# HpWang-whu/RoReg

Hardware: AMD Instinct MI355X
Metric: pair-registrations/sec (higher is better)
Workload: dtype f32 (every f32 operand enters the fp16 matrix cores as hi + lo fp16 under a per-keypoint power-of-two block scale: <= 22 significant bits relative to a CONSERVATIVE per-keypoint bound -- measured on the extractor: the bound sits 2^2..2^6 above the keypoint's true coefficient maximum (config.f16x2_sc

## Files before the change

### include/roreg_hip.h

```cpp
#ifndef ROREG_HIP_H
#define ROREG_HIP_H

#include <stdint.h>
#include <stddef.h>

#ifdef __cplusplus
extern "C" {
#endif

#define ROREG_ABI_VERSION 6
int roreg_abi_version(void);
const char *roreg_last_error(void);

int roreg_set_group_tables(const int32_t *P_host, const int32_t *Nei_host, const double *R_host);

size_t roreg_group_conv_packed_size(int Cin, int Cout, int KS);
int roreg_group_conv_pack_weights(const float *W_host , int Cin, int Cout, int KS,
                                  float *wpack_host );
size_t roreg_group_conv_workspace_size(int B, int Cin, int Cout, int Lin, int Lout, int KS);
int roreg_group_conv(const float *x, const float *wpack, const float *bias,
                     const float *bn_scale, const float *bn_shift, const float *residual,
                     float *out, const int32_t *gather,
                     int B, int Cin, int Cout, int Lin, int Lout, int KS,
                     float *workspace, size_t workspace_floats, void *stream);
// ... 75 lines not shown
int roreg_des2r_irrep(const float *coef1, const int64_t *rows1, const float *coef0, const int64_t *rows0, const void *feats1,
                      const void *feats0, int feat_bf16, int M, int64_t *idx_out, void *stream);
int roreg_des2r_recheck_count(int reset, int32_t *count_out);
int roreg_feat_coefs(const void *x, int x_bf16, float *out, int B, int C, int split, void *stream);

int roreg_et_gather(const void *before0, const void *before1, const void *after0, const void *after1,
                    int feat_bf16 ,
                    const int64_t *rows0, const int64_t *rows1, const int64_t *pre_idx, int M,
                    float *x_out, void *stream);

int roreg_quat_to_trans(const float *q, const int64_t *anchor, const double *keys0, const int64_t *rows0,
                        const double *keys1, const int64_t *rows1, int M,
                        double *Trans_out, float *quat_out, void *stream);

int roreg_ransac_score(const double *k0, const double *k1, const double *w, int w_f32, int M,
                       const double *Trans, const int64_t *hyp_rows, int H, double ird,
                       double *overlap_out, int32_t *best_out, uint8_t *mask_out, void *stream);

int roreg_refine(const double *k0, const double *k1, const double *w, int w_f32, int M,
                 const double *T_in, int t_in_stride ,
                 const double *Trans, const int64_t *hyp_rows, const int32_t *best,
                 double dist, double *T_out, double *stats_out ,
                 void *stream);

typedef struct {
    const void *before0, *before1, *after0, *after1;
    const double *keys0, *keys1;
    const int64_t *matches;
    const int64_t *sel;
    int32_t n, pad_;
    int64_t off;
    const float *coef0, *coef1;
} roreg_lt_task;
int roreg_lt_prepare_batch(const roreg_lt_task *tasks_dev, int n_tasks, int max_n, int flags, int64_t *dr_out, float *x_out,
                           const float *bn_scale , const float *bn_shift, float *x_bound_out , void *stream);
int roreg_lt_finish_batch(const roreg_lt_task *tasks_dev, int n_tasks, int max_n, const float *q_all, const int64_t *dr_all,
                          double *Trans_out, void *stream);
int roreg_role_max(const void *before, const void *after, int feat_bf16, const float *bn_scale , const float *bn_shift, float *out,
                   int N, void *stream);
int roreg_row_bound_roles(const void *x_spatial, int x_bf16, float *bound_out, const float *role_scale, const float *role_shift, float *role_out, int B,
                          void *stream);
int roreg_inv_descriptor_roles(const void *eqv, int eqv_bf16, float *inv, const float *role_scale, const float *role_shift, float *role_out, int N,
                               void *stream);
int roreg_lt_prepare_rows(const roreg_lt_task *tasks_dev, const float *const *roles_dev, int n_tasks, int max_n, int flags, int64_t *dr_out,
                          uint64_t *rows_out, float *x_bound_out, void *stream);

typedef struct {
    const double *keys0, *keys1;
    const int64_t *matches;
    const double *w;
    const double *Trans;
    const int64_t *hyp_rows;
    int32_t M, H;
    int64_t koff;
} roreg_ransac_task;
size_t roreg_ransac_batch_workspace(int n_tasks, long long total_M, int max_H);
int roreg_ransac_batch(const roreg_ransac_task *tasks_dev, int n_tasks, long long total_M, int max_M, int max_H, double ird,
                       int w_f32 ,
                       int32_t *best_out, double *T1_out, double *stats1_out, double *T2_out, double *stats2_out,
                       void *workspace, size_t workspace_bytes, void *stream);

int roreg_refine_batch(const roreg_ransac_task *tasks_dev, const int32_t *sel_dev, int n_sel, long long total_M, const double *T_in,
                       double dist, int w_f32, double *T_out, double *stats_out, const void *workspace, void *stream);

int roreg_mt_shuffle_prefix(const uint32_t *seeds, int n_jobs, const int32_t *sizes, int per_job, int take, int64_t *out, int n_threads);

int roreg_mt_stream_shuffle_prefix(uint32_t *key, int32_t *pos, const int32_t *sizes, int n_lists, int take, int64_t *out);

int roreg_yohoc_draw(const uint32_t *words, long long n_words, const double *cdf, const int32_t *bin_size, int max_iter, int max_tries,
                     int32_t *bin_out, int64_t *pick_out, int32_t *n_hyp_out, long long *words_used);

typedef struct {
    const void *src;
    const int64_t *rows;
    void *dst;
    int32_t n, pad_;
} roreg_gather_task;
int roreg_gather_rows_batch(const roreg_gather_task *tasks_dev, int n_tasks, int max_n, int row_bytes, void *stream);

int roreg_gather_rows_f64(const double *src, const int64_t *rows, int M, int width, double *out, void *stream);

size_t roreg_topk_dot_workspace_size(int m, int n, int k);
int roreg_topk_dot(const float *A, int m, const float *B, int n, int k, int64_t *idx_out, float *val_out ,
                   float *ws, size_t ws_floats, const int32_t *segA, const int32_t *segB, int n_seg, int max_m, int max_n, void *stream);

int roreg_linear(const float *x, int L, int Cin, const float *W , const float *b, int Cout, float *y, void *stream);
int roreg_linear_path(int path);
int roreg_linear_cat3(const float *pos , const float *table , const int64_t *idx ,
                      const float *conf , int m, int k, const float *W , const float *b, int Cout, float *y, void *stream);
int roreg_linear_mfma(const float *x, int L, int Cin, const float *W , const float *b, int Cout, float *y, void *stream);

int roreg_instnorm_stats(const float *h, int L, int C, float eps, float *mean_rstd, double *ws, const int32_t *seg_off, int n_seg,
                         int mult, void *stream);

int roreg_mlp_tail(const float *h, int L, int Cmid, const float *mean_rstd, const float *W2 , const float *b2,
                   float *y, const int32_t *seg_off, int n_seg, int mult, void *stream);
int roreg_mlp_tail_mfma(const float *h, int L, int Cmid, const float *mean_rstd, const float *W2 , const float *b2,
                   float *y, const int32_t *seg_off, int n_seg, int mult, void *stream);

int roreg_context_colmax(const float *R, int L, const int32_t *seg_off, int n_seg, int max_len, float *ctx_out, float *ws, void *stream);

int roreg_knn_attention(const float *qp, const float *kp, const float *vp, const int64_t *idx, int k_is_table, int v_is_table,
                        int m, int k, float *x_out, void *stream);

int roreg_rm_elementwise(int op, const float *a, const float *b, const float *c, const int64_t *idx, int L, int k, int C,
                         float *out, float *ws, void *stream);

size_t roreg_sinkhorn_workspace_size(int m, int n);
int roreg_sinkhorn(const float *src_final, int m, const float *tgt_final, int n, float alpha, int iters, float *Z_out,
                   int64_t *matches0, int64_t *matches1, float *mscores0, float *mscores1, float *ws, size_t ws_floats, void *stream);

size_t roreg_sinkhorn_batch_workspace_size(int n_seg, int max_m, int max_n, long long total_m, long long total_n);
int roreg_sinkhorn_batch_consts(const int32_t *seg_src_host, const int32_t *seg_tgt_host, int n_seg, float *consts_host);
int roreg_sinkhorn_batch(const float *src_final, const float *tgt_final, const int32_t *seg_src, const int32_t *seg_tgt,
                         const int32_t *seg_src_host, const int32_t *seg_tgt_host, const float *consts, int n_seg, float alpha, int iters,
                         int64_t *matches0, int64_t *matches1, float *mscores0, float *mscores1, float *ws, size_t ws_floats,
                         void *stream);

size_t roreg_sinkhorn_batch2_workspace_size(int n_seg, int max_m, int max_n, long long total_m, long long total_n);
int roreg_sinkhorn_batch2(const float *src_final, const float *tgt_final, const int32_t *seg_src, const int32_t *seg_tgt,
                          const int32_t *seg_src_host, const int32_t *seg_tgt_host, const float *consts, int n_seg, float alpha, int iters,
                          int64_t *matches0, int64_t *matches1, float *mscores0, float *mscores1, float *ws, size_t ws_floats,
                          int recompute, void *stream);
size_t roreg_sinkhorn_batch3_workspace_size(int n_seg, int max_m, int max_n, long long total_m, long long total_n, int recompute, int want_Z);
int roreg_sinkhorn_batch3(const float *src_final, const float *tgt_final, const int32_t *seg_src, const int32_t *seg_tgt,
                          const int32_t *seg_src_host, const int32_t *seg_tgt_host, const float *consts, int n_seg, float alpha, int iters,
                          int64_t *matches0, int64_t *matches1, float *mscores0, float *mscores1, float *ws, size_t ws_floats,
                          int recompute, float *Z_out, void *stream);
int roreg_write_files(const char *const *paths, const void *const *headers, const int32_t *header_len, const void *const *data,
                      const int64_t *nbytes, int n, int n_threads);
int roreg_yohoc_draw_many(const uint32_t *seeds, int n_pairs, const int64_t *anchors, const int64_t *offsets, int max_iter, int max_tries,
                          int64_t *rows_out, int32_t *n_hyp_out, double *giveup_out, int n_threads);
size_t roreg_mlp_head_workspace(int L, int n_seg, int C1);
int roreg_mlp_head(const float *x, const float *pos, const float *table, const int64_t *idx, const float *conf, int m, int k, int L, int Cin,
                   const float *W1, const float *b1, int C1, const float *Wr, const float *br, float *h, float *y, const int32_t *seg_off,
                   int n_seg, int mult, float eps, float *mean_rstd, double *ws, void *stream);
int roreg_sinkhorn_early_exit(int on);
int roreg_sinkhorn_iteration_stats(long long *iterations, long long *pairs, int reset, void *stream);

int roreg_set_fourier_tables(const float *F_host);
size_t roreg_irrep_gemm_tiles(int O, int B, int32_t *tiles_host);
size_t roreg_irrep_gemm_tiles_m(int O, int B, int tile_m , int32_t *tiles_host);
int roreg_irrep_gemm(const float *const *X, float *const *Out, const float *const *Add, const float *const *Wpack, int C, int O, int B,
                     const int32_t *tiles_dev, int n_tiles, void *stream);
int roreg_irrep_gemm_split(const float *const *X, float *const *Out, const float *const *Add, const void *const *Wsplit, int C, int O, int B,
                           const int32_t *tiles_dev, int n_tiles, void *stream);
int roreg_irrep_gemm_f16x2(const float *const *X, float *const *Out, const float *const *Add, const void *const *Wsplit2,
                           const float *x_bound_dev, int w_exp, const float *next_u_dev, const float *next_v_dev, float *out_bound_dev,
                           int C, int O, int B, const int32_t *tiles_dev, int n_tiles,
                           int tile_m ,
                           int x_planes , void *stream);
int roreg_gemm_persistent(int on);
int roreg_gemm_thin(int on);
int roreg_row_bound(const void *x_spatial, int x_bf16 , const float *bn_scale, const float *bn_shift,
                    float *bound_out, int B, int C, void *stream);
int roreg_ft_nonlin(const float *Xin , const float *x_spatial, const float *bias,
                    const float *bias2, const float *bn_scale, const float *bn_shift, const float *resid_spatial,
                    float *Xout , float *out_spatial ,
                    const int32_t *g_map ,
                    int Lout , int Lvalid,
                    int B, int C, int split ,
                    const float *out_bound ,
                    float *out_rowmax ,
                    int spatial_bf16 ,
                    int out_planes ,
                    void *stream);
int roreg_ft_nonlin_packed(const float *Xin, const float *bias, const float *bn_scale, const float *bn_shift, uint32_t *out_words,
                           const int32_t *g_map, int Lout, int Lvalid, int B, int C, const float *out_bound, float *raw_col, int raw_g,
                           void *stream);
int roreg_ft_nonlin_gathered(const uint64_t *rows , const int64_t *dr , int feat_bf16, const float *bn_scale ,
                             const float *bn_shift, float *Xout, int B, const float *out_bound , int out_planes, void *stream);

typedef struct roreg_icp_grid_desc {
    double origin[3];
    double edge;
    int32_t dims[3];
    int32_t n;
    int64_t cells;
    int64_t reserved;
} roreg_icp_grid_desc;
size_t roreg_icp_grid_size(const double *lo_host, const double *hi_host, int n, double max_dist, roreg_icp_grid_desc *desc_host,
                           size_t *workspace_bytes);
int roreg_icp_grid_build(const float *points, const roreg_icp_grid_desc *desc_host, void *grid, void *workspace, size_t workspace_bytes,
                         void *stream);
typedef struct roreg_icp_task {
    const void *tgt_grid;
    const void *src_grid;
    const double *T0;
    int32_t n_src;
    int32_t slot0;
} roreg_icp_task;
size_t roreg_icp_batch_workspace(int n_tasks, long long total_slots);
int roreg_icp_batch(const roreg_icp_task *tasks, int n_tasks, const int32_t *work, int n_work, long long total_slots, double max_dist,
                    int max_iter, double tol_deg, double tol_t, double *T_out, int32_t *iters_out, int32_t *inliers_out, double *rmse_out,
                    int32_t *status_out, int32_t *assign_out, double *stats_out, void *workspace, size_t workspace_bytes, void *stream);

int roreg_icp_normals(const void *grid, double radius, int min_neighbors, double *out, void *stream);
typedef struct roreg_icp_plane_task {
    const void *tgt_grid;
    const void *src_grid;
    const double *tgt_normals;
    const double *T0;
    int32_t n_src;
    int32_t slot0;
} roreg_icp_plane_task;
size_t roreg_icp_plane_batch_workspace(int n_tasks, long long total_slots);
int roreg_icp_plane_batch(const roreg_icp_plane_task *tasks, int n_tasks, const int32_t *work, int n_work, long long total_slots, double max_dist,
                          int max_iter, double tol_deg, double tol_t, double *T_out, int32_t *iters_out, int32_t *inliers_out, double *rmse_out,
                          int32_t *status_out, int32_t *assign_out, double *stats_out, void *workspace, size_t workspace_bytes, void *stream);

typedef struct roreg_icp_gicp_task {
    const void *tgt_grid;
    const void *src_grid;
    const double *tgt_normals;
    const double *src_normals;
    const double *T0;
    double epsilon;
    int32_t n_src;
    int32_t slot0;
} roreg_icp_gicp_task;
size_t roreg_icp_gicp_batch_workspace(int n_tasks, long long total_slots);
int roreg_icp_gicp_batch(const roreg_icp_gicp_task *tasks, int n_tasks, const int32_t *work, int n_work, long long total_slots, double max_dist,
                         int max_iter, double tol_deg, double tol_t, double *T_out, int32_t *iters_out, int32_t *inliers_out, double *rmse_out,
                         int32_t *status_out, int32_t *assign_out, double *stats_out, void *workspace, size_t workspace_bytes, void *stream);

size_t roreg_icp_eval_workspace(int n_pairs, long long total_slots);
int roreg_icp_eval_batch(const roreg_icp_task *tasks, int n_pairs, const int32_t *work, int n_work, long long total_slots, double max_dist,
                         double *stats_out, double *info_out, int32_t *status_out, int32_t *assign_out, void *workspace, size_t workspace_bytes,
                         void *stream);

size_t roreg_voxel_workspace(int n);
int roreg_voxel_downsample(const float *points, int n, double voxel, int32_t *inverse, int32_t *first, int32_t *counts, int32_t *coords,
                           double *centroid, int32_t *info, void *workspace, size_t workspace_bytes, void *stream);

typedef struct roreg_pg_graph {
    int32_t node0, n_nodes, edge0, n_edges, act0, n_act, anchor, reserved0;
    int64_t h0;
    double tau, lambda0, tol_t, tol_rot, tol_cost, reserved1;
} roreg_pg_graph;
size_t roreg_pg_workspace(const roreg_pg_graph *graphs_host, int n_graphs);
int roreg_pg_optimize_batch(const roreg_pg_graph *graphs_host, const roreg_pg_graph *graphs, int n_graphs, const int32_t *edge_i,
                            const int32_t *edge_j, const int32_t *edge_graph, const double *transforms, const double *infos, const int32_t *var,
                            const int32_t *inc_ptr, const int32_t *inc_edge, const int32_t *act_graph, const int32_t *act_node,
                            const int32_t *walk, int has_init, int max_iter, double *poses, double *cost_out, int32_t *iters_out,
                            int32_t *status_out, double *weights_out, double *chi2_out, double *history_out, double *lin_out, double *H_out,
                            double *gd_out, void *workspace, size_t workspace_bytes, void *stream);

size_t roreg_sparse_map_workspace(int n);
int roreg_sparse_stride_map(const int32_t *coords, int n, int ts, const int32_t *cuts, int n_items, int32_t *coarse, int32_t *parent,
                            int32_t *coarse_cuts, int32_t *info, void *workspace, size_t workspace_bytes, void *stream);
int roreg_sparse_kernel_map(const int32_t *coords_in, int n_in, const int32_t *coords_out, int n_out, int k, int step, int32_t *map,
                            int32_t *info, void *workspace, size_t workspace_bytes, void *stream);
int roreg_sparse_conv(const float *x, int ldx, int Cin, int n_in, const int32_t *map, int n_out, int K, const float *W, int Cout,
                      const float *scale, const float *shift, const float *residual, int ldr, int relu, float *out, int ldo, void *stream);
int roreg_sparse_l2norm(const float *x, int n, int C, float *out, void *stream);

int roreg_profile_enable(int on);
int roreg_profile_read(int slot, double *total_ms, int *launches);

#ifdef __cplusplus
}
#endif
#endif
```

### roreg_amd/_abi.py

```python
import ctypes
from ctypes import c_int, c_void_p, c_size_t, c_double, c_float, c_char_p

import numpy as np

ABI_VERSION = 6

_P = c_void_p
PROTOTYPES = {
    'roreg_abi_version': (c_int, []),
    'roreg_last_error': (c_char_p, []),
    'roreg_set_group_tables': (c_int, [_P, _P, _P]),
    'roreg_group_conv_packed_size': (c_size_t, [c_int, c_int, c_int]),
    'roreg_group_conv_pack_weights': (c_int, [_P, c_int, c_int, c_int, _P]),
    'roreg_group_conv_workspace_size': (c_size_t, [c_int, c_int, c_int, c_int, c_int, c_int]),
    'roreg_group_conv': (c_int, [_P, _P, _P, _P, _P, _P, _P, _P, c_int, c_int, c_int, c_int, c_int, c_int, _P, c_size_t, _P]),
    'roreg_group_conv_split': (c_int, [_P, _P, _P, _P, _P, _P, _P, _P, c_int, c_int, c_int, c_int, c_int, c_int, c_int, _P]),
    'roreg_group_conv_f16x2': (c_int, [_P, _P, c_int, _P, _P, _P, c_float, c_float, _P, _P, _P, _P, _P, c_int, c_int, c_int, c_int, c_int, c_int, c_int, _P]),
    'roreg_group_conv_f16x2_packed': (c_int, [_P, _P, c_int, _P, _P, _P, _P, _P, _P, c_int, c_int, c_int, c_int, c_int, c_int, c_int, _P]),
    'roreg_dense_f16x2': (c_int, [_P, _P, c_int, _P, _P, _P, c_float, c_float, _P, _P, c_int, _P, _P, c_int, c_int, c_int, _P]),
    'roreg_dense_split': (c_int, [_P, _P, _P, _P, _P, _P, c_int, _P, c_int, c_int, c_int, _P]),
    'roreg_gf_finalize': (c_int, [_P, _P, c_int, _P, c_int, _P]),
    'roreg_det_score': (c_int, [_P, _P, c_int, _P]),
    'roreg_inv_descriptor': (c_int, [_P, c_int, _P, c_int, _P]),
    'roreg_nn_search': (c_int, [_P, _P, c_int, _P, _P, c_int, c_int, _P, _P, _P, _P]),
    'roreg_nn_search_ex': (c_int, [_P, _P, c_int, _P, _P, c_int, c_int, c_int, _P, _P, _P, _P]),
    'roreg_pdist': (c_int, [_P, c_int, _P, c_int, c_int, c_int, _P, _P]),
    'roreg_knn_search_workspace': (c_size_t, [c_int, c_int]),
    'roreg_knn_search': (c_int, [_P, c_int, _P, c_int, c_int, c_int, _P, _P, c_size_t, _P]),
    'roreg_knn_search_ex': (c_int, [_P, c_int, _P, c_int, c_int, c_int, c_int, _P, _P, _P, c_size_t, _P]),
    'roreg_knn_search_seg_workspace': (c_size_t, [ctypes.c_longlong, c_int, c_int, c_int]),
    'roreg_knn_search_seg': (c_int, [_P, _P, _P, _P, c_int, ctypes.c_longlong, c_int, c_int, c_int, c_int, _P, _P, c_size_t, _P]),
    'roreg_mutual_matches': (c_int, [_P, _P, c_int, c_int, _P, _P, _P, _P, _P]),
    'roreg_mutual_match_batch_workspace': (c_size_t, [c_int, c_int]),
    'roreg_mutual_match_batch': (c_int, [_P, c_int, c_int, _P, _P, _P, c_size_t, _P]),
    'roreg_des2r': (c_int, [_P, _P, _P, _P, c_int, _P, _P, _P]),
    'roreg_set_des2r_tables': (c_int, [c_int, _P, _P, _P, _P]),
    'roreg_group_corr_irrep': (c_int, [_P, _P, _P, _P, c_int, c_int, _P, _P]),
    'roreg_group_corr_mfma': (c_int, [_P, _P, _P, _P, c_int, c_int, _P, _P]),
    'roreg_des2r_irrep': (c_int, [_P, _P, _P, _P, _P, _P, c_int, c_int, _P, _P]),
    'roreg_des2r_recheck_count': (c_int, [c_int, _P]),
    'roreg_feat_coefs': (c_int, [_P, c_int, _P, c_int, c_int, c_int, _P]),
    'roreg_et_gather': (c_int, [_P, _P, _P, _P, c_int, _P, _P, _P, c_int, _P, _P]),
    'roreg_quat_to_trans': (c_int, [_P, _P, _P, _P, _P, _P, c_int, _P, _P, _P]),
    'roreg_ransac_score': (c_int, [_P, _P, _P, c_int, c_int, _P, _P, c_int, c_double, _P, _P, _P, _P]),
    'roreg_refine': (c_int, [_P, _P, _P, c_int, c_int, _P, c_int, _P, _P, _P, c_double, _P, _P, _P]),
    'roreg_lt_prepare_batch': (c_int, [_P, c_int, c_int, c_int, _P, _P, _P, _P, _P, _P]),
    'roreg_lt_finish_batch': (c_int, [_P, c_int, c_int, _P, _P, _P, _P]),
    'roreg_role_max': (c_int, [_P, _P, c_int, _P, _P, _P, c_int, _P]),
    'roreg_row_bound_roles': (c_int, [_P, c_int, _P, _P, _P, _P, c_int, _P]),
    'roreg_inv_descriptor_roles': (c_int, [_P, c_int, _P, _P, _P, _P, c_int, _P]),
    'roreg_lt_prepare_rows': (c_int, [_P, _P, c_int, c_int, c_int, _P, _P, _P, _P]),
    'roreg_ransac_batch_workspace': (c_size_t, [c_int, ctypes.c_longlong, c_int]),
    'roreg_ransac_batch': (c_int, [_P, c_int, ctypes.c_longlong, c_int, c_int, c_double, c_int, _P, _P, _P, _P, _P, _P, c_size_t, _P]),
    'roreg_refine_batch': (c_int, [_P, _P, c_int, ctypes.c_longlong, _P, ctypes.c_double, c_int, _P, _P, _P, _P]),
    'roreg_yohoc_draw': (c_int, [_P, ctypes.c_longlong, _P, _P, c_int, c_int, _P, _P, _P, _P]),
    'roreg_gather_rows_batch': (c_int, [_P, c_int, c_int, c_int, _P]),
    'roreg_gather_rows_f64': (c_int, [_P, _P, c_int, c_int, _P, _P]),
    'roreg_group_corr': (c_int, [_P, _P, _P, _P, c_int, c_int, _P, _P, _P]),
    'roreg_topk_dot_workspace_size': (c_size_t, [c_int, c_int, c_int]),
    'roreg_topk_dot': (c_int, [_P, c_int, _P, c_int, c_int, _P, _P, _P, c_size_t, _P, _P, c_int, c_int, c_int, _P]),
    'roreg_context_colmax': (c_int, [_P, c_int, _P, c_int, c_int, _P, _P, _P]),
    'roreg_sinkhorn_batch_workspace_size': (c_size_t, [c_int, c_int, c_int, ctypes.c_longlong, ctypes.c_longlong]),
    'roreg_sinkhorn_batch_consts': (c_int, [_P, _P, c_int, _P]),
    'roreg_sinkhorn_batch': (c_int, [_P, _P, _P, _P, _P, _P, _P, c_int, c_float, c_int, _P, _P, _P, _P, _P, c_size_t, _P]),
    'roreg_sinkhorn_batch2_workspace_size': (c_size_t, [c_int, c_int, c_int, ctypes.c_longlong, ctypes.c_longlong]),
    'roreg_sinkhorn_batch2': (c_int, [_P, _P, _P, _P, _P, _P, _P, c_int, c_float, c_int, _P, _P, _P, _P, _P, c_size_t, c_int, _P]),
    'roreg_sinkhorn_batch3_workspace_size': (c_size_t, [c_int, c_int, c_int, ctypes.c_longlong, ctypes.c_longlong, c_int, c_int]),
    'roreg_sinkhorn_batch3': (c_int, [_P, _P, _P, _P, _P, _P, _P, c_int, c_float, c_int, _P, _P, _P, _P, _P, c_size_t, c_int, _P, _P]),
    'roreg_write_files': (c_int, [_P, _P, _P, _P, _P, c_int, c_int]),
    'roreg_yohoc_draw_many': (c_int, [_P, c_int, _P, _P, c_int, c_int, _P, _P, _P, c_int]),
    'roreg_mlp_head_workspace': (c_size_t, [c_int, c_int, c_int]),
    'roreg_mlp_head': (c_int, [_P, _P, _P, _P, _P, c_int, c_int, c_int, c_int, _P, _P, c_int, _P, _P, _P, _P, _P, c_int, c_int, c_float, _P, _P, _P]),
    'roreg_sinkhorn_early_exit': (c_int, [c_int]),
    'roreg_sinkhorn_iteration_stats': (c_int, [_P, _P, c_int, _P]),
    'roreg_linear': (c_int, [_P, c_int, c_int, _P, _P, c_int, _P, _P]),
    'roreg_linear_mfma': (c_int, [_P, c_int, c_int, _P, _P, c_int, _P, _P]),
    'roreg_linear_path': (c_int, [c_int]),
    'roreg_linear_cat3': (c_int, [_P, _P, _P, _P, c_int, c_int, _P, _P, c_int, _P, _P]),
    'roreg_gemm_persistent': (c_int, [c_int]),
    'roreg_gemm_thin': (c_int, [c_int]),
    'roreg_instnorm_stats': (c_int, [_P, c_int, c_int, c_float, _P, _P, _P, c_int, c_int, _P]),
    'roreg_mlp_tail': (c_int, [_P, c_int, c_int, _P, _P, _P, _P, _P, c_int, c_int, _P]),
    'roreg_mlp_tail_mfma': (c_int, [_P, c_int, c_int, _P, _P, _P, _P, _P, c_int, c_int, _P]),
    'roreg_knn_attention': (c_int, [_P, _P, _P, _P, c_int, c_int, c_int, c_int, _P, _P]),
    'roreg_rm_elementwise': (c_int, [c_int, _P, _P, _P, _P, c_int, c_int, c_int, _P, _P, _P]),
    'roreg_sinkhorn_workspace_size': (c_size_t, [c_int, c_int]),
    'roreg_sinkhorn': (c_int, [_P, c_int, _P, c_int, c_float, c_int, _P, _P, _P, _P, _P, _P, c_size_t, _P]),
    'roreg_icp_grid_size': (c_size_t, [_P, _P, c_int, c_double, _P, _P]),
    'roreg_icp_grid_build': (c_int, [_P, _P, _P, _P, c_size_t, _P]),
    'roreg_icp_batch_workspace': (c_size_t, [c_int, ctypes.c_longlong]),
    'roreg_icp_batch': (c_int, [_P, c_int, _P, c_int, ctypes.c_longlong, c_double, c_int, c_double, c_double, _P, _P, _P, _P, _P, _P, _P, _P, c_size_t, _P]),
    'roreg_icp_normals': (c_int, [_P, c_double, c_int, _P, _P]),
    'roreg_icp_plane_batch_workspace': (c_size_t, [c_int, ctypes.c_longlong]),
    'roreg_icp_plane_batch': (c_int, [_P, c_int, _P, c_int, ctypes.c_longlong, c_double, c_int, c_double, c_double, _P, _P, _P, _P, _P, _P, _P, _P, c_size_t, _P]),
    'roreg_icp_gicp_batch_workspace': (c_size_t, [c_int, ctypes.c_longlong]),
    'roreg_icp_gicp_batch': (c_int, [_P, c_int, _P, c_int, ctypes.c_longlong, c_double, c_int, c_double, c_double, _P, _P, _P, _P, _P, _P, _P, _P, c_size_t, _P]),
    'roreg_icp_eval_workspace': (c_size_t, [c_int, ctypes.c_longlong]),
    'roreg_icp_eval_batch': (c_int, [_P, c_int, _P, c_int, ctypes.c_longlong, c_double, _P, _P, _P, _P, _P, c_size_t, _P]),
    'roreg_voxel_workspace': (c_size_t, [c_int]),
    'roreg_voxel_downsample': (c_int, [_P, c_int, c_double, _P, _P, _P, _P, _P, _P, _P, c_size_t, _P]),
    'roreg_pg_workspace': (c_size_t, [_P, c_int]),
    'roreg_pg_optimize_batch': (c_int, [_P, _P, c_int, _P, _P, _P, _P, _P, _P, _P, _P, _P, _P, _P, c_int, c_int, _P, _P, _P, _P, _P, _P, _P, _P, _P, _P, _P, c_size_t, _P]),
    'roreg_sparse_map_workspace': (c_size_t, [c_int]),
    'roreg_sparse_stride_map': (c_int, [_P, c_int, c_int, _P, c_int, _P, _P, _P, _P, _P, c_size_t, _P]),
    'roreg_sparse_kernel_map': (c_int, [_P, c_int, _P, c_int, c_int, c_int, _P, _P, _P, c_size_t, _P]),
    'roreg_sparse_conv': (c_int, [_P, c_int, c_int, c_int, _P, c_int, c_int, _P, c_int, _P, _P, _P, c_int, c_int, _P, c_int, _P]),
    'roreg_sparse_l2norm': (c_int, [_P, c_int, c_int, _P, _P]),
    'roreg_profile_enable': (c_int, [c_int]),
    'roreg_profile_read': (c_int, [c_int, _P, _P]),
    'roreg_set_fourier_tables': (c_int, [_P]),
    'roreg_mt_shuffle_prefix': (c_int, [_P, c_int, _P, c_int, c_int, _P, c_int]),
    'roreg_mt_stream_shuffle_prefix': (c_int, [_P, _P, _P, c_int, c_int, _P]),
    'roreg_irrep_gemm_tiles': (c_size_t, [c_int, c_int, _P]),
    'roreg_irrep_gemm_tiles_m': (c_size_t, [c_int, c_int, c_int, _P]),
    'roreg_irrep_gemm': (c_int, [_P, _P, _P, _P, c_int, c_int, c_int, _P, c_int, _P]),
    'roreg_irrep_gemm_split': (c_int, [_P, _P, _P, _P, c_int, c_int, c_int, _P, c_int, _P]),
    'roreg_irrep_gemm_f16x2': (c_int, [_P, _P, _P, _P, _P, c_int, _P, _P, _P, c_int, c_int, c_int, _P, c_int, c_int, c_int, _P]),
    'roreg_row_bound': (c_int, [_P, c_int, _P, _P, _P, c_int, c_int, _P]),
    'roreg_ft_nonlin': (c_int, [_P, _P, _P, _P, _P, _P, _P, _P, _P, _P, c_int, c_int, c_int, c_int, c_int, _P, _P, c_int, c_int, _P]),
    'roreg_ft_nonlin_packed': (c_int, [_P, _P, _P, _P, _P, _P, c_int, c_int, c_int, c_int, _P, _P, c_int, _P]),
    'roreg_ft_nonlin_gathered': (c_int, [_P, _P, c_int, _P, _P, _P, c_int, _P, c_int, _P]),
}


_RANSAC_TASK = np.dtype([('keys0', np.uint64), ('keys1', np.uint64), ('matches', np.uint64), ('w', np.uint64), ('Trans', np.uint64),
                         ('hyp_rows', np.uint64), ('M', np.int32), ('H', np.int32), ('koff', np.int64)])

_MATCH_TASK = np.dtype([('desc0', np.uint64), ('desc1', np.uint64), ('rows0', np.uint64), ('rows1', np.uint64), ('m0', np.int32), ('m1', np.int32)])

_GATHER_TASK = np.dtype([('src', np.uint64), ('rows', np.uint64), ('dst', np.uint64), ('n', np.int32), ('pad', np.int32)])

_LT_TASK = np.dtype([('before0', np.uint64), ('before1', np.uint64), ('after0', np.uint64), ('after1', np.uint64), ('keys0', np.uint64),
                     ('keys1', np.uint64), ('matches', np.uint64), ('sel', np.uint64), ('n', np.int32), ('pad', np.int32), ('off', np.int64),
                     ('coef0', np.uint64), ('coef1', np.uint64)])

_ICP_GRID_DESC = np.dtype([('origin', np.float64, 3), ('edge', np.float64), ('dims', np.int32, 3), ('n', np.int32), ('cells', np.int64),
                           ('reserved', np.int64)])

_ICP_TASK = np.dtype([('tgt_grid', np.uint64), ('src_grid', np.uint64), ('T0', np.uint64), ('n_src', np.int32), ('slot0', np.int32)])

_ICP_PLANE_TASK = np.dtype([('tgt_grid', np.uint64), ('src_grid', np.uint64), ('tgt_normals', np.uint64), ('T0', np.uint64), ('n_src', np.int32),
                            ('slot0', np.int32)])

_ICP_GICP_TASK = np.dtype([('tgt_grid', np.uint64), ('src_grid', np.uint64), ('tgt_normals', np.uint64), ('src_normals', np.uint64), ('T0', np.uint64),
                           ('epsilon', np.float64), ('n_src', np.int32), ('slot0', np.int32)])

_PG_GRAPH = np.dtype([('node0', np.int32), ('n_nodes', np.int32), ('edge0', np.int32), ('n_edges', np.int32), ('act0', np.int32), ('n_act', np.int32),
                      ('anchor', np.int32), ('reserved0', np.int32), ('h0', np.int64), ('tau', np.float64), ('lambda0', np.float64),
                      ('tol_t', np.float64), ('tol_rot', np.float64), ('tol_cost', np.float64), ('reserved1', np.float64)])
```

### roreg_amd/_hip_fourier.py

```python
import os
from ctypes import c_void_p

import numpy as np
import torch

from . import hip as _core
from .hip import HipError, _check, _feat, _ptr, _stream, lib

__all__ = ['DenseSplitLayer', 'IRREP_DIMS', 'IRREP_OFFSETS', '_bf16_split3', '_keypoint_of_columns', '_ptr_array', '_res_ptr', '_tile_cache', 'bf16_split3_frags', 'bf16_split3_pack', 'bound_exp', 'coef_pitch', 'coef_size', 'coef_views', 'dense_split', 'ensure_fourier', 'f16_scale_exp', 'f16_split2_frags', 'f16_split2_pack', 'frag_pack', 'ft_nonlin', 'ft_nonlin_gathered', 'ft_nonlin_packed', 'gemm_persistent', 'gemm_thin', 'group_conv_split_pack', 'irrep_gemm', 'next_bound', 'next_bound_spatial', 'pack_coefs_f16x2', 'row_bound', 'unpack_coefs_f16x2', 'words_to_planes']


_fourier_ready = False
IRREP_DIMS = (1, 3, 3, 4, 5)
IRREP_OFFSETS = (0, 1, 10, 19, 35, 60)


def ensure_fourier():
    global _fourier_ready
    if not _fourier_ready:
        from .fourier import group_fourier
        F = np.ascontiguousarray(group_fourier().F, np.float32)
        _check(lib().roreg_set_fourier_tables(F.ctypes.data), 'roreg_set_fourier_tables')
        _fourier_ready = True


def _ptr_array(views):
    arr = (c_void_p * 5)(*[c_void_p(v.data_ptr()) for v in views])
    return arr


def coef_pitch(B):
    return (int(B) + 31) // 32 * 32


def coef_size(C, B):
    return 60 * C * coef_pitch(B)


def coef_views(buf, C, B):
    Bp = coef_pitch(B)
    return [buf[IRREP_OFFSETS[r] * C * Bp:IRREP_OFFSETS[r + 1] * C * Bp].view(IRREP_DIMS[r] * C, IRREP_DIMS[r] * Bp) for r in range(5)]


_tile_cache = {}


def _x_planes_kernel(x_planes):
    if not x_planes:
        return 0
    if x_planes is not True and x_planes in (1, 2):
        return int(x_planes)
    return 2 if _core.MFMA16 else 1


def irrep_gemm(X_buf, Wpacks, C, O, B, split=None, add=None, f16x2=None, x_bound=None, next_bound=None, x_planes=False):
    Bp = coef_pitch(B)
    if X_buf.numel() != 60 * C * Bp or (add is not None and add.numel() != 60 * O * Bp):
        raise HipError(f'irrep_gemm: coefficient buffers must hold 60*C*{Bp} floats (B={B} padded to the 32-keypoint pitch)')
    out = torch.empty(60 * O * Bp, dtype=torch.float32, device=X_buf.device)
    tile_m = 256 if (f16x2 is not None and O % 256 == 0 and not os.environ.get('ROREG_TILE_M128')) else 128
    key = (O, Bp, tile_m)
    t = _tile_cache.get(key)
    if t is None:
        n = lib().roreg_irrep_gemm_tiles_m(O, Bp, tile_m, None)
        host = np.empty((n, 3), np.int32)
        lib().roreg_irrep_gemm_tiles_m(O, Bp, tile_m, host.ctypes.data)
        t = torch.from_numpy(host).cuda()
        _tile_cache[key] = t
    xv = coef_views(X_buf, C, B); ov = coef_views(out, O, B)
    av = _ptr_array(coef_views(add, O, B)) if add is not None else None
    if _core.PROFILE is not None:
        e0 = torch.cuda.Event(enable_timing=True); e1 = torch.cuda.Event(enable_timing=True); e0.record()
    bound_out = None
    if f16x2 is not None:
        wl, w_exp = f16x2
        if x_bound is None or x_bound.numel() != Bp:
            raise HipError(f'irrep_gemm: the fp16 x 2 GEMM needs x_bound with one value per (padded) keypoint ({Bp})')
        nu = nv = None
        if next_bound is not None:
            nu, nv = next_bound
            if nu.numel() != O or nv.numel() != O:
                raise HipError('irrep_gemm: next_bound must hold one (u, v) per output channel')
            bound_out = torch.zeros(Bp, dtype=torch.float32, device=X_buf.device)
        _check(lib().roreg_irrep_gemm_f16x2(_ptr_array(xv), _ptr_array(ov), av, _ptr_array(wl), _ptr(x_bound, torch.float32), int(w_exp),
                                            _ptr(nu, torch.float32), _ptr(nv, torch.float32), _ptr(bound_out), C, O, Bp,
                                            _ptr(t, torch.int32), int(t.shape[0]), tile_m, _x_planes_kernel(x_planes), _stream()), 'roreg_irrep_gemm_f16x2')
    elif split is not None:
        _check(lib().roreg_irrep_gemm_split(_ptr_array(xv), _ptr_array(ov), av, _ptr_array(split), C, O, Bp, _ptr(t, torch.int32), int(t.shape[0]),
                                            _stream()), 'roreg_irrep_gemm_split')
    else:
        _check(lib().roreg_irrep_gemm(_ptr_array(xv), _ptr_array(ov), av, _ptr_array(Wpacks), C, O, Bp, _ptr(t, torch.int32), int(t.shape[0]), _stream()),
               'roreg_irrep_gemm')
    if _core.PROFILE is not None:
        e1.record(); _core.PROFILE.append((('irrep_gemm_f16x2' if f16x2 is not None else 'irrep_gemm_split' if split is not None else 'irrep_gemm', Bp, C, O), e0, e1))
    return (out, bound_out) if next_bound is not None else out


class _GemmSwitch:

    def __init__(self, entry, coerce, doc, on=None):
        self.entry, self.coerce, self.__doc__, self.on = entry, coerce, doc, on

    def __call__(self, on=True):
        return _GemmSwitch(self.entry, self.coerce, self.__doc__, self.coerce(on))

    def __enter__(self):
        self.prev = getattr(lib(), self.entry)(self.on)

    def __exit__(self, *exc):
        getattr(lib(), self.entry)(self.prev)
        return False


gemm_persistent = _GemmSwitch('roreg_gemm_persistent', int,
                              """`with hip.gemm_persistent(True | False):` -- how the 16x16x32 LDS-DMA GEMM is launched inside the block (roreg_gemm_persistent): persistent
    workgroups that claim tiles, or one workgroup per tile.  Same bits either way -- tests and A/B measurements.""")
gemm_thin = _GemmSwitch('roreg_gemm_thin', lambda on: int(bool(on)),
                        """`with hip.gemm_thin(True | False):` -- whether the thin layers (C == 32 or O == 32, fp16 x 2, word layout, no residual) run on their own
    kernels inside the block (roreg_gemm_thin; the default) or on the generic one.  Same bits either way -- tests and A/B measurements.""")


def row_bound(x, bn=None, roles=None):
    B, C = int(x.shape[0]), int(x.shape[1])
    out = torch.empty(coef_pitch(B), dtype=torch.float32, device=x.device)
    scale, shift = bn if bn is not None else (None, None)
    xp, bf = _feat(x)
    if roles is not None:
        if bn is not None or C != 32:
            raise HipError('row_bound: roles go with the 32-channel input features and no BatchNorm')
        r_scale, r_shift, role = _core._role_args(roles, B)
        _check(lib().roreg_row_bound_roles(xp, bf, _ptr(out), _ptr(r_scale), _ptr(r_shift), _ptr(role), B, _stream()), 'roreg_row_bound_roles')
        return out
    _check(lib().roreg_row_bound(xp, bf, _ptr(scale), _ptr(shift), _ptr(out), B, C, _stream()), 'roreg_row_bound')
    return out


def _keypoint_of_columns(d, Bp):
    n = torch.arange(d * Bp, device='cuda')
    return ((n // 32) // d) * 32 + (n % 32)


def bound_exp(bound):
    _, ex = torch.frexp(bound.float())
    e = torch.where((bound > 0) & torch.isfinite(bound), 14 - ex, torch.zeros_like(ex))
    return e.clamp(-100, 100)


def pack_coefs_f16x2(X_buf, C, B, bound=None):
    Bp = coef_pitch(B)
    views = coef_views(X_buf, C, B)
    if bound is None:
        bound = torch.zeros(Bp, dtype=torch.float32, device=X_buf.device)
        for r, v in enumerate(views):
            kp = _keypoint_of_columns(IRREP_DIMS[r], Bp)
            bound.scatter_reduce_(0, kp, v.abs().amax(0), 'amax')
    e = bound_exp(bound)
    out = torch.empty_like(X_buf)
    for r, (v, o) in enumerate(zip(views, coef_views(out, C, B))):
        kp = _keypoint_of_columns(IRREP_DIMS[r], Bp)
        y = torch.ldexp(v, e[kp][None, :])
        hi = y.half()
        lo = (y - hi.float()).half()
        w = (hi.view(torch.int16).to(torch.int32) & 0xffff) | (lo.view(torch.int16).to(torch.int32) << 16)
        o.copy_(w.view(torch.float32))
    return out, bound


def words_to_planes(X_words, C, B):
    w = X_words.contiguous().view(torch.int32).view(-1, 2, 16)
    hi = (w & 0xffff).to(torch.int16).transpose(1, 2); lo = (w >> 16).to(torch.int16).transpose(1, 2)
    return torch.cat([hi.reshape(-1, 32), lo.reshape(-1, 32)], 1).contiguous().view(torch.float32).view(-1)


def unpack_coefs_f16x2(X_words, bound, C, B):
    Bp = coef_pitch(B)
    e = bound_exp(bound)
    out = torch.empty_like(X_words)
    for r, (v, o) in enumerate(zip(coef_views(X_words, C, B), coef_views(out, C, B))):
        kp = _keypoint_of_columns(IRREP_DIMS[r], Bp)
        w = v.view(torch.int32)
        hi = (w & 0xffff).to(torch.int16).view(torch.float16).float()
        lo = (w >> 16).to(torch.int16).view(torch.float16).float()
        o.copy_(torch.ldexp(hi + lo, -e[kp][None, :]))
    return out


def next_bound_spatial(bn, bias):
    scale, shift = bn
    sc = scale.detach().double().abs().cpu(); sh = shift.detach().double().abs().cpu()
    b = bias.detach().double().cpu()
    k = 1.0 + 2.0 ** -9
    u = (np.sqrt(60.0) * k) * sc
    v = k * (sc * b.abs() + sh) + 1e-30
    return u.float().cuda().contiguous(), v.float().cuda().contiguous()


def ft_nonlin_packed(B, C, coef_in, bias, bn, out_bound, g_map=None, Lout=60, Lvalid=60, raw_g=None):
    ensure_fourier()
    dev = coef_in.device
    if coef_in.numel() != coef_size(C, B) or out_bound.numel() != coef_pitch(B):
        raise HipError('ft_nonlin_packed: coef_in / out_bound sizes')
    words = torch.empty((B, C, Lout if g_map is not None else 60), dtype=torch.int32, device=dev)
    raw = torch.empty((B, C), dtype=torch.float32, device=dev) if raw_g is not None else None
    scale, shift = bn if bn is not None else (None, None)
    _check(lib().roreg_ft_nonlin_packed(_ptr(coef_in, torch.float32), _ptr(bias), _ptr(scale), _ptr(shift), _ptr(words), _ptr(g_map, torch.int32),
                                        int(Lout), int(Lvalid), B, C, _ptr(out_bound, torch.float32), _ptr(raw), int(raw_g or 0), _stream()),
           'roreg_ft_nonlin_packed')
    return words, raw


def next_bound(bn, bias, bias2=None):
    scale, shift = bn
    sc = scale.detach().double().abs().cpu(); sh = shift.detach().double().abs().cpu()
    b = bias.detach().double().cpu() + (bias2.detach().double().cpu() if bias2 is not None else 0.0)
    k = 1.0 + 2.0 ** -9
    u = (60.0 * k) * sc
    v = (np.sqrt(60.0) * k) * (sc * b.abs() + sh) + 1e-30
    return u.float().cuda().contiguous(), v.float().cuda().contiguous()


def ft_nonlin(B, C, coef_in=None, x_spatial=None, bias=None, bias2=None, bn=None, resid_spatial=None, spatial_out=False,
              g_map=None, Lout=60, Lvalid=60, split=False, out_bound=None, want_rowmax=False, planes=False):
    ensure_fourier()
    dev = (coef_in if coef_in is not None else x_spatial).device
    if spatial_out:
        out = torch.empty((B, C, Lout if g_map is not None else 60), dtype=torch.float32, device=dev); xout = None; osp = _ptr(out)
    else:
        out = torch.empty(coef_size(C, B), dtype=torch.float32, device=dev); xout = _ptr(out); osp = None
    scale, shift = bn if bn is not None else (None, None)
    if want_rowmax and not spatial_out:
        raise HipError('ft_nonlin: want_rowmax goes with spatial_out')
    amax = torch.zeros(B, dtype=torch.float32, device=dev) if want_rowmax else None
    if coef_in is not None and coef_in.numel() != coef_size(C, B):
        raise HipError(f'ft_nonlin: coef_in must hold 60*C*{coef_pitch(B)} floats')
    if out_bound is not None and out_bound.numel() != coef_pitch(B):
        raise HipError(f'ft_nonlin: out_bound must hold one value per (padded) keypoint ({coef_pitch(B)})')
    xs, bf_x = _feat(x_spatial); rs, bf_r = _feat(resid_spatial)
    if x_spatial is not None and resid_spatial is not None and bf_x != bf_r:
        raise HipError('ft_nonlin: x_spatial and resid_spatial must share one dtype')
    _check(lib().roreg_ft_nonlin(_ptr(coef_in, torch.float32), xs, _ptr(bias),
                                 _ptr(bias2), _ptr(scale), _ptr(shift), rs, xout, osp,
                                 _ptr(g_map, torch.int32), int(Lout), int(Lvalid), B, C, 2 if split == 'f16x2' else (1 if split else 0),
                                 _ptr(out_bound, torch.float32), _ptr(amax), bf_x or bf_r, 1 if planes else 0, _stream()), 'roreg_ft_nonlin')
    return (out, amax) if want_rowmax else out


def ft_nonlin_gathered(g, bn=None, planes=False):
    ensure_fourier()
    _core.ensure_tables()
    B = g.shape[0]
    out = torch.empty(coef_size(128, B), dtype=torch.float32, device=g.rows.device)
    scale, shift = bn if bn is not None else (None, None)
    if g.bound.numel() != coef_pitch(B) or g.dr.numel() != B:
        raise HipError('ft_nonlin_gathered: rows / dr / bound sizes')
    _check(lib().roreg_ft_nonlin_gathered(_ptr(g.rows, torch.int64), _ptr(g.dr, torch.int64), 1 if g.bf16 else 0, _ptr(scale), _ptr(shift), _ptr(out), B,
                                          _ptr(g.bound, torch.float32), 1 if planes else 0, _stream()), 'roreg_ft_nonlin_gathered')
    return out


def _bf16_split3(x):
    out = []
    rem = np.ascontiguousarray(x, np.float32)
    for _ in range(3):
        u = rem.view(np.uint32)
        r = ((u >> 16) & 1) + 0x7fff
        hi = ((u + r) >> 16).astype(np.uint16)
        out.append(hi)
        rem = rem - (hi.astype(np.uint32) << 16).view(np.float32)
    return out


def f16_scale_exp(absmax):
    return 14 - int(np.frexp(float(absmax))[1]) if absmax > 0 else 0
# ... 82 lines not shown
```

### roreg_amd/csrc/fourier.hip

```cpp
#include "common.h"
#include "primitives.h"
#include <algorithm>
#include <atomic>
#include <cmath>
#include <cstdlib>
#include <type_traits>
#include <utility>
#include <vector>

namespace {

constexpr int NIRR = 5;

struct GemmDescs {
    const float *X[NIRR];
    float *Out[NIRR];
    const float *Add[NIRR];
    const float4 *W[NIRR];
    int K[NIRR], M[NIRR], Mpad[NIRR], N[NIRR];
};

__device__ __forceinline__ void lds_dma16(const void *src, void *dst) {
    __builtin_amdgcn_global_load_lds((const __attribute__((address_space(1))) void *)src, (__attribute__((address_space(3))) void *)dst, 16, 0, 0);
}

template <int CT>
__global__ __launch_bounds__(256, 2) void irrep_gemm_kernel(GemmDescs p, const int *__restrict__ tiles) {
    extern __shared__ __attribute__((aligned(16))) char smem[];
    float *xs = reinterpret_cast<float *>(smem);
    constexpr int NCOL = 256, OT = 128, NQ = CT / 8;
    const int tid = threadIdx.x, lane = tid & 63, w = tid >> 6;
    const int j = lane & 31, h = lane >> 5;
    const int irr = tiles[blockIdx.x * 3], mt = tiles[blockIdx.x * 3 + 1], nt = tiles[blockIdx.x * 3 + 2];
    if (irr < 0) return;
    const float *__restrict__ X = p.X[irr];
    const float4 *__restrict__ W = p.W[irr];
    const int K = p.K[irr], M = p.M[irr], Mpad = p.Mpad[irr], N = p.N[irr];
    const int wo = w & 1, wb = w >> 1;
    const int m_wave = mt * OT + wo * 64;
    const int n0 = nt * NCOL;
    const int ncol_wave = wb * 128;

    f32x16 acc[2][4];
#pragma unroll
    for (int a = 0; a < 2; ++a)
#pragma unroll
        for (int t = 0; t < 4; ++t)
#pragma unroll
            for (int r = 0; r < 16; ++r) acc[a][t][r] = 0.f;

    int ncol = n0 + lane * 4;
    if (ncol > N - 4) ncol = N - 4;
    const float *xrow = X + ncol;
    auto issue_tile = [&](int k0, int buf) {
#pragma unroll
        for (int i = 0; i < CT / 4; ++i) {
            const int c = w * (CT / 4) + i;
            lds_dma16(xrow + (size_t)(k0 + c) * N, xs + (buf * CT + c) * NCOL);
        }
    };
    float4 a_cur[NQ][2], a_nxt[NQ][2];
    auto load_a = [&](int k0, float4 (&a)[NQ][2]) {
        const float4 *wk = W + ((size_t)(k0 / 8) * Mpad + m_wave + j) * 2 + h;
#pragma unroll
        for (int q = 0; q < NQ; ++q)
#pragma unroll
            for (int ot = 0; ot < 2; ++ot) a[q][ot] = wk[((size_t)q * Mpad + ot * 32) * 2];
    };

    issue_tile(0, 0);
    load_a(0, a_cur);
    asm volatile("s_waitcnt vmcnt(0)" ::: "memory");
    __syncthreads();
    int buf = 0;
    for (int k0 = 0; k0 < K; k0 += CT) {
        const bool more = k0 + CT < K;
        if (more) {
            issue_tile(k0 + CT, buf ^ 1);
            load_a(k0 + CT, a_nxt);
        }
        const float *xt = xs + buf * (CT * NCOL) + ncol_wave + j;
#pragma unroll
        for (int q = 0; q < NQ; ++q) {
#pragma unroll
            for (int r = 0; r < 4; ++r) {
                float bv[4];
#pragma unroll
                for (int t = 0; t < 4; ++t) bv[t] = xt[(q * 8 + r * 2 + h) * NCOL + t * 32];
#pragma unroll
                for (int ot = 0; ot < 2; ++ot) {
                    const float av = r == 0 ? a_cur[q][ot].x : r == 1 ? a_cur[q][ot].y : r == 2 ? a_cur[q][ot].z : a_cur[q][ot].w;
#pragma unroll
                    for (int t = 0; t < 4; ++t) acc[ot][t] = __builtin_amdgcn_mfma_f32_32x32x2f32(av, bv[t], acc[ot][t], 0, 0, 0);
                }
            }
        }
        if (more) {
            asm volatile("s_waitcnt vmcnt(0)" ::: "memory");
#pragma unroll
            for (int q = 0; q < NQ; ++q) { a_cur[q][0] = a_nxt[q][0]; a_cur[q][1] = a_nxt[q][1]; }
        }
        __syncthreads();
        buf ^= 1;
    }
    float *__restrict__ Out = p.Out[irr];
    const float *__restrict__ Add = p.Add[irr];
#pragma unroll
    for (int ot = 0; ot < 2; ++ot)
#pragma unroll
        for (int t = 0; t < 4; ++t) {
            const int n = n0 + ncol_wave + t * 32 + j;
            if (n >= N) continue;
#pragma unroll
            for (int r = 0; r < 16; ++r) {
                const int m = cd_row32(r, h, m_wave + ot * 32);
                if (m < M) {
                    float o = acc[ot][t][r];
                    if (Add) o += Add[(size_t)m * N + n];
                    Out[(size_t)m * N + n] = o;
                }
            }
        }
}

typedef unsigned u32x4 __attribute__((ext_vector_type(4)));

struct GemmSplitDescs {
    const float *X[NIRR];
    float *Out[NIRR];
    const float *Add[NIRR];
    const float *xbound;
    int w_exp;
    const float *nb_u, *nb_v;
    float *out_bound;
    int O;
    const void *W[NIRR];
    int K[NIRR], M[NIRR], Mpad[NIRR], N[NIRR];
};

__constant__ int kIrrDim[NIRR] = {1, 3, 3, 4, 5};
__device__ __forceinline__ int column_keypoint(int n, int d) { return ((n >> 5) / d) * 32 + (n & 31); }

enum : int { COLS_BLOCKED = 0, COLS_INTERLEAVED = 1, COLS_PAIRED = 2 };
template <int MODE>
__device__ __forceinline__ int wave_col(int t, int j) { return MODE == COLS_INTERLEAVED ? 4 * j + t : MODE == COLS_PAIRED ? t * 32 + (j >> 1) + 16 * (j & 1) : t * 32 + j; }
template <int MODE>
__device__ __forceinline__ int col_slot(int n ) {
    static_assert(MODE != COLS_PAIRED, "the LDS-DMA kernel does not stage through fragment slots");
    if constexpr (MODE == COLS_BLOCKED) return n ^ ((n >> 3) & 1);
    const int t = n & 3, q = (n & 127) >> 2;
    return (n & ~127) | (t * 32 + ((q + 4 * t) & 31));
}

template <int NT, int NCOL>
__device__ __forceinline__ void bound_stage_merge(const GemmSplitDescs &p, const unsigned *cm, int n0, int N, int dirr) {
    const int tid = threadIdx.x;
    __syncthreads();
    for (int i = tid; i < NCOL; i += NT) {
        const int n = n0 + i;
        if (n < N) atomicMax(reinterpret_cast<unsigned *>(p.out_bound) + column_keypoint(n, dirr), cm[i]);
    }
}

template <int NP, int WO, int COLS = COLS_INTERLEAVED>
__device__ __forceinline__ void gemm_split_epilogue(const GemmSplitDescs &p, int irr, int mt, int n0, int wo, int ncol_wave, f32x16 (&acc)[2][4],
                                                    char *smem) {
    constexpr int NCOL = 256, OT = WO * 64, NT = WO * 128;
    const int tid = threadIdx.x, lane = tid & 63;
    const int j = lane & 31, h = lane >> 5;
    const unsigned jc = (unsigned)wave_col<COLS == COLS_PAIRED ? COLS_PAIRED : COLS_BLOCKED>(0, j);
    const int M = p.M[irr], N = p.N[irr];
    const int dirr = kIrrDim[irr];
    float *__restrict__ Out = p.Out[irr];
    const float *__restrict__ Add = p.Add[irr];
    float oscale[4] = {1.f, 1.f, 1.f, 1.f};
    float bmax[4] = {0.f, 0.f, 0.f, 0.f};
    const bool want_bound = NP == 2 && p.out_bound != nullptr;
    float *su = reinterpret_cast<float *>(smem), *sv = su + OT;
    unsigned *cm = reinterpret_cast<unsigned *>(sv + OT);
    if constexpr (NP == 2) {
#pragma unroll
        for (int t = 0; t < 4; ++t) {
            const int n = n0 + ncol_wave + wave_col<COLS>(t, j);
            if (n < N) oscale[t] = ldexpf(1.f, -(bound_exp(p.xbound[column_keypoint(n, dirr)]) + p.w_exp));
        }
        if (want_bound) {
            for (int i = tid; i < OT; i += NT) {
                const int m = mt * OT + i;
                su[i] = m < M ? p.nb_u[m % p.O] : 0.f; sv[i] = m < M ? p.nb_v[m % p.O] : 0.f;
            }
            for (int i = tid; i < NCOL; i += NT) cm[i] = 0u;
            __syncthreads();
        }
    }
    const bool interior = (mt + 1) * OT <= M && n0 + NCOL <= N;
    if (interior) {
        const size_t base = (size_t)(mt * OT + wo * 64) * N + n0 + ncol_wave;
        float *__restrict__ ob = Out + base;
        const float *__restrict__ ab = Add ? Add + base : nullptr;
        const unsigned un = (unsigned)N;
        auto body = [&](auto has_add, auto has_bound) {
#pragma unroll
            for (int ot = 0; ot < 2; ++ot)
#pragma unroll
                for (int rq = 0; rq < 4; ++rq) {
                    float res[4][4];
                    if constexpr (decltype(has_add)::value) {
#pragma unroll
                        for (int rr = 0; rr < 4; ++rr) {
                            const unsigned roff = (unsigned)(ot * 32 + rr + 8 * rq + 4 * h) * un;
                            if constexpr (COLS == COLS_INTERLEAVED) {
                                const float4 q = *reinterpret_cast<const float4 *>(ab + roff + 4u * (unsigned)j);
                                res[rr][0] = q.x; res[rr][1] = q.y; res[rr][2] = q.z; res[rr][3] = q.w;
                            } else {
#pragma unroll
                                for (int t = 0; t < 4; ++t) res[rr][t] = ab[roff + jc + t * 32];
                            }
                        }
                    }
#pragma unroll
                    for (int rr = 0; rr < 4; ++rr) {
                        const int r = rq * 4 + rr;
                        const int rl = ot * 32 + rr + 8 * rq + 4 * h;
                        float ur = 0.f, vr = 0.f;
                        if constexpr (decltype(has_bound)::value) { ur = su[wo * 64 + rl]; vr = sv[wo * 64 + rl]; }
                        float o4[4];
#pragma unroll
                        for (int t = 0; t < 4; ++t) {
                            float o = acc[ot][t][r];
                            if constexpr (NP == 2) o *= oscale[t];
                            if constexpr (decltype(has_add)::value) o += res[rr][t];
                            o4[t] = o;
                            if constexpr (decltype(has_bound)::value) bmax[t] = fmaxf(bmax[t], fmaf(ur, fabsf(o), vr));
                        }
                        if constexpr (COLS == COLS_INTERLEAVED) {
                            *reinterpret_cast<float4 *>(ob + (unsigned)rl * un + 4u * (unsigned)j) = make_float4(o4[0], o4[1], o4[2], o4[3]);
                        } else {
#pragma unroll
                            for (int t = 0; t < 4; ++t) ob[(unsigned)rl * un + jc + t * 32] = o4[t];
                        }
                    }
                }
        };
        if (Add) { if (want_bound) body(std::true_type{}, std::true_type{}); else body(std::true_type{}, std::false_type{}); }
        else     { if (want_bound) body(std::false_type{}, std::true_type{}); else body(std::false_type{}, std::false_type{}); }
    } else {
#pragma unroll
        for (int ot = 0; ot < 2; ++ot)
#pragma unroll
            for (int r = 0; r < 16; ++r) {
                const int row = cd_row32(r, h, wo * 64 + ot * 32);
                const int m = mt * OT + row;
                if (m >= M) continue;
                float ur = 0.f, vr = 0.f;
                if constexpr (NP == 2) { if (want_bound) { ur = su[row]; vr = sv[row]; } }
#pragma unroll
                for (int t = 0; t < 4; ++t) {
                    const int n = n0 + ncol_wave + wave_col<COLS>(t, j);
                    if (n >= N) continue;
                    float o = acc[ot][t][r];
                    if constexpr (NP == 2) o *= oscale[t];
                    if (Add) o += Add[(size_t)m * N + n];
                    Out[(size_t)m * N + n] = o;
                    if constexpr (NP == 2) { if (want_bound) bmax[t] = fmaxf(bmax[t], fmaf(ur, fabsf(o), vr)); }
                }
            }
    }
    if constexpr (NP == 2) {
        if (want_bound) {
#pragma unroll
            for (int t = 0; t < 4; ++t) {
                const float bm = fmaxf(bmax[t], __shfl_xor(bmax[t], 32));
                if (h == 0) atomicMax(cm + ncol_wave + wave_col<COLS>(t, j), __float_as_uint(bm));
            }
            bound_stage_merge<NT, NCOL>(p, cm, n0, N, dirr);
        }
    }
}

#define ROREG_WAIT_X(cnt, xr) asm volatile("s_waitcnt vmcnt(" #cnt ")" : "+v"(xr[0]), "+v"(xr[1]), "+v"(xr[2]), "+v"(xr[3]), "+v"(xr[4]), "+v"(xr[5]), "+v"(xr[6]), "+v"(xr[7]) :: "memory")
template <int CT, int NP, int WO, int BIG, int PIPE = 0>
__global__ __launch_bounds__(WO * 128, 2) void irrep_gemm_split_kernel(GemmSplitDescs p, const int *__restrict__ tiles) {
    using frag = typename std::conditional<NP == 3, bf16x8, f16x8>::type;
    extern __shared__ __attribute__((aligned(16))) char smem[];
    constexpr int NCOL = 256, OT = WO * 64, NT = WO * 128, CPT = 512 / NT;
// ... 235 lines not shown
        H[i] = __builtin_amdgcn_perm(v[2 * i + 1], v[2 * i], 0x05040100u);
        L[i] = __builtin_amdgcn_perm(v[2 * i + 1], v[2 * i], 0x07060302u);
    }
    hi = __builtin_bit_cast(f16x8, H); lo = __builtin_bit_cast(f16x8, L);
}

template <int D>
__device__ __forceinline__ void thin_k_body(const GemmSplitDescs &p, int irr, int nt, f16x8 *as, float *uv ) {
    constexpr int NS = 2 * D;
    constexpr int NI = 2 * NS;
    constexpr int NDMA = (NI + 7) / 8;
    constexpr int SLOT = NI * 64;
    const int tid = threadIdx.x, lane = tid & 63, w = tid >> 6, j = lane & 31, h = lane >> 5;
    const int N = p.N[irr], Mpad = p.Mpad[irr], O = p.O;
    const int nblk = D * O / 32;
    const f16x8 *__restrict__ W = reinterpret_cast<const f16x8 *>(p.W[irr]);
    const size_t split_stride = (size_t)NS * 2 * Mpad;
    const int n = nt * 256 + w * 32 + j;
    const bool live = n < N;
    const int nl = live ? n : N - 32 + j;

    const f16x8 *wsrc[NDMA];
    int wdst[NDMA];
#pragma unroll
    for (int q = 0; q < NDMA; ++q) {
        const int i = (w + 8 * q) % NI, sp = i / NS, ks = i % NS;
        wsrc[q] = W + sp * split_stride + (size_t)(ks * 2 + h) * Mpad + j;
        wdst[q] = i * 64;
    }
    auto dma = [&](int blk, int slot) {
#pragma unroll
        for (int q = 0; q < NDMA; ++q)
            lds_dma16(wsrc[q] + blk * 32, as + slot * SLOT + wdst[q]);
        __builtin_amdgcn_sched_barrier(0);
        asm volatile("" ::: "memory");
    };
    dma(0, 0);

    f16x8 bh[NS], bl[NS];
    {
        const unsigned *xq = reinterpret_cast<const unsigned *>(p.X[irr]) + nl + (size_t)(8 * h) * N;
#pragma unroll
        for (int s = 0; s < NS; ++s) {
            unsigned v[8];
#pragma unroll
            for (int e = 0; e < 8; ++e) v[e] = __builtin_nontemporal_load(xq + (size_t)(16 * s + e) * N);
            words_to_frags(v, bh[s], bl[s]);
        }
    }
    if (!live) {
        for (int blk = 0; blk < nblk; ++blk) {
            asm volatile("s_waitcnt vmcnt(0) lgkmcnt(0)\n\ts_barrier" ::: "memory");
            dma(blk + 1 < nblk ? blk + 1 : nblk - 1, (blk + 1) & 1);
        }
        asm volatile("s_waitcnt vmcnt(0)" ::: "memory");
        return;
    }
    const float oscale = ldexpf(1.f, -(bound_exp(p.xbound[column_keypoint(n, D)]) + p.w_exp));
    float bmax = 0.f;
    float *__restrict__ Out = p.Out[irr];
    const unsigned ocol = (unsigned)(4 * h) * (unsigned)N + (unsigned)n;
    const unsigned uvbase = (unsigned)(uintptr_t)uv + 16 * h;

    auto store_quad = [&](int pb, const f32x16 &c, int rq, const f32x4 &u, const f32x4 &v, auto bound_c) {
        float *ob = Out + (size_t)(pb * 32 + 8 * rq) * N;
        #pragma unroll
        for (int rr = 0; rr < 4; ++rr) {
            const float o = c[rq * 4 + rr] * oscale;
            __builtin_nontemporal_store(o, ob + (size_t)rr * N + ocol);
            if constexpr (decltype(bound_c)::value) bmax = fmaxf(bmax, fmaf(u[rr], fabsf(o), v[rr]));
        }
    };
    auto read_uv = [&](int pb, int rq, f32x4 &u, f32x4 &v) {
        const unsigned a = uvbase + (unsigned)(((pb * 32) % O + 8 * rq) * 4);
        asm volatile("ds_read_b128 %0, %1" : "=v"(u) : "v"(a));
        asm volatile("ds_read_b128 %0, %1" : "=v"(v) : "v"(a + 4 * 512));
    };
    auto block = [&](int blk, f32x16 &cur, const f32x16 &prev, auto drain_c, auto w16_c, auto bound_c) {
        constexpr bool DRAIN = decltype(drain_c)::value, BOUND = decltype(bound_c)::value;
        if constexpr (decltype(w16_c)::value) asm volatile("s_waitcnt vmcnt(16)\n\ts_barrier" ::: "memory");
        else asm volatile("s_waitcnt vmcnt(0) lgkmcnt(0)\n\ts_barrier" ::: "memory");
        dma(blk + 1 < nblk ? blk + 1 : nblk - 1, (blk + 1) & 1);
        const unsigned abase = (unsigned)(uintptr_t)(as + (blk & 1) * SLOT) + lane * 16;
        f16x8 a[2][2];
        a[0][0] = lds_frag_read(abase, 0); a[0][1] = lds_frag_read(abase, NS * 1024);
#pragma unroll
        for (int r = 0; r < 16; ++r) cur[r] = 0.f;
#pragma unroll
        for (int s = 0; s < NS; ++s) {
            f32x4 u[4], v[4];
#pragma unroll
            for (int rq = 0; rq < 4; ++rq)
                if (DRAIN && BOUND && rq * NS / 4 == s) read_uv(blk - 1, rq, u[rq], v[rq]);
            ROREG_WAIT_LDS2(a[s & 1][0], a[s & 1][1]);
#pragma unroll
            for (int rq = 0; rq < 4; ++rq)
                if (DRAIN && BOUND && rq * NS / 4 == s) ROREG_WAIT_LDS2(u[rq], v[rq]);
            if (s + 1 < NS) { a[(s + 1) & 1][0] = lds_frag_read(abase, (s + 1) * 1024); a[(s + 1) & 1][1] = lds_frag_read(abase, (NS + s + 1) * 1024); }
            cur = __builtin_amdgcn_mfma_f32_32x32x16_f16(a[s & 1][1], bh[s], cur, 0, 0, 0);
            cur = __builtin_amdgcn_mfma_f32_32x32x16_f16(a[s & 1][0], bl[s], cur, 0, 0, 0);
            cur = __builtin_amdgcn_mfma_f32_32x32x16_f16(a[s & 1][0], bh[s], cur, 0, 0, 0);
#pragma unroll
            for (int rq = 0; rq < 4; ++rq)
                if (DRAIN && rq * NS / 4 == s) store_quad(blk - 1, prev, rq, u[rq], v[rq], bound_c);
        }
    };
    auto run = [&](auto bound_c) {
        using T = std::true_type; using F = std::false_type;
        f32x16 c0, c1;
#pragma unroll
        for (int r = 0; r < 16; ++r) { c0[r] = 0.f; c1[r] = 0.f; }
        block(0, c0, c1, F{}, F{}, bound_c);
        if (nblk > 1) block(1, c1, c0, T{}, F{}, bound_c);
        for (int blk = 2; blk < nblk; blk += 2) {
            block(blk, c0, c1, T{}, T{}, bound_c);
            if (blk + 1 < nblk) block(blk + 1, c1, c0, T{}, T{}, bound_c);
        }
        const f32x16 &last = (nblk & 1) ? c0 : c1;
        f32x4 u[4], v[4];
        if constexpr (decltype(bound_c)::value) {
#pragma unroll
            for (int rq = 0; rq < 4; ++rq) read_uv(nblk - 1, rq, u[rq], v[rq]);
#pragma unroll
            for (int rq = 0; rq < 4; ++rq) ROREG_WAIT_LDS2(u[rq], v[rq]);
        }
#pragma unroll
        for (int rq = 0; rq < 4; ++rq) store_quad(nblk - 1, last, rq, u[rq], v[rq], bound_c);
    };
    if (p.out_bound != nullptr) {
        run(std::true_type{});
        const float bm = fmaxf(bmax, __shfl_xor(bmax, 32));
        if (h == 0) atomicMax(reinterpret_cast<unsigned *>(p.out_bound) + column_keypoint(n, D), __float_as_uint(bm));
    } else {
        run(std::false_type{});
    }
    asm volatile("s_waitcnt vmcnt(0)" ::: "memory");
}

__global__ __launch_bounds__(512) void irrep_gemm_thin_k_kernel(GemmSplitDescs p) {
    __shared__ __attribute__((aligned(16))) f16x8 as[2 * 20 * 64];
    __shared__ __attribute__((aligned(16))) float uv[2 * 512];
    if (p.out_bound != nullptr)
        for (int i = threadIdx.x; i < p.O; i += 512) { uv[i] = p.nb_u[i]; uv[512 + i] = p.nb_v[i]; }
    int irr, nt;
    thin_wg_irrep<false>(p, irr, nt);
    switch (irr) {
        case 0: thin_k_body<1>(p, irr, nt, as, uv); break;
        case 1: case 2: thin_k_body<3>(p, irr, nt, as, uv); break;
        case 3: thin_k_body<4>(p, irr, nt, as, uv); break;
        default: thin_k_body<5>(p, irr, nt, as, uv); break;
    }
}

template <int D, int CB>
__device__ __forceinline__ void thin_m_body(const GemmSplitDescs &p, int irr, int nt, f16x8 *as) {
    constexpr int NI = 2 * D;
    constexpr int NDMA = (NI + 3) / 4;
    constexpr int SLOT = NI * 64;
    const int tid = threadIdx.x, lane = tid & 63, w = tid >> 6, j = lane & 31, h = lane >> 5;
    const int N = p.N[irr], Mpad = p.Mpad[irr], K = p.K[irr];
    const int nsteps = K / 16;
    const f16x8 *__restrict__ W = reinterpret_cast<const f16x8 *>(p.W[irr]);
    const size_t split_stride = (size_t)nsteps * 2 * Mpad;
    const int n = nt * (128 * CB) + w * (32 * CB) + CB * j;
    const bool live = n < N;
    const int nl = live ? n : N - CB;

    const f16x8 *wsrc[NDMA];
    int wdst[NDMA];
#pragma unroll
    for (int q = 0; q < NDMA; ++q) {
        const int i = (w + 4 * q) % NI, sp = i / D, rb = i % D;
        wsrc[q] = W + sp * split_stride + (size_t)h * Mpad + rb * 32 + j;
        wdst[q] = i * 64;
    }
    auto dma = [&](int s, int slot) {
        const size_t off = (size_t)(s < nsteps ? s : nsteps - 1) * 2 * Mpad;
#pragma unroll
        for (int q = 0; q < NDMA; ++q)
            lds_dma16(wsrc[q] + off, as + slot * SLOT + wdst[q]);
        __builtin_amdgcn_sched_barrier(0);
    };
    const unsigned *xp = reinterpret_cast<const unsigned *>(p.X[irr]);
    const unsigned xoff = ((unsigned)(8 * h) * (unsigned)N + (unsigned)nl) * 4u;
    typedef typename std::conditional<CB == 1, unsigned, unsigned long long>::type xword;
    auto load_x = [&](int s, xword (&x)[8]) {
        const unsigned *q = xp + (size_t)(s < nsteps ? s : nsteps - 1) * 16 * N;
#pragma unroll
        for (int e = 0; e < 8; ++e) {
            if constexpr (CB == 1) asm volatile("global_load_dword %0, %1, %2" : "=v"(x[e]) : "v"(xoff), "s"(q + (size_t)e * N) : "memory");
            else asm volatile("global_load_dwordx2 %0, %1, %2" : "=v"(x[e]) : "v"(xoff), "s"(q + (size_t)e * N) : "memory");
        }
        __builtin_amdgcn_sched_barrier(0);
    };

    f32x16 acc[D][CB];
#pragma unroll
    for (int rb = 0; rb < D; ++rb)
#pragma unroll
        for (int cb = 0; cb < CB; ++cb)
#pragma unroll
            for (int r = 0; r < 16; ++r) acc[rb][cb][r] = 0.f;

    auto step = [&](int s, int slot, xword (&x)[8]) {
        if constexpr (NDMA == 1) ROREG_WAIT_X(9, x); else if constexpr (NDMA == 2) ROREG_WAIT_X(10, x); else ROREG_WAIT_X(11, x);
        asm volatile("s_barrier" ::: "memory");
        f16x8 bh[CB], bl[CB];
#pragma unroll
        for (int cb = 0; cb < CB; ++cb) {
            unsigned v[8];
#pragma unroll
            for (int e = 0; e < 8; ++e) v[e] = (unsigned)(x[e] >> (CB == 1 ? 0 : 32 * cb));
            words_to_frags(v, bh[cb], bl[cb]);
        }
        __builtin_amdgcn_sched_barrier(0);
        const int fill = slot >= 1 ? slot - 1 : 2;
        dma(s + 2, fill);
        load_x(s + 2, x);
        const unsigned abase = (unsigned)(uintptr_t)(as + slot * SLOT) + lane * 16;
        f16x8 a[2][2];
        a[0][0] = lds_frag_read(abase, 0); a[0][1] = lds_frag_read(abase, D * 1024);
#pragma unroll
        for (int rb = 0; rb < D; ++rb) {
            ROREG_WAIT_LDS2(a[rb & 1][0], a[rb & 1][1]);
            if (rb + 1 < D) { a[(rb + 1) & 1][0] = lds_frag_read(abase, (rb + 1) * 1024); a[(rb + 1) & 1][1] = lds_frag_read(abase, (D + rb + 1) * 1024); }
#pragma unroll
            for (int cb = 0; cb < CB; ++cb) {
                const f16x8 b[2] = {bh[cb], bl[cb]};
                acc[rb][cb] = split_mma<2>(a[rb & 1], b, acc[rb][cb]);
            }
        }
    };
    xword xa[8], xb[8];
    dma(0, 0); load_x(0, xa);
    dma(1, 1); load_x(1, xb);
    int slot = 0;
    for (int s = 0; s < nsteps; s += 2) {
        step(s, slot, xa);
        slot = slot == 2 ? 0 : slot + 1;
        step(s + 1, slot, xb);
        slot = slot == 2 ? 0 : slot + 1;
    }
    ROREG_WAIT_X(0, xa);
    ROREG_WAIT_X(0, xb);

    if (!live) return;
    float oscale[CB];
#pragma unroll
    for (int cb = 0; cb < CB; ++cb) oscale[cb] = ldexpf(1.f, -(bound_exp(p.xbound[column_keypoint(n + cb, D)]) + p.w_exp));
    const bool want_bound = p.out_bound != nullptr;
    float ur[16], vr[16], bmax[CB];
#pragma unroll
    for (int cb = 0; cb < CB; ++cb) bmax[cb] = 0.f;
    if (want_bound) {
#pragma unroll
        for (int r = 0; r < 16; ++r) { const int o = cd_row32(r, h); ur[r] = p.nb_u[o]; vr[r] = p.nb_v[o]; }
    }
    float *__restrict__ ob = p.Out[irr] + n + (size_t)(4 * h) * N;
#pragma unroll
    for (int rb = 0; rb < D; ++rb)
#pragma unroll
        for (int r = 0; r < 16; ++r) {
            float o[CB];
#pragma unroll
            for (int cb = 0; cb < CB; ++cb) {
                o[cb] = acc[rb][cb][r] * oscale[cb];
                if (want_bound) bmax[cb] = fmaxf(bmax[cb], fmaf(ur[r], fabsf(o[cb]), vr[r]));
            }
            float *dst = ob + (size_t)cd_row32(r, 0, rb * 32) * N;
            if constexpr (CB == 1) *dst = o[0]; else *reinterpret_cast<float2 *>(dst) = make_float2(o[0], o[CB - 1]);
        }
    if (want_bound) {
#pragma unroll
        for (int cb = 0; cb < CB; ++cb) {
            const float bm = fmaxf(bmax[cb], __shfl_xor(bmax[cb], 32));
            if (h == 0) atomicMax(reinterpret_cast<unsigned *>(p.out_bound) + column_keypoint(n + cb, D), __float_as_uint(bm));
        }
    }
}

__global__ __launch_bounds__(256, 2) void irrep_gemm_thin_m_kernel(GemmSplitDescs p) {
    __shared__ __attribute__((aligned(16))) f16x8 as[3 * 10 * 64];
    int irr, nt;
    thin_wg_irrep<true>(p, irr, nt);
    switch (irr) {
        case 0: thin_m_body<1, 2>(p, irr, nt, as); break;
        case 1: case 2: thin_m_body<3, 2>(p, irr, nt, as); break;
        case 3: thin_m_body<4, 1>(p, irr, nt, as); break;
        default: thin_m_body<5, 1>(p, irr, nt, as); break;
    }
}
#undef ROREG_WAIT_LDS2
#undef ROREG_WAIT_X


template <int XIMG, int QUAD, int OFF>
__device__ __forceinline__ void xdma_read_b(unsigned a, f16x8 (&b)[2]) {
    unsigned long long u[4];
    asm volatile("ds_read_b64_tr_b16 %0, %1 offset:%2" : "=v"(u[0]) : "v"(a), "n"(OFF));
    asm volatile("ds_read_b64_tr_b16 %0, %1 offset:%2" : "=v"(u[1]) : "v"(a), "n"(OFF + QUAD));
    asm volatile("ds_read_b64_tr_b16 %0, %1 offset:%2" : "=v"(u[2]) : "v"(a), "n"(XIMG + OFF));
    asm volatile("ds_read_b64_tr_b16 %0, %1 offset:%2" : "=v"(u[3]) : "v"(a), "n"(XIMG + OFF + QUAD));
    struct Pair { unsigned long long lo, hi; };
    b[0] = __builtin_bit_cast(f16x8, Pair{u[0], u[1]});
    b[1] = __builtin_bit_cast(f16x8, Pair{u[2], u[3]});
}

template <int BIG>
__global__ __launch_bounds__(512, 2) void irrep_gemm_xdma_kernel(GemmSplitDescs p, const int *__restrict__ tiles) {
    using frag = f16x8;
    extern __shared__ __attribute__((aligned(16))) char smem[];
    constexpr int NCOL = 256, OT = 256;
    constexpr int XIMG = 16 * NCOL * 2, XSTAGE = 2 * XIMG;
    constexpr int ABUF = 2 * 2 * OT;
    char *xs = smem;
    frag *as = reinterpret_cast<frag *>(smem + 3 * XSTAGE);
    const int tid = threadIdx.x, lane = tid & 63, w = tid >> 6;
    const int j = lane & 31, h = lane >> 5;
    const int irr = tiles[blockIdx.x * 3], mt = tiles[blockIdx.x * 3 + 1], nt = tiles[blockIdx.x * 3 + 2];
    if (irr < 0) return;
    const frag *__restrict__ W = reinterpret_cast<const frag *>(p.W[irr]);
    const int K = p.K[irr], Mpad = p.Mpad[irr], N = p.N[irr];
    const size_t split_stride = (size_t)(K / 16) * 2 * Mpad;
    const int wo = w % 4, wb = w / 4;
    const int n0 = nt * NCOL;
    const int ncol_wave = wb * 128;
    const int nsteps = K / 16;

    f32x16 acc[2][4];
#pragma unroll
    for (int a = 0; a < 2; ++a)
#pragma unroll
        for (int t = 0; t < 4; ++t)
#pragma unroll
            for (int r = 0; r < 16; ++r) acc[a][t][r] = 0.f;

    const int x_plane = w >> 2;
    const char *xsrc[2];
    int xdst[2];
#pragma unroll
    for (int i2 = 0; i2 < 2; ++i2) {
        const int mm = (2 * w + i2) & 7;
        const int pi = mm * 64 + lane;
        const int beta = pi >> 3, r = (pi & 7) >> 1, half = pi & 1;
        const int k = 4 * (beta >> 4) + r;
        int col = n0 + 16 * (beta & 15) + 8 * half;
        if (col > N - 8) col = N - 8;
        xsrc[i2] = reinterpret_cast<const char *>(p.X[irr]) + (size_t)k * N * 4 + (col >> 5) * 128 + x_plane * 64 + (col & 31) * 2;
        xdst[i2] = x_plane * XIMG + mm * 1024;
    }
    const size_t xstep = (size_t)16 * N * 4;
    auto dma_x = [&](int i2, int kstep, int stage) {
        const char *q = xsrc[i2] + (size_t)(kstep < nsteps ? kstep : nsteps - 1) * xstep;
        lds_dma16(q, xs + stage * XSTAGE + xdst[i2]);
    };
    const frag *wsrc = W + (size_t)(tid / OT) * Mpad + mt * OT + (tid % OT);
    auto dma_w = [&](int sp, int kstep, int buf) {
        const frag *q = wsrc + (size_t)(kstep < nsteps ? kstep : nsteps - 1) * 2 * Mpad;
        lds_dma16(q + sp * split_stride, as + buf * ABUF + sp * (2 * OT) + w * 64);
    };
    const int aslot = h * OT + wo * 64 + j;
    const unsigned xlane = (unsigned)(uintptr_t)xs + (unsigned)((2 * h * 16 + wb * 8 + ((lane >> 4) & 1)) * 128 + (lane & 15) * 8);
    frag aA[2][2], aB[2][2], b[4][2];
    auto read_a = [&](int buf, frag (&a)[2][2]) {
        const frag *at = as + buf * ABUF + aslot;
#pragma unroll
        for (int ot = 0; ot < 2; ++ot)
#pragma unroll
            for (int sp = 0; sp < 2; ++sp) a[ot][sp] = at[sp * (2 * OT) + ot * 32];
    };
    auto read_b = [&](unsigned stage_off, auto tc) { xdma_read_b<XIMG, 2048, decltype(tc)::value * 256>(xlane + stage_off, b[decltype(tc)::value]); };
#define ROREG_WAIT_FRAGS(waits)                                                                                                          \
    asm volatile(waits : "+v"(b[0][0]), "+v"(b[0][1]), "+v"(b[1][0]), "+v"(b[1][1]), "+v"(b[2][0]), "+v"(b[2][1]), "+v"(b[3][0]), "+v"(b[3][1]) \
                 :: "memory")
    auto step = [&](int ks, int wbuf, unsigned xs_next , int xs_fill ,
                    const frag (&a)[2][2], frag (&an)[2][2]) {
        const frag *aq = as + (wbuf ^ 1) * ABUF + aslot;
        auto mm = [&](int t, int i) {
            const f16x8 bb = b[t][i == 1 ? 1 : 0];
            const int ai = i == 0 ? 1 : 0;
            acc[0][t] = __builtin_amdgcn_mfma_f32_32x32x16_f16(a[0][ai], bb, acc[0][t], 0, 0, 0);
            acc[1][t] = __builtin_amdgcn_mfma_f32_32x32x16_f16(a[1][ai], bb, acc[1][t], 0, 0, 0);
            __builtin_amdgcn_sched_barrier(0);
        };
        auto rb = [&](auto tc) { read_b(xs_next, tc); __builtin_amdgcn_sched_barrier(0); };
        auto ra = [&](int ot) { an[ot][0] = aq[ot * 32]; an[ot][1] = aq[2 * OT + ot * 32]; __builtin_amdgcn_sched_barrier(0); };
        using std::integral_constant;
        __builtin_amdgcn_sched_barrier(0);
        mm(0, 0); dma_w(0, ks + 2, wbuf); __builtin_amdgcn_sched_barrier(0);
        mm(0, 1); dma_w(1, ks + 2, wbuf); __builtin_amdgcn_sched_barrier(0);
        mm(0, 2); rb(integral_constant<int, 0>{});
        mm(1, 0); ra(0); mm(1, 1); ra(1); mm(1, 2); rb(integral_constant<int, 1>{});
        mm(2, 0); dma_x(0, ks + 3, xs_fill); __builtin_amdgcn_sched_barrier(0);
        mm(2, 1); dma_x(1, ks + 3, xs_fill); __builtin_amdgcn_sched_barrier(0);
        mm(2, 2); rb(integral_constant<int, 2>{});
        mm(3, 0); mm(3, 1); mm(3, 2); rb(integral_constant<int, 3>{});
        ROREG_WAIT_FRAGS("s_waitcnt vmcnt(2) lgkmcnt(0)\n\ts_barrier");
    };
    dma_x(0, 0, 0); dma_x(1, 0, 0); dma_x(0, 1, 1); dma_x(1, 1, 1); dma_x(0, 2, 2); dma_x(1, 2, 2);
    dma_w(0, 0, 0); dma_w(1, 0, 0); dma_w(0, 1, 1); dma_w(1, 1, 1);
    asm volatile("s_waitcnt vmcnt(0)\n\ts_barrier" ::: "memory");
    read_a(0, aA);
    read_b(0u, std::integral_constant<int, 0>{}); read_b(0u, std::integral_constant<int, 1>{});
    read_b(0u, std::integral_constant<int, 2>{}); read_b(0u, std::integral_constant<int, 3>{});
    ROREG_WAIT_FRAGS("s_waitcnt lgkmcnt(0)\n\ts_barrier");
    int cur = 0;
    for (int ks = 0; ks < nsteps; ks += 2) {
        const int n1 = cur == 2 ? 0 : cur + 1, n2 = n1 == 2 ? 0 : n1 + 1;
        step(ks, 0, (unsigned)(n1 * XSTAGE), cur, aA, aB);
        step(ks + 1, 1, (unsigned)(n2 * XSTAGE), n1, aB, aA);
        cur = n2;
    }
    asm volatile("s_waitcnt vmcnt(0)\n\ts_barrier" ::: "memory");
#undef ROREG_WAIT_FRAGS
    gemm_split_epilogue<2, 4, COLS_PAIRED>(p, irr, mt, n0, wo, ncol_wave, acc, smem);
}

template <int N, class F> __device__ __forceinline__ void static_for(F &&f);

typedef float f32x4_t __attribute__((ext_vector_type(4)));
struct Epi16Pre {
    float osc[4];
    float u, v;
};
__device__ __forceinline__ Epi16Pre gemm_split_epilogue16_request(const GemmSplitDescs &p, int irr, int mt, int n0, int wb) {
    constexpr int OT = 256;
    const int tid = threadIdx.x, rl = tid & 31;
    const int N = p.N[irr], M = p.M[irr], dirr = kIrrDim[irr];
    const int ncol = n0 + wb * 128 + 4 * rl;
    Epi16Pre e;
    const f32x4_t xb = ncol < N ? *reinterpret_cast<const f32x4_t *>(p.xbound + column_keypoint(ncol, dirr)) : f32x4_t{0.f, 0.f, 0.f, 0.f};
#pragma unroll
    for (int i = 0; i < 4; ++i) e.osc[i] = xb[i];
    e.u = 0.f; e.v = 0.f;
    if (p.out_bound != nullptr && tid < OT) {
        const int m = mt * OT + tid;
        if (m < M) { e.u = p.nb_u[m % p.O]; e.v = p.nb_v[m % p.O]; }
    }
    return e;
}
__device__ __forceinline__ void gemm_split_epilogue16_scales(const GemmSplitDescs &p, Epi16Pre &e, bool col_ok) {
#pragma unroll
// ... 899 lines not shown
                    }
#pragma unroll
                    for (int q = 0; q < 8; ++q)
                        if (lane < p.Lout) ob[(size_t)(g8 * 8 + q) * ostep] = lane < p.Lvalid ? tv[q] : 0.f;
                }
            } else {
                for (int bl = 0; bl < 32 && b0 + bl < B; ++bl)
                    if (lane < p.Lout) {
                        float tv = tb[bl * 65 + lane];
                        if (rs_late && lane < ROREG_G) tv += ld_sp(p.r_spatial, ((size_t)(b0 + bl) * C + c) * ROREG_G + lane);
                        p.out_spatial[((size_t)(b0 + bl) * C + c) * p.Lout + lane] = lane < p.Lvalid ? tv : 0.f;
                    }
            }
            asm volatile("s_waitcnt lgkmcnt(0)" ::: "memory");
            if (p.out_rowmax) {
                wmax = fmaxf(wmax, __shfl_xor(wmax, 32));
                atomicMax(reinterpret_cast<unsigned *>(p.out_rowmax) + bb, __float_as_uint(valid ? wmax : 0.f));
            }
        }
        if (!OUT_SPATIAL) {
            f32x16 o[2];
#pragma unroll
            for (int t = 0; t < 2; ++t)
#pragma unroll
                for (int r = 0; r < 16; ++r) o[t][r] = 0.f;
            if constexpr (SPLIT == 3) {
#pragma unroll
                for (int st = 0; st < 4; ++st) {
                    float x8[8];
#pragma unroll
                    for (int e = 0; e < 8; ++e) x8[e] = v[st >> 1][8 * (st & 1) + e];
                    bf16x8 b[3];
                    split3(x8, b[0], b[1], b[2]);
                    o[0] = table_mma(sA2s + ((st * 2 + 0) * 3) * 64 + lane, b, o[0]);
                    o[1] = table_mma(sA2s + ((st * 2 + 1) * 3) * 64 + lane, b, o[1]);
                }
            } else if constexpr (SPLIT == 2) {
                float mx = 0.f;
#pragma unroll
                for (int t = 0; t < 2; ++t)
#pragma unroll
                    for (int r = 0; r < 16; ++r) mx = fmaxf(mx, fabsf(v[t][r]));
                float xsc, osc;
                column_scale(mx, xsc, osc);
#pragma unroll
                for (int st = 0; st < 4; ++st) {
                    float x8[8];
#pragma unroll
                    for (int e = 0; e < 8; ++e) x8[e] = v[st >> 1][8 * (st & 1) + e];
                    f16x8 bh, bl;
                    split2(x8, xsc, bh, bl);
                    const f16x8 b[2] = {bh, bl};
                    o[0] = table_mma(sA2h + ((st * 2 + 0) * 2) * 64 + lane, b, o[0]);
                    o[1] = table_mma(sA2h + ((st * 2 + 1) * 2) * 64 + lane, b, o[1]);
                }
                if constexpr (PACK_OUT) {
                    const float psc = osc * ldexpf(1.f, bound_exp(cv[NCV]));
#pragma unroll
                    for (int t = 0; t < 2; ++t)
#pragma unroll
                        for (int r = 0; r < 16; ++r) {
                            const float x = o[t][r] * psc;
                            const _Float16 h1 = (_Float16)x;
                            const _Float16 l1 = (_Float16)(x - (float)h1);
                            o[t][r] = __uint_as_float((unsigned)__builtin_bit_cast(unsigned short, h1) | ((unsigned)__builtin_bit_cast(unsigned short, l1) << 16));
                        }
                } else {
#pragma unroll
                    for (int t = 0; t < 2; ++t)
#pragma unroll
                        for (int r = 0; r < 16; ++r) o[t][r] *= osc;
                }
            } else {
#pragma unroll
                for (int t = 0; t < 2; ++t)
#pragma unroll
                    for (int r = 0; r < 16; ++r) {
                        const int s = t * 16 + r;
                        o[0] = __builtin_amdgcn_mfma_f32_32x32x2f32(sA2[(s * 2 + 0) * 64 + lane], v[t][r], o[0], 0, 0, 0);
                        o[1] = __builtin_amdgcn_mfma_f32_32x32x2f32(sA2[(s * 2 + 1) * 64 + lane], v[t][r], o[1], 0, 0, 0);
                    }
            }
            if constexpr (OUT_ROWS) {
#pragma unroll
                for (int t = 0; t < 2; ++t)
#pragma unroll
                    for (int r = 0; r < 16; ++r) {
                        const int qq = h ? kPS.qb[t * 16 + r] : kPS.qa[t * 16 + r];
                        if (qq < ROREG_G) tb[jn * 65 + qq] = o[t][r];
                    }
                asm volatile("s_waitcnt lgkmcnt(0)" ::: "memory");
                const int b0 = tbi * 32;
                if (b0 + 32 <= B) {
                    float *ob = p.out_spatial + ((size_t)b0 * C + c) * ROREG_G + lane;
                    const size_t ostep = (size_t)C * ROREG_G;
#pragma unroll
                    for (int g8 = 0; g8 < 4; ++g8) {
                        float tv[8];
#pragma unroll
                        for (int q = 0; q < 8; ++q) tv[q] = tb[(g8 * 8 + q) * 65 + lane];
#pragma unroll
                        for (int q = 0; q < 8; ++q)
                            if (lane < ROREG_G) ob[(size_t)(g8 * 8 + q) * ostep] = tv[q];
                    }
                } else {
                    for (int bl = 0; bl < 32 && b0 + bl < B; ++bl)
                        if (lane < ROREG_G) p.out_spatial[((size_t)(b0 + bl) * C + c) * ROREG_G + lane] = tb[bl * 65 + lane];
                }
                asm volatile("s_waitcnt lgkmcnt(0)" ::: "memory");
            } else if (PACK_OUT && p.out_planes) {
                const int tb = tbi;
                const unsigned sel = (jn & 16) ? 0x07060302u : 0x05040100u;
                static_for<32>([&](auto ic) {
                    constexpr int S = decltype(ic)::value, t = S / 16, r = S % 16;
                    const unsigned own = __float_as_uint(o[t][r]);
                    const auto pr = __builtin_amdgcn_permlane16_swap(own, own, false, false);
                    const unsigned word = __builtin_amdgcn_perm(pr[1], pr[0], sel);
                    unsigned *dst = reinterpret_cast<unsigned *>(const_cast<char *>(slot_ptr(ic, p.Xout, c, tb)));
                    if (kPS.kind[S] != 2 || h == 0) __builtin_nontemporal_store(word, dst);
                });
            } else {
                const int tb = tbi;
                static_for<32>([&](auto ic) {
                    constexpr int S = decltype(ic)::value, t = S / 16, r = S % 16;
                    float *dst = reinterpret_cast<float *>(const_cast<char *>(slot_ptr(ic, p.Xout, c, tb)));
                    if (kPS.kind[S] != 2 || h == 0) __builtin_nontemporal_store(o[t][r], dst);
                });
            }
        }
    };
    if (wave_global < n_tiles) {
        const int last = wave_global + ((n_tiles - 1 - wave_global) / n_waves) * n_waves;
        float cb[NCV + 1];
        GDesc da{0u, 0u, 0}, db{0u, 0u, 0};
        if constexpr (GATHER) {
            da = load_desc(wave_global);
            db = load_desc(min(wave_global + n_waves, last));
            load_rows_gathered(wave_global, da, cn);
        } else {
            load_coefs(wave_global, cn);
        }
        __builtin_amdgcn_s_waitcnt(0x0F70);
        for (int tile = wave_global; tile <= last; tile += 2 * n_waves) {
            const int t1 = min(tile + n_waves, last), t2 = min(tile + 2 * n_waves, last), t3 = min(tile + 3 * n_waves, last);
            process(tile, t1, cn, cb, t2, db, da);
            process(t1, t2, cb, cn, t3, da, db);
        }
    }
}

#undef OFF_OF
#undef OFF_Q

float *g_A1 = nullptr, *g_A2 = nullptr;
uint16_t *g_A1s = nullptr, *g_A2s = nullptr, *g_A1h = nullptr, *g_A2h = nullptr;
int g_f_exp = 0;

}

extern "C" int roreg_set_fourier_tables(const float *F_host ) {
    ROREG_REQUIRE(F_host, "roreg_set_fourier_tables: null table");
    static float A1[30 * 2 * 64], A2[32 * 2 * 64];
    for (int s = 0; s < 30; ++s)
        for (int tile = 0; tile < 2; ++tile)
            for (int lane = 0; lane < 64; ++lane) {
                const int qq = 2 * s + (lane >> 5), g = tile * 32 + (lane & 31);
                A1[(s * 2 + tile) * 64 + lane] = g < 60 ? F_host[qq * 60 + g] : 0.f;
            }
    for (int t = 0; t < 2; ++t)
        for (int r = 0; r < 16; ++r)
            for (int tile = 0; tile < 2; ++tile)
                for (int lane = 0; lane < 64; ++lane) {
                    const int qq = slot_out_q(tile * 32 + (lane & 31)), g = cd_row32(r, lane >> 5, t * 32);
                    A2[((t * 16 + r) * 2 + tile) * 64 + lane] = (qq < 60 && g < 60) ? F_host[qq * 60 + g] : 0.f;
                }
    if (!g_A1) {
        if (hipMalloc(&g_A1, sizeof(A1)) != hipSuccess || hipMalloc(&g_A2, sizeof(A2)) != hipSuccess) {
            roreg::set_error("roreg_set_fourier_tables: hipMalloc failed");
            return 1;
        }
    }
    if (hipMemcpy(g_A1, A1, sizeof(A1), hipMemcpyHostToDevice) != hipSuccess || hipMemcpy(g_A2, A2, sizeof(A2), hipMemcpyHostToDevice) != hipSuccess) {
        roreg::set_error("roreg_set_fourier_tables: hipMemcpy failed");
        return 1;
    }
    static uint16_t A1s[4 * 2 * 3 * 64 * 8], A2s[4 * 2 * 3 * 64 * 8];
    auto split3_host = [](float x, uint16_t out[3]) {
        float rem = x;
        for (int sp = 0; sp < 3; ++sp) {
            uint32_t u; memcpy(&u, &rem, 4);
            const uint32_t r = ((u >> 16) & 1u) + 0x7fffu;
            const uint16_t hi = (uint16_t)((u + r) >> 16);
            out[sp] = hi;
            const uint32_t back = (uint32_t)hi << 16;
            float v; memcpy(&v, &back, 4);
            rem = rem - v;
        }
    };
    for (int st = 0; st < 4; ++st)
        for (int tile = 0; tile < 2; ++tile)
            for (int lane = 0; lane < 64; ++lane)
                for (int e = 0; e < 8; ++e) {
                    const int j = lane & 31, h = lane >> 5;
                    const int q1 = 16 * st + 8 * h + e, g1 = tile * 32 + j;
                    const float f1 = (q1 < 60 && g1 < 60) ? F_host[q1 * 60 + g1] : 0.f;
                    const int r = 8 * (st & 1) + e, q2 = slot_out_q(tile * 32 + j), g2 = cd_row32(r, h, 32 * (st >> 1));
                    const float f2 = (q2 < 60 && g2 < 60) ? F_host[q2 * 60 + g2] : 0.f;
                    uint16_t p1[3], p2[3];
                    split3_host(f1, p1); split3_host(f2, p2);
                    for (int sp = 0; sp < 3; ++sp) {
                        const size_t at = ((((size_t)st * 2 + tile) * 3 + sp) * 64 + lane) * 8 + e;
                        A1s[at] = p1[sp]; A2s[at] = p2[sp];
                    }
                }
    if (!g_A1s) {
        if (hipMalloc(&g_A1s, sizeof(A1s)) != hipSuccess || hipMalloc(&g_A2s, sizeof(A2s)) != hipSuccess) {
            roreg::set_error("roreg_set_fourier_tables: hipMalloc failed");
            return 1;
        }
    }
    if (hipMemcpy(g_A1s, A1s, sizeof(A1s), hipMemcpyHostToDevice) != hipSuccess || hipMemcpy(g_A2s, A2s, sizeof(A2s), hipMemcpyHostToDevice) != hipSuccess) {
        roreg::set_error("roreg_set_fourier_tables: hipMemcpy failed");
        return 1;
    }
    static uint16_t A1h[4 * 2 * 2 * 64 * 8], A2h[4 * 2 * 2 * 64 * 8];
    float fmx = 0.f;
    for (int i = 0; i < 3600; ++i) fmx = std::max(fmx, std::fabs(F_host[i]));
    int fex = 0;
    (void)std::frexp(fmx, &fex);
    g_f_exp = fmx > 0.f ? 14 - fex : 0;
    auto f2h = [](float x) -> uint16_t {
        _Float16 hv = (_Float16)x;
        uint16_t b; memcpy(&b, &hv, 2);
        return b;
    };
    auto h2f = [](uint16_t b) -> float { _Float16 hv; memcpy(&hv, &b, 2); return (float)hv; };
    for (int st = 0; st < 4; ++st)
        for (int tile = 0; tile < 2; ++tile)
            for (int lane = 0; lane < 64; ++lane)
                for (int e = 0; e < 8; ++e) {
                    const int j = lane & 31, h = lane >> 5;
                    const int q1 = 16 * st + 8 * h + e, g1 = tile * 32 + j;
                    const float f1 = (q1 < 60 && g1 < 60) ? std::ldexp(F_host[q1 * 60 + g1], g_f_exp) : 0.f;
                    const int r = 8 * (st & 1) + e, q2 = slot_out_q(tile * 32 + j), g2 = cd_row32(r, h, 32 * (st >> 1));
                    const float f2 = (q2 < 60 && g2 < 60) ? std::ldexp(F_host[q2 * 60 + g2], g_f_exp) : 0.f;
                    const uint16_t h1 = f2h(f1), h2 = f2h(f2);
                    const size_t hi_at = ((((size_t)st * 2 + tile) * 2 + 0) * 64 + lane) * 8 + e, lo_at = hi_at + 64 * 8;
                    A1h[hi_at] = h1; A1h[lo_at] = f2h(f1 - h2f(h1));
                    A2h[hi_at] = h2; A2h[lo_at] = f2h(f2 - h2f(h2));
                }
    if (!g_A1h) {
        if (hipMalloc(&g_A1h, sizeof(A1h)) != hipSuccess || hipMalloc(&g_A2h, sizeof(A2h)) != hipSuccess) {
            roreg::set_error("roreg_set_fourier_tables: hipMalloc failed");
            return 1;
        }
    }
    if (hipMemcpy(g_A1h, A1h, sizeof(A1h), hipMemcpyHostToDevice) != hipSuccess || hipMemcpy(g_A2h, A2h, sizeof(A2h), hipMemcpyHostToDevice) != hipSuccess) {
        roreg::set_error("roreg_set_fourier_tables: hipMemcpy failed");
        return 1;
    }
    return 0;
}

extern "C" size_t roreg_irrep_gemm_tiles_m(int O, int B, int tile_m, int32_t *tiles_host);
extern "C" size_t roreg_irrep_gemm_tiles(int O, int B, int32_t *tiles_host ) { return roreg_irrep_gemm_tiles_m(O, B, 128, tiles_host); }

extern "C" size_t roreg_irrep_gemm_tiles_m(int O, int B, int tile_m , int32_t *tiles_host) {
    static const int dims[5] = {1, 3, 3, 4, 5};
    struct Block { int r, mg, ng, cost; };
    std::vector<Block> blocks;
    for (int r = 4; r >= 0; --r) {
        const int d = dims[r];
        const int mts = round_up(d * O, tile_m) / tile_m, nts = (d * B + 255) / 256;
        for (int ng = 0; ng * 8 < nts; ++ng)
            for (int mg = 0; mg * 8 < mts; ++mg) {
                const int a = std::min(8, mts - mg * 8), b = std::min(8, nts - ng * 8);
                blocks.push_back({r, mg, ng, a * b * d});
            }
    }
    std::stable_sort(blocks.begin(), blocks.end(), [](const Block &x, const Block &y) { return x.cost > y.cost; });
    std::vector<std::vector<int>> stream(8);
    long long load[8] = {0, 0, 0, 0, 0, 0, 0, 0};
    for (const Block &bk : blocks) {
        int k = 0;
        for (int q = 1; q < 8; ++q)
            if (load[q] < load[k]) k = q;
        load[k] += bk.cost;
        const int d = dims[bk.r];
        const int mts = round_up(d * O, tile_m) / tile_m, nts = (d * B + 255) / 256;
        for (int nt = bk.ng * 8; nt < std::min(nts, bk.ng * 8 + 8); ++nt)
            for (int mt = bk.mg * 8; mt < std::min(mts, bk.mg * 8 + 8); ++mt) {
                stream[k].push_back(bk.r); stream[k].push_back(mt); stream[k].push_back(nt);
            }
    }
    size_t longest = 0;
    for (int k = 0; k < 8; ++k) longest = std::max(longest, stream[k].size() / 3);
    const size_t n = longest * 8;
    if (tiles_host)
        for (size_t i = 0; i < longest; ++i)
            for (int k = 0; k < 8; ++k) {
                int32_t *t = tiles_host + (i * 8 + k) * 3;
                if (i * 3 < stream[k].size()) { t[0] = stream[k][i * 3]; t[1] = stream[k][i * 3 + 1]; t[2] = stream[k][i * 3 + 2]; }
                else { t[0] = -1; t[1] = 0; t[2] = 0; }
            }
    return n;
}

extern "C" int roreg_irrep_gemm(const float *const *X, float *const *Out, const float *const *Add, const float *const *Wpack, int C, int O, int B,
                                const int32_t *tiles_dev, int n_tiles, void *stream) {
    ROREG_REQUIRE(X && Out && Wpack && tiles_dev && C > 0 && O > 0 && B > 0 && n_tiles > 0, "roreg_irrep_gemm: bad arguments");
    ROREG_REQUIRE(C % 32 == 0, "roreg_irrep_gemm: C must be a multiple of 32 (got %d)", C);
    ROREG_REQUIRE(B % 4 == 0, "roreg_irrep_gemm: B must be a multiple of 4 (got %d); pad the keypoint batch", B);
    static const int dims[5] = {1, 3, 3, 4, 5};
    GemmDescs p;
    for (int r = 0; r < 5; ++r) {
        p.X[r] = X[r]; p.Out[r] = Out[r]; p.Add[r] = Add ? Add[r] : nullptr; p.W[r] = reinterpret_cast<const float4 *>(Wpack[r]);
        p.K[r] = dims[r] * C; p.M[r] = dims[r] * O; p.Mpad[r] = round_up(dims[r] * O, 128); p.N[r] = dims[r] * B;
    }
    constexpr int CT = 32;
    const size_t lds = 2 * CT * 256 * sizeof(float);
    return roreg::launch_lds("roreg_irrep_gemm", irrep_gemm_kernel<CT>, dim3(n_tiles), dim3(256), lds, roreg::as_stream(stream), p, tiles_dev);
}

struct GemmSwitch {
    const char *env;
    int dflt, hi;
    std::atomic<int> v{-1};
    int get() {
        int x = v.load(std::memory_order_relaxed);
        if (x < 0) {
            const char *e = getenv(env);
            x = e && e[0] >= '0' && e[0] <= '0' + hi ? e[0] - '0' : dflt;
            v.store(x, std::memory_order_relaxed);
        }
        return x;
    }
    int set(int on) {
        const int prev = get();
        if (on >= 0 && on <= hi) v.store(on, std::memory_order_relaxed);
        return prev;
    }
};
static GemmSwitch g_gemm_persist{"ROREG_GEMM_PERSIST", 0, 2};
static GemmSwitch g_gemm_thin{"ROREG_GEMM_THIN", 1, 1};
extern "C" int roreg_gemm_persistent(int on) { return g_gemm_persist.set(on); }
extern "C" int roreg_gemm_thin(int on) { return g_gemm_thin.set(on); }
static int gemm_cu_count() {
    static const int n = [] {
        int dev = 0, cus = 0;
        if (hipGetDevice(&dev) != hipSuccess || hipDeviceGetAttribute(&cus, hipDeviceAttributeMultiprocessorCount, dev) != hipSuccess || cus <= 0) cus = 256;
        return cus;
    }();
    return n;
}
template <int NP, int WO>
static int launch_gemm_split(const char *what, const float *const *X, float *const *Out, const float *const *Add, const void *const *Wsplit,
                             const float *xbound, int w_exp, const float *nb_u, const float *nb_v, float *out_bound, int C, int O, int B,
                             const int32_t *tiles_dev, int n_tiles, void *stream, int x_planes = 0) {
    static const int dims[5] = {1, 3, 3, 4, 5};
    GemmSplitDescs p;
    for (int r = 0; r < 5; ++r) {
        p.X[r] = X[r]; p.Out[r] = Out[r]; p.Add[r] = Add ? Add[r] : nullptr; p.W[r] = Wsplit[r];
        p.K[r] = dims[r] * C; p.M[r] = dims[r] * O; p.Mpad[r] = round_up(dims[r] * O, 128); p.N[r] = dims[r] * B;
        if (WO == 4 && p.Mpad[r] % 256 != 0) { roreg::set_error("%s: tile_m = 256 needs O %% 256 == 0 (got %d)", what, O); return 2; }
    }
    p.xbound = xbound; p.w_exp = w_exp; p.nb_u = nb_u; p.nb_v = nb_v; p.out_bound = out_bound; p.O = O;
    if constexpr (NP == 2) {
        if (!x_planes && !Add && (O == 32 || (C == 32 && O % 32 == 0 && O <= 512)) && g_gemm_thin.get()) {
            int wgs = 0;
            for (int r = 0; r < 5; ++r) { const int tc = C == 32 ? thin_tile_cols<false>(r) : thin_tile_cols<true>(r); wgs += (p.N[r] + tc - 1) / tc; }
            if (C == 32) hipLaunchKernelGGL(irrep_gemm_thin_k_kernel, dim3(wgs), dim3(512), 0, roreg::as_stream(stream), p);
            else hipLaunchKernelGGL(irrep_gemm_thin_m_kernel, dim3(wgs), dim3(256), 0, roreg::as_stream(stream), p);
            hipError_t e2 = hipGetLastError();
            if (e2 != hipSuccess) { roreg::set_error("%s: launch failed: %s", what, hipGetErrorString(e2)); return 1; }
            return 0;
        }
    }
    auto launch = [&](auto kern, int wgs, int threads, size_t lds, auto... more) {
        return roreg::launch_lds(what, kern, dim3(wgs), dim3(threads), lds, roreg::as_stream(stream), p, tiles_dev, more...);
    };
    constexpr int CT = 32;
    const bool big = (long long)C * O == 256ll * 512;
    if (x_planes) {
        if constexpr (NP == 2 && WO == 4) {
            if (x_planes != 2) return launch(big ? irrep_gemm_xdma_kernel<1> : irrep_gemm_xdma_kernel<0>, n_tiles, 512, 3 * (2 * 16 * 256 * 2) + 2 * (2 * 2 * 256) * 16);
            const size_t lds16 = (size_t)(6 + 4) * 16384;
            const int form = g_gemm_persist.get();
            if (form == 2)
                return launch(big ? irrep_gemm_xdma16h_kernel<1> : irrep_gemm_xdma16h_kernel<0>, 2 * n_tiles, 256, (size_t)6 * 8192 + 2 * 16384);
            if (form == 1) {
                static const int ra = [] { const char *v = getenv("ROREG_GEMM_PERSIST_RA"); return v ? atoi(v) : 2; }();
                auto kp = ra == 0 ? (big ? irrep_gemm_xdma16p_kernel<1, 0> : irrep_gemm_xdma16p_kernel<0, 0>)
                        : ra == 4 ? (big ? irrep_gemm_xdma16p_kernel<1, 4> : irrep_gemm_xdma16p_kernel<0, 4>)
                                  : (big ? irrep_gemm_xdma16p_kernel<1, 2> : irrep_gemm_xdma16p_kernel<0, 2>);
                const int wgs = std::min(n_tiles, std::max(8, gemm_cu_count() / 8 * 8));
                return launch(kp, wgs, 512, lds16, n_tiles / 8);
            }
            return launch(big ? irrep_gemm_xdma16_kernel<1> : irrep_gemm_xdma16_kernel<0>, n_tiles, 512, lds16);
        } else {
            roreg::set_error("%s: the half-block layout needs the fp16 x 2 kernel with tile_m = 256", what);
            return 2;
        }
    }
    static const int pipe = [] { const char *e = getenv("ROREG_GEMM_PIPE"); return e ? atoi(e) : 1; }();
    auto kern = big ? irrep_gemm_split_kernel<CT, NP, WO, 1> : irrep_gemm_split_kernel<CT, NP, WO, 0>;
    if constexpr (NP == 2) { if (pipe == 1) kern = big ? irrep_gemm_split_kernel<CT, NP, WO, 1, 1> : irrep_gemm_split_kernel<CT, NP, WO, 0, 1>; }
    return launch(kern, n_tiles, WO * 128, 2 * (NP * 2 * 256 + NP * (WO * 64) * 2) * 16);
}

extern "C" int roreg_irrep_gemm_split(const float *const *X, float *const *Out, const float *const *Add, const void *const *Wsplit, int C, int O, int B,
                                      const int32_t *tiles_dev, int n_tiles, void *stream) {
    ROREG_REQUIRE(X && Out && Wsplit && tiles_dev && C > 0 && O > 0 && B > 0 && n_tiles > 0, "roreg_irrep_gemm_split: bad arguments");
    ROREG_REQUIRE(C % 32 == 0 && B % 4 == 0, "roreg_irrep_gemm_split: C %% 32 and B %% 4 must be 0 (got %d, %d)", C, B);
    return launch_gemm_split<3, 2>("roreg_irrep_gemm_split", X, Out, Add, Wsplit, nullptr, 0, nullptr, nullptr, nullptr, C, O, B, tiles_dev, n_tiles, stream);
}

extern "C" int roreg_irrep_gemm_f16x2(const float *const *X, float *const *Out, const float *const *Add, const void *const *Wsplit2,
                                      const float *x_bound_dev, int w_exp, const float *next_u_dev, const float *next_v_dev, float *out_bound_dev,
                                      int C, int O, int B, const int32_t *tiles_dev, int n_tiles, int tile_m, int x_planes, void *stream) {
    ROREG_REQUIRE(X && Out && Wsplit2 && tiles_dev && C > 0 && O > 0 && B > 0 && n_tiles > 0, "roreg_irrep_gemm_f16x2: bad arguments");
    ROREG_REQUIRE(!x_planes || tile_m == 256, "roreg_irrep_gemm_f16x2: x_planes needs tile_m = 256");
    ROREG_REQUIRE(C % 32 == 0 && B % 32 == 0, "roreg_irrep_gemm_f16x2: C %% 32 and B %% 32 must be 0 (got %d, %d)", C, B);
    ROREG_REQUIRE(x_bound_dev, "roreg_irrep_gemm_f16x2: x_bound_dev (the per-keypoint bound the activations were split under) is required");
    ROREG_REQUIRE(!out_bound_dev || (next_u_dev && next_v_dev), "roreg_irrep_gemm_f16x2: out_bound_dev needs next_u_dev / next_v_dev");
    ROREG_REQUIRE(tile_m == 128 || tile_m == 256, "roreg_irrep_gemm_f16x2: tile_m must be 128 or 256 (the value the tile list was built with)");
    if (tile_m == 256)
        return launch_gemm_split<2, 4>("roreg_irrep_gemm_f16x2", X, Out, Add, Wsplit2, x_bound_dev, w_exp, next_u_dev, next_v_dev, out_bound_dev, C, O, B,
                                       tiles_dev, n_tiles, stream, x_planes);
    return launch_gemm_split<2, 2>("roreg_irrep_gemm_f16x2", X, Out, Add, Wsplit2, x_bound_dev, w_exp, next_u_dev, next_v_dev, out_bound_dev, C, O, B,
                                   tiles_dev, n_tiles, stream);
}

__global__ __launch_bounds__(256) void row_bound_kernel(const float *__restrict__ x, int x_bf16, const float *__restrict__ bn_scale,
                                                        const float *__restrict__ bn_shift, float *__restrict__ bound, int B, int Bp, int C) {
    const int b = blockIdx.x * 4 + (threadIdx.x >> 6), lane = threadIdx.x & 63;
    if (b >= Bp) return;
    float mx = 0.f;
    if (b < B) {
        const size_t row = (size_t)b * C * ROREG_G;
        for (int i = lane; i < C * ROREG_G; i += 64) {
            float v = x_bf16 ? __uint_as_float((unsigned)reinterpret_cast<const unsigned short *>(x)[row + i] << 16) : x[row + i];
            if (bn_scale) { const int c = i / ROREG_G; v = fmaxf(fmaf(v, bn_scale[c], bn_shift[c]), 0.f); }
            mx = fmaxf(mx, fabsf(v));
        }
#pragma unroll
        for (int o = 32; o > 0; o >>= 1) mx = fmaxf(mx, __shfl_xor(mx, o));
    }
    if (lane == 0) bound[b] = mx * 7.7536f;
}

__global__ __launch_bounds__(256) void row_bound_roles_kernel(const float *__restrict__ x, int x_bf16, float *__restrict__ bound, int B, int Bp,
                                                              const float *__restrict__ role_scale, const float *__restrict__ role_shift,
                                                              float *__restrict__ role_out) {
    const int b = blockIdx.x * 4 + (threadIdx.x >> 6), lane = threadIdx.x & 63;
    if (b >= Bp) return;
    float mx = 0.f, m1 = 0.f, m0 = 0.f;
    if (b < B) {
        const size_t row = (size_t)b * ROREG_F * ROREG_G;
        for (int i = lane; i < ROREG_F * ROREG_G; i += 64) {
            const float v = x_bf16 ? __uint_as_float((unsigned)reinterpret_cast<const unsigned short *>(x)[row + i] << 16) : x[row + i];
            const int c = i / ROREG_G;
            mx = fmaxf(mx, fabsf(v));
            m1 = fmaxf(m1, fmaxf(fmaf(v, role_scale[c], role_shift[c]), 0.f));
            m0 = fmaxf(m0, fmaxf(fmaf(v, role_scale[ROREG_F + c], role_shift[ROREG_F + c]), 0.f));
        }
#pragma unroll
        for (int o = 32; o > 0; o >>= 1) { mx = fmaxf(mx, __shfl_xor(mx, o)); m1 = fmaxf(m1, __shfl_xor(m1, o)); m0 = fmaxf(m0, __shfl_xor(m0, o)); }
        if (lane == 0) { role_out[(size_t)b * 4] = m1; role_out[(size_t)b * 4 + 1] = m0; }
    }
    if (lane == 0) bound[b] = mx * 7.7536f;
}

extern "C" int roreg_row_bound_roles(const void *x_spatial, int x_bf16, float *bound_out, const float *role_scale, const float *role_shift, float *role_out,
                                     int B, void *stream) {
    ROREG_REQUIRE(x_spatial && bound_out && role_scale && role_shift && role_out && B > 0, "roreg_row_bound_roles: bad arguments");
    const int Bp = (B + 31) / 32 * 32;
    hipLaunchKernelGGL(row_bound_roles_kernel, dim3((Bp + 3) / 4), dim3(256), 0, roreg::as_stream(stream), reinterpret_cast<const float *>(x_spatial), x_bf16, bound_out,
                       B, Bp, role_scale, role_shift, role_out);
    ROREG_CHECK_LAUNCH("roreg_row_bound_roles");
    return 0;
}

extern "C" int roreg_row_bound(const void *x_spatial, int x_bf16, const float *bn_scale, const float *bn_shift, float *bound_out, int B, int C,
                               void *stream) {
    ROREG_REQUIRE(x_spatial && bound_out && B > 0 && C > 0, "roreg_row_bound: bad arguments");
    ROREG_REQUIRE((bn_scale == nullptr) == (bn_shift == nullptr), "roreg_row_bound: bn_scale and bn_shift go together");
    const int Bp = (B + 31) / 32 * 32;
    hipLaunchKernelGGL(row_bound_kernel, dim3((Bp + 3) / 4), dim3(256), 0, roreg::as_stream(stream), reinterpret_cast<const float *>(x_spatial), x_bf16, bn_scale, bn_shift,
                       bound_out, B, Bp, C);
    ROREG_CHECK_LAUNCH("roreg_row_bound");
    return 0;
}

template <void (*KERN)(NonlinParams)>
static void launch_ft(const NonlinParams &p, long long n_tiles, hipStream_t s) {
    static const int resident = [] {
        int per_cu = 0, dev = 0, cus = 256;
        if (hipOccupancyMaxActiveBlocksPerMultiprocessor(&per_cu, KERN, 256, 0) != hipSuccess || per_cu < 1) per_cu = 2;
        if (hipGetDevice(&dev) == hipSuccess) (void)hipDeviceGetAttribute(&cus, hipDeviceAttributeMultiprocessorCount, dev);
        return per_cu * cus;
    }();
    static const int rounds = [] { const char *e = getenv("ROREG_FT_ROUNDS"); const int r = e ? atoi(e) : 0; return r > 0 ? r : 4; }();
    const long long want = (n_tiles + 3) / 4, cap = (long long)resident * rounds;
    hipLaunchKernelGGL(KERN, dim3((unsigned)(want > cap ? cap : want)), dim3(256), 0, s, p);
}

extern "C" int roreg_ft_nonlin(const float *Xin, const float *x_spatial, const float *bias, const float *bias2,
                               const float *bn_scale, const float *bn_shift, const float *resid_spatial, float *Xout, float *out_spatial,
                               const int32_t *g_map, int Lout, int Lvalid, int B, int C, int split, const float *out_bound, float *out_rowmax,
                               int spatial_bf16, int out_planes, void *stream) {
    ROREG_REQUIRE(g_A1 && g_A2, "roreg_ft_nonlin: roreg_set_fourier_tables has not been called");
    ROREG_REQUIRE((Xin != nullptr) != (x_spatial != nullptr), "roreg_ft_nonlin: exactly one of Xin / x_spatial");
    ROREG_REQUIRE((Xout != nullptr) != (out_spatial != nullptr), "roreg_ft_nonlin: exactly one of Xout / out_spatial");
    ROREG_REQUIRE((bn_scale == nullptr) == (bn_shift == nullptr) && B > 0 && C > 0 && C <= 512, "roreg_ft_nonlin: bad arguments (C <= 512)");
    ROREG_REQUIRE((long long)60 * C * B < (1ll << 40), "roreg_ft_nonlin: tensor too large");
    ROREG_REQUIRE(!g_map || (Lout >= Lvalid && Lvalid > 0 && Lout <= 64), "roreg_ft_nonlin: bad Lout/Lvalid");
    NonlinParams p;
    memset(&p, 0, sizeof(p));
    p.Xin = Xin; p.Xout = Xout;
    p.x_spatial = x_spatial; p.r_spatial = resid_spatial; p.out_spatial = out_spatial;
    p.g_map = g_map; p.Lout = g_map ? Lout : ROREG_G; p.Lvalid = g_map ? Lvalid : ROREG_G;
    p.bias = bias; p.bias2 = bias2; p.bn_scale = bn_scale; p.bn_shift = bn_shift; p.A1 = g_A1; p.A2 = g_A2;
    p.A1s = reinterpret_cast<const bf16x8 *>(g_A1s); p.A2s = reinterpret_cast<const bf16x8 *>(g_A2s); p.out_bound = out_bound; p.out_rowmax = out_rowmax; p.x_bf16 = spatial_bf16;
    p.A1h = reinterpret_cast<const f16x8 *>(g_A1h); p.A2h = reinterpret_cast<const f16x8 *>(g_A2h); p.f_exp = g_f_exp;
    p.B = B; p.Bp = (B + 31) / 32 * 32; p.C = C; p.tiles_per_c = (B + 31) / 32;
    p.out_planes = out_planes;
    ROREG_REQUIRE((unsigned long long)C * p.Bp * 20ull < (1ull << 32), "roreg_ft_nonlin: C * round_up(B, 32) must stay below 2^32 / 20 (32-bit lane offsets)");
    ROREG_REQUIRE(!out_planes || (split == 2 && Xout), "roreg_ft_nonlin: out_planes is a layout of the fp16 x 2 coefficient output");
    const long long n_tiles = (long long)C * p.tiles_per_c;
    hipStream_t s = roreg::as_stream(stream);
    roreg::ProfScope prof(roreg::PROF_FT_NONLIN, s);
    const bool in_sp = x_spatial != nullptr, out_sp = out_spatial != nullptr;
    if (in_sp && out_sp) { roreg::set_error("roreg_ft_nonlin: spatial -> spatial is not a transform"); return 2; }
    ROREG_REQUIRE(split != 2 || out_sp || out_bound, "roreg_ft_nonlin: split = 2 writes the coefficients as fp16 hi/lo pairs and needs out_bound");
    ROREG_REQUIRE(!spatial_bf16 || in_sp || resid_spatial, "roreg_ft_nonlin: spatial_bf16 refers to x_spatial / resid_spatial");
    ROREG_REQUIRE(!out_rowmax || out_sp, "roreg_ft_nonlin: out_rowmax goes with a group-domain output");
    ROREG_REQUIRE(split >= 0 && split <= 2, "roreg_ft_nonlin: split must be 0 (f32 MFMA), 1 (bf16 x 3) or 2 (fp16 x 2)");
    if (split == 2) {
        if (in_sp) launch_ft<ft_nonlin_kernel<true, false, 2, 4, 1>>(p, n_tiles, s);
        else if (!out_sp) launch_ft<ft_nonlin_kernel<false, false, 2, 4, 1>>(p, n_tiles, s);
        else launch_ft<ft_nonlin_kernel<false, true, 2, 4, 1>>(p, n_tiles, s);
    } else if (split == 1) {
        if (in_sp) launch_ft<ft_nonlin_kernel<true, false, 3, 4, 1>>(p, n_tiles, s);
        else if (!out_sp) launch_ft<ft_nonlin_kernel<false, false, 3, 4, 1>>(p, n_tiles, s);
        else launch_ft<ft_nonlin_kernel<false, true, 3, 4, 1>>(p, n_tiles, s);
    } else {
        if (in_sp) launch_ft<ft_nonlin_kernel<true, false, 0, 4, 1>>(p, n_tiles, s);
        else if (!out_sp) launch_ft<ft_nonlin_kernel<false, false, 0, 4, 1>>(p, n_tiles, s);
        else launch_ft<ft_nonlin_kernel<false, true, 0, 4, 1>>(p, n_tiles, s);
    }
    ROREG_CHECK_LAUNCH("roreg_ft_nonlin");
    return 0;
}

extern "C" int roreg_ft_nonlin_packed(const float *Xin, const float *bias, const float *bn_scale, const float *bn_shift, uint32_t *out_words,
                                      const int32_t *g_map, int Lout, int Lvalid, int B, int C, const float *out_bound, float *raw_col, int raw_g,
                                      void *stream) {
    ROREG_REQUIRE(g_A1 && g_A2, "roreg_ft_nonlin_packed: roreg_set_fourier_tables has not been called");
    ROREG_REQUIRE(Xin && out_words && out_bound && B > 0 && C > 0 && C <= 512 && (bn_scale == nullptr) == (bn_shift == nullptr), "roreg_ft_nonlin_packed: bad arguments");
    ROREG_REQUIRE(!g_map || (Lout >= Lvalid && Lvalid > 0 && Lout <= 64), "roreg_ft_nonlin_packed: bad Lout/Lvalid");
    ROREG_REQUIRE(!raw_col || (raw_g >= 0 && raw_g < ROREG_G), "roreg_ft_nonlin_packed: raw_g out of range");
    NonlinParams p;
    memset(&p, 0, sizeof(p));
    p.Xin = Xin; p.out_spatial = reinterpret_cast<float *>(out_words);
    p.g_map = g_map; p.Lout = g_map ? Lout : ROREG_G; p.Lvalid = g_map ? Lvalid : ROREG_G;
    p.bias = bias; p.bn_scale = bn_scale; p.bn_shift = bn_shift; p.A1 = g_A1; p.A2 = g_A2;
    p.A1s = reinterpret_cast<const bf16x8 *>(g_A1s); p.A2s = reinterpret_cast<const bf16x8 *>(g_A2s);
    p.A1h = reinterpret_cast<const f16x8 *>(g_A1h); p.A2h = reinterpret_cast<const f16x8 *>(g_A2h); p.f_exp = g_f_exp;
    p.out_bound = out_bound; p.sp_pack = 1; p.raw_col = raw_col; p.raw_g = raw_g;
    p.B = B; p.Bp = (B + 31) / 32 * 32; p.C = C; p.tiles_per_c = (B + 31) / 32;
    ROREG_REQUIRE((unsigned long long)C * p.Bp * 20ull < (1ull << 32), "roreg_ft_nonlin_packed: C * round_up(B, 32) must stay below 2^32 / 20 (32-bit lane offsets)");
    hipStream_t s = roreg::as_stream(stream);
    roreg::ProfScope prof(roreg::PROF_FT_NONLIN, s);
    launch_ft<ft_nonlin_kernel<false, true, 2, 4, 1>>(p, (long long)C * p.tiles_per_c, s);
    ROREG_CHECK_LAUNCH("roreg_ft_nonlin_packed");
    return 0;
}

extern "C" int roreg_ft_nonlin_gathered(const uint64_t *rows, const int64_t *dr, int feat_bf16, const float *bn_scale, const float *bn_shift, float *Xout,
                                        int B, const float *out_bound, int out_planes, void *stream) {
    ROREG_REQUIRE(g_A1 && g_A2, "roreg_ft_nonlin_gathered: roreg_set_fourier_tables has not been called");
    ROREG_REQUIRE(roreg::group_tables().ready, "roreg_ft_nonlin_gathered: group tables not set");
    ROREG_REQUIRE(rows && dr && Xout && out_bound && B > 0 && (bn_scale == nullptr) == (bn_shift == nullptr), "roreg_ft_nonlin_gathered: bad arguments");
    constexpr int C = 4 * ROREG_F;
    ROREG_REQUIRE((long long)60 * C * B < (1ll << 40), "roreg_ft_nonlin_gathered: tensor too large");
    NonlinParams p;
    memset(&p, 0, sizeof(p));
    p.Xout = Xout; p.Lout = ROREG_G; p.Lvalid = ROREG_G;
    p.bn_scale = bn_scale; p.bn_shift = bn_shift; p.A1 = g_A1; p.A2 = g_A2;
    p.A1s = reinterpret_cast<const bf16x8 *>(g_A1s); p.A2s = reinterpret_cast<const bf16x8 *>(g_A2s);
    p.A1h = reinterpret_cast<const f16x8 *>(g_A1h); p.A2h = reinterpret_cast<const f16x8 *>(g_A2h); p.f_exp = g_f_exp;
    p.out_bound = out_bound; p.x_bf16 = feat_bf16; p.out_planes = out_planes;
    p.g_rows = reinterpret_cast<const roreg::LtRow *>(rows); p.g_dr = dr; p.g_P8 = roreg::group_tables().P8;
    p.B = B; p.Bp = (B + 31) / 32 * 32; p.C = C; p.tiles_per_c = (B + 31) / 32;
    ROREG_REQUIRE((unsigned long long)C * p.Bp * 20ull < (1ull << 32), "roreg_ft_nonlin_gathered: 128 * round_up(B, 32) must stay below 2^32 / 20 (32-bit lane offsets)");
    hipStream_t s = roreg::as_stream(stream);
    roreg::ProfScope prof(roreg::PROF_FT_NONLIN, s);
    launch_ft<ft_nonlin_kernel<true, false, 2, 4, 1, false, true>>(p, (long long)C * p.tiles_per_c, s);
    ROREG_CHECK_LAUNCH("roreg_ft_nonlin_gathered");
    return 0;
}

extern "C" int roreg_feat_coefs(const void *x, int x_bf16, float *out, int B, int C, int split, void *stream) {
    if (B == 0) return 0;
    ROREG_REQUIRE(g_A1 && g_A2, "roreg_feat_coefs: roreg_set_fourier_tables has not been called");
    ROREG_REQUIRE(x && out && B > 0 && C > 0 && C <= 512 && split >= 0 && split <= 2, "roreg_feat_coefs: bad arguments");
    NonlinParams p;
    memset(&p, 0, sizeof(p));
    p.x_spatial = reinterpret_cast<const float *>(x); p.x_bf16 = x_bf16; p.out_spatial = out;
    p.Lout = ROREG_G; p.Lvalid = ROREG_G; p.A1 = g_A1; p.A2 = g_A2;
    p.A1s = reinterpret_cast<const bf16x8 *>(g_A1s); p.A2s = reinterpret_cast<const bf16x8 *>(g_A2s);
    p.A1h = reinterpret_cast<const f16x8 *>(g_A1h); p.A2h = reinterpret_cast<const f16x8 *>(g_A2h); p.f_exp = g_f_exp;
    p.B = B; p.Bp = (B + 31) / 32 * 32; p.C = C; p.tiles_per_c = (B + 31) / 32;
    const long long n_tiles = (long long)C * p.tiles_per_c;
    hipStream_t s = roreg::as_stream(stream);
    if (split == 2) launch_ft<ft_nonlin_kernel<true, false, 2, 4, 1, true>>(p, n_tiles, s);
    else if (split == 1) launch_ft<ft_nonlin_kernel<true, false, 3, 4, 1, true>>(p, n_tiles, s);
    else launch_ft<ft_nonlin_kernel<true, false, 0, 4, 1, true>>(p, n_tiles, s);
    ROREG_CHECK_LAUNCH("roreg_feat_coefs");
    return 0;
}
```

### roreg_amd/csrc/pointwise.hip

```cpp
#include "common.h"

#pragma clang fp contract(off)

namespace {

__device__ __forceinline__ float np_pairwise_sum(const float *a, int n) {
    float r[8];
#pragma unroll
    for (int j = 0; j < 8; ++j) r[j] = a[j];
    int i = 8;
    for (; i < n - (n % 8); i += 8) {
#pragma unroll
        for (int j = 0; j < 8; ++j) r[j] = __fadd_rn(r[j], a[i + j]);
    }
    float res = __fadd_rn(__fadd_rn(__fadd_rn(r[0], r[1]), __fadd_rn(r[2], r[3])),
                          __fadd_rn(__fadd_rn(r[4], r[5]), __fadd_rn(r[6], r[7])));
    for (; i < n; ++i) res = __fadd_rn(res, a[i]);
    return res;
}

__device__ __forceinline__ float clamp_min_norm(float n) { return n < 1e-4f ? 1e-4f : n; }

template <typename OT>
__global__ __launch_bounds__(256) void gf_finalize_kernel(const float *__restrict__ raw, void *__restrict__ eqv_v,
                                                          float *__restrict__ inv, int B) {
    const int lane = threadIdx.x & 63, w = threadIdx.x >> 6;
    const int b = blockIdx.x * 4 + w;
    if (b >= B) return;
    const float *src = raw + (size_t)b * (ROREG_F * ROREG_G);
    OT *dst = reinterpret_cast<OT *>(eqv_v) + (size_t)b * (ROREG_F * ROREG_G);
    const bool act = lane < ROREG_G;
    float v[ROREG_F];
    float n2 = 0.f;
#pragma unroll
    for (int f = 0; f < ROREG_F; ++f) {
        v[f] = act ? src[f * ROREG_G + lane] : 0.f;
        n2 += v[f] * v[f];
    }
    const float nrm = clamp_min_norm(sqrtf(n2));
    if (act) {
#pragma unroll
        for (int f = 0; f < ROREG_F; ++f) dst[f * ROREG_G + lane] = (OT)(v[f] / nrm);
    }
    if (inv) {
        float mine = 0.f, m2 = 0.f;
#pragma unroll
        for (int f = 0; f < ROREG_F; ++f) {
            float s = v[f];
#pragma unroll
            for (int o = 32; o > 0; o >>= 1) s += __shfl_xor(s, o);
            s *= (1.0f / ROREG_G);
            m2 += s * s;
            if (lane == f) mine = s;
        }
        const float mn = clamp_min_norm(sqrtf(m2));
        if (lane < ROREG_F) inv[(size_t)b * ROREG_F + lane] = mine / mn;
    }
}

template <typename FT, bool ROLES = false>
__global__ __launch_bounds__(256) void inv_descriptor_kernel(const void *__restrict__ eqv_v, float *__restrict__ inv, int N,
                                                             const float *__restrict__ role_scale = nullptr, const float *__restrict__ role_shift = nullptr,
                                                             float *__restrict__ role_out = nullptr) {
    __shared__ float tile[4][ROREG_F * ROREG_G + 32];
    const int lane = threadIdx.x & 63, w = threadIdx.x >> 6;
    const int n = blockIdx.x * 4 + w;
    const bool live = n < N;
    if (live) {
        const FT *src = reinterpret_cast<const FT *>(eqv_v) + (size_t)n * (ROREG_F * ROREG_G);
        if constexpr (ROLES) {
            float m1 = 0.f, m0 = 0.f, v[ROREG_F];
#pragma unroll
            for (int c = 0; c < ROREG_F; ++c) v[c] = lane < ROREG_G ? (float)src[c * ROREG_G + lane] : 0.f;
#pragma unroll
            for (int c = 0; c < ROREG_F; ++c) {
                if (lane < ROREG_G) {
                    tile[w][c * ROREG_G + lane] = v[c];
                    m1 = fmaxf(m1, fmaxf(fmaf(v[c], role_scale[c], role_shift[c]), 0.f));
                    m0 = fmaxf(m0, fmaxf(fmaf(v[c], role_scale[ROREG_F + c], role_shift[ROREG_F + c]), 0.f));
                }
            }
#pragma unroll
            for (int o = 32; o > 0; o >>= 1) { m1 = fmaxf(m1, __shfl_xor(m1, o)); m0 = fmaxf(m0, __shfl_xor(m0, o)); }
            if (lane == 0) { role_out[(size_t)n * 4 + 2] = m1; role_out[(size_t)n * 4 + 3] = m0; }
        } else
        for (int i = lane; i < ROREG_F * ROREG_G; i += 64) tile[w][i] = (float)src[i];
    }
    __syncthreads();
    if (!live) return;
    float m = 0.f;
    if (lane < ROREG_F) {
        float row[ROREG_G];
#pragma unroll
        for (int g = 0; g < ROREG_G; ++g) row[g] = tile[w][lane * ROREG_G + g];
        m = (float)((double)np_pairwise_sum(row, ROREG_G) / 60.0);
    }
    float sq[ROREG_F];
#pragma unroll
    for (int f = 0; f < ROREG_F; ++f) {
        const float mf = __shfl(m, f);
        sq[f] = __fmul_rn(mf, mf);
    }
    const float nrm = __fadd_rn(sqrtf(np_pairwise_sum(sq, ROREG_F)), 1e-5f);
    if (lane < ROREG_F) inv[(size_t)n * ROREG_F + lane] = __fdiv_rn(m, nrm);
}

__global__ __launch_bounds__(256) void det_score_kernel(const float *__restrict__ enc, const uint8_t *__restrict__ P8,
                                                        float *__restrict__ scores, int B) {
    __shared__ float fn[4][16 * ROREG_G];
    __shared__ uint8_t Pl[ROREG_G * ROREG_G];
    for (int i = threadIdx.x; i < ROREG_G * ROREG_G; i += 256) Pl[i] = P8[i];
    __syncthreads();
    const int lane = threadIdx.x & 63, w = threadIdx.x >> 6;
    const int b = blockIdx.x * 4 + w;
    const bool live = b < B;
    const float *src = enc + (size_t)(live ? b : 0) * (16 * ROREG_G);
    const bool act = lane < ROREG_G;
    float v[16];
    float n2 = 0.f;
#pragma unroll
    for (int f = 0; f < 16; ++f) {
        v[f] = act ? src[f * ROREG_G + lane] : 0.f;
        n2 += v[f] * v[f];
    }
    const float rn = sqrtf(n2);
    if (act) {
#pragma unroll
        for (int f = 0; f < 16; ++f) fn[w][f * ROREG_G + lane] = v[f] / rn;
    }
    __syncthreads();
    if (!live) return;
    float c = 0.f;
    if (act) {
        float s[16];
#pragma unroll
        for (int f = 0; f < 16; ++f) s[f] = 0.f;
        for (int g = 0; g < ROREG_G; ++g) {
            const int pg = Pl[lane * ROREG_G + g];
#pragma unroll
            for (int f = 0; f < 16; ++f) s[f] += fn[w][f * ROREG_G + pg] * fn[w][f * ROREG_G + g];
        }
#pragma unroll
        for (int f = 0; f < 16; ++f) c += s[f];
    }
    float sum = act ? c : 0.f;
#pragma unroll
    for (int o = 32; o > 0; o >>= 1) sum += __shfl_xor(sum, o);
    const float mean = sum * (1.0f / ROREG_G);
    float d = act ? (c - mean) : 0.f;
    float ss = d * d;
#pragma unroll
    for (int o = 32; o > 0; o >>= 1) ss += __shfl_xor(ss, o);
    if (lane == 0) scores[b] = sqrtf(ss / (ROREG_G - 1));
}

template <typename FT>
__device__ __forceinline__ void et_gather_body(const void *__restrict__ before0_v, const void *__restrict__ before1_v,
                                               const void *__restrict__ after0_v, const void *__restrict__ after1_v, size_t r0, size_t r1,
                                               int a, const int32_t *__restrict__ P, float *__restrict__ dst,
                                               const float *__restrict__ bn_scale = nullptr, const float *__restrict__ bn_shift = nullptr,
                                               float *__restrict__ bound_row = nullptr) {
    __shared__ int perm[ROREG_G];
    __shared__ float red[4];
    if (threadIdx.x < ROREG_G) perm[threadIdx.x] = P[a * ROREG_G + threadIdx.x];
    __syncthreads();
    const FT *s_b1 = reinterpret_cast<const FT *>(before1_v) + r1 * (ROREG_F * ROREG_G), *s_b0 = reinterpret_cast<const FT *>(before0_v) + r0 * (ROREG_F * ROREG_G);
    const FT *s_a1 = reinterpret_cast<const FT *>(after1_v) + r1 * (ROREG_F * ROREG_G), *s_a0 = reinterpret_cast<const FT *>(after0_v) + r0 * (ROREG_F * ROREG_G);
    float mx = 0.f;
    for (int i = threadIdx.x; i < ROREG_F * ROREG_G; i += 256) {
        const int c = i / ROREG_G, g = i - c * ROREG_G;
        const int pg = c * ROREG_G + perm[g];
        const float v0 = (float)s_b1[pg], v1 = (float)s_b0[i], v2 = (float)s_a1[pg], v3 = (float)s_a0[i];
        __builtin_nontemporal_store(v0, dst + i);
        __builtin_nontemporal_store(v1, dst + ROREG_F * ROREG_G + i);
// ... 332 lines not shown
```

### roreg_amd/csrc/primitives.h

```cpp
#pragma once
#include <hip/hip_runtime.h>

typedef float f32x16 __attribute__((ext_vector_type(16)));
typedef __bf16 bf16x8 __attribute__((ext_vector_type(8)));
typedef _Float16 f16x8 __attribute__((ext_vector_type(8)));

template <class T>
constexpr T round_up(T x, int a) { return (x + a - 1) / a * a; }

__device__ __forceinline__ int bound_exp(float mx) {
    int e = 0;
    if (mx > 0.f && mx < __builtin_inff()) { int ex; (void)frexpf(mx, &ex); e = 14 - ex; }
    return e > 100 ? 100 : (e < -100 ? -100 : e);
}

__device__ __forceinline__ void split3(const float (&v)[8], bf16x8 &b1, bf16x8 &b2, bf16x8 &b3) {
#pragma unroll
    for (int e = 0; e < 8; ++e) {
        const __bf16 h1 = (__bf16)v[e];
        const float r1 = v[e] - (float)h1;
        const __bf16 h2 = (__bf16)r1;
        const float r2 = r1 - (float)h2;
        b1[e] = h1; b2[e] = h2; b3[e] = (__bf16)r2;
    }
}

__device__ __forceinline__ void split2(const float (&v)[8], float scale, f16x8 &hi, f16x8 &lo) {
#pragma unroll
    for (int e = 0; e < 8; ++e) {
        const float x = v[e] * scale;
        const _Float16 h1 = (_Float16)x;
        hi[e] = h1; lo[e] = (_Float16)(x - (float)h1);
    }
}

__device__ __forceinline__ f32x16 mfma_32x32x16(const bf16x8 &a, const bf16x8 &b, f32x16 c) { return __builtin_amdgcn_mfma_f32_32x32x16_bf16(a, b, c, 0, 0, 0); }
__device__ __forceinline__ f32x16 mfma_32x32x16(const f16x8 &a, const f16x8 &b, f32x16 c) { return __builtin_amdgcn_mfma_f32_32x32x16_f16(a, b, c, 0, 0, 0); }
template <int NP, class F>
__device__ __forceinline__ f32x16 split_mma(const F (&a)[NP], const F (&b)[NP], f32x16 c) {
    static_assert(NP == 2 || NP == 3, "fp16 x 2 or bf16 x 3");
    if constexpr (NP == 3) {
        c = mfma_32x32x16(a[2], b[0], c);
        c = mfma_32x32x16(a[1], b[1], c);
        c = mfma_32x32x16(a[0], b[2], c);
    }
    c = mfma_32x32x16(a[1], b[0], c);
    c = mfma_32x32x16(a[0], b[1], c);
    c = mfma_32x32x16(a[0], b[0], c);
    return c;
}
template <int NP, class F>
__device__ __forceinline__ void split_mma_pair(const F (&a)[2][NP], const F (&b)[NP], f32x16 &c0, f32x16 &c1) {
    static_assert(NP == 2 || NP == 3, "fp16 x 2 or bf16 x 3");
    f32x16 x = c0, y = c1;
    const F b1 = b[0], b2 = b[1];
    if constexpr (NP == 3) {
        const F b3 = b[2];
        x = mfma_32x32x16(a[0][2], b1, x); y = mfma_32x32x16(a[1][2], b1, y);
        x = mfma_32x32x16(a[0][1], b2, x); y = mfma_32x32x16(a[1][1], b2, y);
        x = mfma_32x32x16(a[0][0], b3, x); y = mfma_32x32x16(a[1][0], b3, y);
    }
    x = mfma_32x32x16(a[0][1], b1, x); y = mfma_32x32x16(a[1][1], b1, y);
    x = mfma_32x32x16(a[0][0], b2, x); y = mfma_32x32x16(a[1][0], b2, y);
    x = mfma_32x32x16(a[0][0], b1, x); y = mfma_32x32x16(a[1][0], b1, y);
    c0 = x; c1 = y;
}

__host__ __device__ constexpr int cd_row32(int r, int h, int first = 0) { return first + (r & 3) + 8 * (r >> 2) + 4 * h; }

__device__ __forceinline__ double wave_sum(double v) {
#pragma unroll
    for (int o = 32; o > 0; o >>= 1) v += __shfl_xor(v, o);
    return v;
}

__device__ __forceinline__ int seg_of(const int *__restrict__ off, int n_seg, int r) {
    int lo = 0, hi = n_seg - 1;
    while (lo < hi) {
        const int mid = (lo + hi + 1) >> 1;
        if (off[mid] <= r) lo = mid; else hi = mid - 1;
    }
    return lo;
}

template <int CTRL, int ROW_MASK>
__device__ __forceinline__ float dpp_mov(float x) {
    return __builtin_bit_cast(float, __builtin_amdgcn_update_dpp(__builtin_bit_cast(int, x), __builtin_bit_cast(int, x), CTRL, ROW_MASK, 0xf, false));
}
```

### roreg_amd/engine.py

```python
from dataclasses import dataclass, field

import os
import time

import numpy as np
import torch

from . import hip


@dataclass
class CloudState:
    before: torch.Tensor
    eqv: torch.Tensor = None
    eqv_ft: torch.Tensor = None
    inv: torch.Tensor = None
    role: torch.Tensor = None
    role_bn: object = None
    keys: torch.Tensor = None
    det: np.ndarray = None
    keys_host: np.ndarray = None
    nms: dict = field(default_factory=dict)
    points: torch.Tensor = None
    points_box: np.ndarray = None
# ... 113 lines not shown
                if done is not None:
                    done.synchronize()
                t_landed = time.perf_counter()
                a = host.numpy() if torch.is_tensor(host) else host
                hip.write_npy_files([path], [a], n_threads=1)
                self.log.append((os.path.basename(os.path.dirname(path)), a.nbytes, t_landed, time.perf_counter()))
                del a, host
                if buf is not None:
                    hip.pinned_pool.release(buf)
            except Exception as e:
                self.error = e

    def save(self, rel, a):
        self.save_path(f'{self.dir}/{rel}.npy', a)

    def save_path(self, path, a):
        if not torch.is_tensor(a):
            self.q.put((path, np.ascontiguousarray(a), None, None))
            return
        ready = torch.cuda.Event(); ready.record()
        host, buf = self._pinned(a)
        with torch.cuda.stream(self.stream):
            self.stream.wait_event(ready)
            host.copy_(a, non_blocking=True)
            done = torch.cuda.Event(); done.record(self.stream)
        a.record_stream(self.stream)
        self.q.put((path, host, done, buf))

    @staticmethod
    def _pinned(a):
        nbytes = a.numel() * a.element_size()
        buf = hip.pinned_pool.acquire(nbytes)
        return buf[:nbytes].view(a.dtype).reshape(a.shape), buf

    def submit(self, fn):
        self.q.put(fn)

    def save_many_host(self, rels, arrays):
        if not len(rels):
            return
        paths = [f'{self.dir}/{r}.npy' for r in rels]

        def write():
            t0 = time.perf_counter()
            hip.write_npy_files(paths, arrays, n_threads=2)
            self.log.append((os.path.basename(os.path.dirname(paths[0])), sum(a.nbytes for a in arrays), t0, time.perf_counter()))
        self.q.put(write)

    def save_many(self, rels, tensors):
        if not tensors:
            return
        shapes = [tuple(t.shape) for t in tensors]
        flat = torch.cat([t.reshape(-1) for t in tensors])
        ready = torch.cuda.Event(); ready.record()
        host, buf = self._pinned(flat)
        with torch.cuda.stream(self.stream):
            self.stream.wait_event(ready)
            host.copy_(flat, non_blocking=True)
            done = torch.cuda.Event(); done.record(self.stream)
        flat.record_stream(self.stream)
        self.q.put(([f'{self.dir}/{r}.npy' for r in rels], host, done, shapes, buf))

    def close(self):
        if self._creator is not None:
            self._cq.put(None)
            self._creator.join()
            self._creator = None
        for _ in self.threads:
            self.q.put(None)
        for t in self.threads:
            t.join()
        if self.error is not None:
            raise self.error


class _LazySeq:

    def __init__(self, container, ids):
        self.container, self.ids = container, ids

    def __len__(self):
        return len(self.ids)

    def __getitem__(self, q):
        return self.container[self.ids[q]]


def even_groups(sizes, cap):
    sizes = [int(x) for x in sizes]
    if not sizes:
        return []
    n_groups = max(1, -(-sum(sizes) // int(cap)))
    target = sum(sizes) / n_groups
    out, i = [], 0
    while i < len(sizes):
        j, pts = i, 0
        while j < len(sizes) and (j == i or (pts + sizes[j] <= cap and pts + sizes[j] / 2 <= target)):
            pts += sizes[j]; j += 1
        out.append((i, j)); i = j
    return out


class RegistrationEngine:
    def __init__(self, cfg, gf_net, et_net, rd_net=None, rm_net=None):
        self.cfg = cfg
        self.gf = gf_net
        self.et = et_net
        self.rd = rd_net
        self.rm = rm_net
        hip.ensure_tables()
        self.rm_max_points = int(os.environ.get('ROREG_RM_MAX_POINTS', 260000))
        self.feat_dtype = torch.bfloat16 if getattr(cfg, 'dtype', 'fp32') == 'bf16' else torch.float32
        self.extract_rows = int(os.environ.get('ROREG_EXTRACT_ROWS', 65536))
        self.lt_rows = int(os.environ.get('ROREG_LT_ROWS', 131072))
        self.phase_ms = None
        self._side = None

    def _mark(self, name, t0):
        if self.phase_ms is None:
            return t0
        import time
        torch.cuda.synchronize()
        t1 = time.perf_counter()
        self.phase_ms[name] = self.phase_ms.get(name, 0.0) + 1e3 * (t1 - t0)
        return t1

    def set_descriptor_dtype(self, name):
        if name not in ('fp32', 'bf16'):
            raise ValueError("descriptor dtype must be 'fp32' or 'bf16'")
        self.feat_dtype = torch.bfloat16 if name == 'bf16' else torch.float32

    def set_gemm_mode(self, mode):
        from .network.gf_fourier import FourierGF
        if mode == 'split':
            mode = 'bf16x3'
        if mode not in hip.GEMM_MODES:
            raise ValueError(f'gemm mode must be one of {hip.GEMM_MODES}')
        net = self.gf.PartI_net
        if net._fourier is None:
            object.__setattr__(net, '_fourier', FourierGF(net))
        net._fourier.gemm = mode
        if self.et is not None:
            self.et.gemm = mode
        if self.rd is not None:
            if self.rd._fourier is None:
                from .network.gf_fourier import FourierRD
                object.__setattr__(self.rd, '_fourier', FourierRD(self.rd.eqv_encoder[0]))
            self.rd._fourier.gemm = mode

    def extract(self, feats, keys):
        x = feats if torch.is_tensor(feats) else torch.from_numpy(np.ascontiguousarray(feats, np.float32))
        x = x.to('cuda', torch.float32).to(self.feat_dtype).contiguous()
        roles = self._role_request(x.shape[0])
        with torch.no_grad():
            eqv = self.gf.PartI_net(x, want_inv=False, out_dtype=self.feat_dtype, roles=roles)['eqv']
        k = keys if torch.is_tensor(keys) else torch.from_numpy(np.ascontiguousarray(keys, np.float64))
        return CloudState(before=x, eqv=eqv, eqv_ft=hip.feat_coefs(eqv), inv=hip.inv_descriptor(eqv, roles=roles), keys=k.to('cuda', torch.float64).contiguous(),
                          role=roles[2] if roles else None, role_bn=roles[0] if roles else None)

    def _role_request(self, n):
        bn = self.et.conv_init_bn() if self.et is not None else None
        if bn is None or n == 0:
            return None
        return bn[0], bn[1], torch.empty((n, 4), dtype=torch.float32, device='cuda')

    def extract_many(self, feats_list, keys_list, max_rows=None, on_batch=None):
        max_rows = self.extract_rows if max_rows is None else max_rows
        def on_device(f):
            if torch.is_tensor(f) and f.is_cuda and f.dtype == self.feat_dtype:
                return f
            if torch.is_tensor(f) and not f.is_cuda and f.is_pinned():
                return f.to('cuda', non_blocking=True).to(torch.float32).to(self.feat_dtype)
            return (f if torch.is_tensor(f) else torch.from_numpy(np.ascontiguousarray(f, np.float32))).to('cuda', torch.float32).to(self.feat_dtype)
        out = []
        i = 0
        n_all = len(keys_list)
        fetched = {}
        def get(q):
            if q not in fetched:
                fetched[q] = feats_list[q]
            return fetched[q]
        while i < n_all:
            j, rows = i, 0
            while j < n_all and (j == i or rows + int(get(j).shape[0]) <= max_rows):
                rows += int(get(j).shape[0]); j += 1
            xs = [on_device(fetched.pop(q)) for q in range(i, j)]
            adjacent = all(xs[q].is_contiguous() and xs[q].dtype == xs[0].dtype and xs[q].untyped_storage().data_ptr() == xs[0].untyped_storage().data_ptr() and
                           xs[q].data_ptr() == xs[q - 1].data_ptr() + xs[q - 1].numel() * xs[q - 1].element_size() for q in range(1, j - i)) and xs[0].is_contiguous()
            if j - i == 1:
                xcat = xs[0].contiguous()
            elif adjacent:
                xcat = torch.as_strided(xs[0], (rows, 32, 60), (1920, 60, 1))
            else:
                xcat = torch.cat(xs, 0)
            roles = self._role_request(rows)
            with torch.no_grad():
                eqv = self.gf.PartI_net(xcat, want_inv=False, out_dtype=self.feat_dtype, roles=roles)['eqv']
            inv = hip.inv_descriptor(eqv, roles=roles)
            eft = hip.feat_coefs(eqv)
            on_host = [q for q in range(i, j) if not (torch.is_tensor(keys_list[q]) and keys_list[q].is_cuda)]
            k_dev = {}
            if on_host:
                hk = [np.ascontiguousarray(keys_list[q].numpy() if torch.is_tensor(keys_list[q]) else keys_list[q], np.float64).reshape(-1, 3) for q in on_host]
                flat_k, ko = hip.upload(np.concatenate(hk)), 0
                for q, h in zip(on_host, hk):
                    k_dev[q] = flat_k[ko:ko + h.shape[0]]; ko += h.shape[0]
            o = 0
            for q in range(i, j):
                n = xs[q - i].shape[0]
                k = k_dev[q] if q in k_dev else keys_list[q]
                if not (k.dtype == torch.float64 and k.is_contiguous()):
                    k = k.to(torch.float64).contiguous()
                out.append(CloudState(before=xcat[o:o + n], eqv=eqv[o:o + n], eqv_ft=eft[o:o + n], inv=inv[o:o + n], keys=k,
                                      role=roles[2][o:o + n] if roles else None, role_bn=roles[0] if roles else None))
                o += n
            if on_batch is not None:
                on_batch(range(i, j), out[i:j])
            i = j
        return out

    def alloc_eqv(self, before):
        return torch.empty((int(before.shape[0]), 32, 60), dtype=self.feat_dtype, device='cuda')

    def cloud_from_eqv(self, before, eqv, keys):
        x = before if torch.is_tensor(before) else torch.from_numpy(np.ascontiguousarray(before, np.float32))
        if not (x.is_cuda and x.dtype == self.feat_dtype):
            x = x.to('cuda', torch.float32).to(self.feat_dtype)
        k = keys if torch.is_tensor(keys) else torch.from_numpy(np.ascontiguousarray(keys, np.float64))
        if not (k.is_cuda and k.dtype == torch.float64 and k.is_contiguous()):
            k = k.to('cuda', torch.float64).contiguous()
        eqv = eqv.to('cuda', self.feat_dtype).contiguous()
        x = x.contiguous()
        bn = self.et.conv_init_bn() if self.et is not None else None
        return CloudState(before=x, eqv=eqv, eqv_ft=hip.feat_coefs(eqv), inv=hip.inv_descriptor(eqv), keys=k,
                          role=hip.role_max(x, eqv, bn) if bn is not None and x.shape[0] else None, role_bn=bn[0] if bn is not None else None)

    def detect(self, cloud):
        self.detect_many([cloud])
        return cloud.det

    @staticmethod
    def _drive(gen):
        try:
            req = next(gen)
            while True:
                req = gen.send([t.cpu().numpy() for t in req])
        except StopIteration as fin:
            return fin.value

    def detect_many(self, clouds):
        return self._drive(self._detect_steps(clouds))

    def _detect_steps(self, clouds):
        todo = [c for c in clouds if c.det is None]
        if not todo:
            return
        raw, i = [], 0
        with torch.no_grad():
            while i < len(todo):
                j, rows = i, 0
                while j < len(todo) and (j == i or rows + todo[j].eqv.shape[0] <= 65536):
                    rows += todo[j].eqv.shape[0]; j += 1
                x = todo[i].eqv if j - i == 1 else torch.cat([c.eqv for c in todo[i:j]])
                raw.append(self.rd({'feats': x})['scores'])
                i = j
        flat = (yield [torch.cat(raw)])[0]
        offs = np.cumsum([0] + [c.eqv.shape[0] for c in todo])

        def rank(q):
            s = flat[offs[q]:offs[q + 1]].copy()
            a = np.argsort(s)
            s[a] = np.arange(s.shape[0]) / s.shape[0]
            return s
        for c, s in zip(todo, _host_pool().map(rank, range(len(todo)))):
            c.det = s

    def nms_many(self, clouds, keynum):
        return self._drive(self._nms_steps(clouds, keynum))

    def _nms_steps(self, clouds, keynum):
        from .test.matcher import NMS_sample
        sampler = NMS_sample(keynum, 5)
        todo = [c for c in clouds if keynum not in c.nms]
        need = []
        for c in todo:
            if c.keys.shape[0] < keynum:
                c.nms[keynum] = np.arange(c.keys.shape[0])
            else:
                need.append(c)
        if need:
            seg = hip.Segments([c.keys.shape[0] for c in need])
            pts = torch.cat([c.keys.float() for c in need]).contiguous()
            flat = (yield [hip.knn_search_seg(pts, seg, 5)])[0]
            picks = _host_pool().map(lambda q: sampler.sample_from_neighbours(need[q].det, flat[seg.host[q]:seg.host[q + 1]]), range(len(need)))
            for c, pick in zip(need, picks):
                c.nms[keynum] = pick

    def sample(self, c0, c1, keynum, seed=None):
        rng = np.random if seed is None else np.random.RandomState(int(seed) % (2 ** 32))
        n0, n1 = c0.before.shape[0], c1.before.shape[0]
        if self.cfg.RD:
            self.nms_many([c0, c1], keynum)
            s0, s1 = c0.nms[keynum], c1.nms[keynum]
        else:
            s0 = np.arange(n0); s1 = np.arange(n1)
            rng.shuffle(s0); rng.shuffle(s1)
            s0 = s0[0:keynum]; s1 = s1[0:keynum]
        return s0, s1

    @staticmethod
    def _match_rm_finish(s0, s1, m0, sc0):
        valid = np.nonzero(m0 >= 0)[0]
        if valid.shape[0] < 3:
            return np.array([[np.asarray(s0, np.int64)[1], np.asarray(s1, np.int64)[1]]], np.int64), np.ones(1, np.float32)
        return np.stack([np.asarray(s0, np.int64)[m0[valid]], np.asarray(s1, np.int64)[valid]], 1), sc0[valid]

    def match_rm_many(self, jobs, max_points=None):
        return self._drive(self._match_rm_steps(jobs, max_points))

    def _match_rm_steps(self, jobs, max_points=None):
        if not jobs:
            return []
        max_points = self.rm_max_points if max_points is None else max_points
        longest = max(max(len(s0), len(s1)) for _, _, s0, s1 in jobs)
        ot_mode = (2 if hip.OT_COOP else 1) if hip.OT_RECOMPUTE else 0
        per_pair = 4 * hip.lib().roreg_sinkhorn_batch3_workspace_size(1, longest, longest, longest, longest, ot_mode, 0) + 60_000 * 2 * longest
        max_points = max(longest, min(max_points, int(0.25 * torch.cuda.mem_get_info()[0] / per_pair) * longest))
        flat = np.concatenate([np.ascontiguousarray(x, np.int64) for _, _, s0, s1 in jobs for x in (s0, s1)])
        flat_dev = hip.upload(flat)
        rows, o = [], 0
        for _, _, s0, s1 in jobs:
            rows.append((flat_dev[o:o + len(s0)], flat_dev[o + len(s0):o + len(s0) + len(s1)])); o += len(s0) + len(s1)
        issued = []
        for i, j in even_groups([max(len(s0), len(s1)) for _, _, s0, s1 in jobs], max_points):
            seg_s = hip.Segments([len(jobs[q][3]) for q in range(i, j)]); seg_t = hip.Segments([len(jobs[q][2]) for q in range(i, j)])
            se = torch.empty((seg_s.total, 32, 60), dtype=self.feat_dtype, device='cuda'); te = torch.empty((seg_t.total, 32, 60), dtype=self.feat_dtype, device='cuda')
            sk = torch.empty((seg_s.total, 3), dtype=torch.float64, device='cuda'); tk = torch.empty((seg_t.total, 3), dtype=torch.float64, device='cuda')
            gf, gk = [], []
            for q in range(i, j):
                c0, c1 = jobs[q][0], jobs[q][1]
                d0, d1 = rows[q]
                a, b = seg_s.host[q - i], seg_t.host[q - i]
                gf += [(c1.eqv, d1, se[a:a + d1.shape[0]]), (c0.eqv, d0, te[b:b + d0.shape[0]])]
                gk += [(c1.keys, d1, sk[a:a + d1.shape[0]]), (c0.keys, d0, tk[b:b + d0.shape[0]])]
            hip.gather_rows_batch(gf); hip.gather_rows_batch(gk)
            with torch.no_grad():
                issued += self.rm.match_stacked(se.float(), te.float(), sk.float(), tk.float(), seg_s, seg_t)
        m0_all, sc_all = yield [torch.cat([m for m, _ in issued]), torch.cat([s for _, s in issued])]
        out, o = [], 0
        for (c0, c1, s0, s1), (m, _) in zip(jobs, issued):
            n = int(m.shape[0])
            out.append(self._match_rm_finish(s0, s1, m0_all[o:o + n], sc_all[o:o + n])); o += n
# ... 454 lines not shown
```

### roreg_amd/network/gf_fourier.py

```python
import numpy as np
import torch

from .. import hip
from ..fourier import group_fourier, DIMS
from .ops import _version_key


def _fold_bn(bn):
    scale = bn.weight.detach().float().cpu() / torch.sqrt(bn.running_var.detach().float().cpu() + bn.eps)
    shift = bn.bias.detach().float().cpu() - bn.running_mean.detach().float().cpu() * scale
    return scale.cuda().contiguous(), shift.cuda().contiguous()


class _Layer:
    def __init__(self, conv):
        gf = group_fourier()
        W = conv.weight.detach().double().cpu().numpy()
        O, C = W.shape[0], W.shape[1]
        W = W.reshape(O, C, 13)
        self.C, self.O = C, O
        self.bias = conv.bias.detach().float().cuda().contiguous()
        self.wpack = []
        self.wsplit = []
        self.dense = []
        for ri, Wh in enumerate(gf.transform_weights(W)):
            d = DIMS[ri]
            Wm = np.ascontiguousarray(Wh.transpose(3, 0, 2, 1)).reshape(d * O, d * C)
            Mpad = (d * O + 127) // 128 * 128
            Wp = np.zeros((Mpad, d * C), np.float32)
            Wp[:d * O] = Wm.astype(np.float32)
            self.dense.append(Wp)
            self.wpack.append(hip.pack_conv_weights(torch.from_numpy(Wp).reshape(Mpad, d * C, 1)))
            self.wsplit.append(hip.bf16_split3_pack(Wp) if (d * C) % 16 == 0 else None)
        w_exp = hip.f16_scale_exp(max(float(np.abs(Wp).max()) for Wp in self.dense))
        self.wsplit2 = ([hip.f16_split2_pack(Wp, w_exp) for Wp in self.dense], w_exp) if all(Wp.shape[1] % 16 == 0 for Wp in self.dense) else None


class FourierGF:
    def __init__(self, net):
        self.net = net
        self._key = None
        self.gemm = hip.GEMM_MODE

    def _plan(self):
        key = _version_key(self.net)
        if self._key != key:
            res = self.net.SO3_Conv_layers[0]
            self.l_in = _Layer(self.net.Conv_in[0])
            self.l_1 = _Layer(res.comb_layer_in[2]); self.bn_1 = _fold_bn(res.comb_layer_in[0])
            self.l_2 = _Layer(res.comb_layer_out[2]); self.bn_2 = _fold_bn(res.comb_layer_out[0])
            self.l_out = _Layer(self.net.Conv_out.comb_layer[2]); self.bn_3 = _fold_bn(self.net.Conv_out.comb_layer[0])
            self._key = key

    def _plan_bounds(self):
        if getattr(self, '_nb_key', None) != self._key:
            self.nb_1 = hip.next_bound(self.bn_1, self.l_in.bias)
            self.nb_2 = hip.next_bound(self.bn_2, self.l_1.bias)
            self.nb_3 = hip.next_bound(self.bn_3, self.l_2.bias, self.l_in.bias)
            self._nb_key = self._key

    def forward_raw(self, x, roles=None):
        self._plan()
        hip.ensure_fourier()
        B = x.shape[0]
        sp = {'f32': False, 'bf16x3': True, 'f16x2': 'f16x2'}[self.gemm]
        if self.gemm == 'f16x2':
            self._plan_bounds()
            b0 = hip.row_bound(x, roles=roles)
            X0 = hip.ft_nonlin(B, 32, x_spatial=x, split=sp, out_bound=b0)
            T0, b1 = hip.irrep_gemm(X0, None, 32, 256, B, f16x2=self.l_in.wsplit2, x_bound=b0, next_bound=self.nb_1)
            del X0
            xd = hip.use_planes(512) and hip.use_planes(256)
            X1 = hip.ft_nonlin(B, 256, coef_in=T0, bias=self.l_in.bias, bn=self.bn_1, split=sp, out_bound=b1, planes=xd)
            T1, b2 = hip.irrep_gemm(X1, None, 256, 512, B, f16x2=self.l_1.wsplit2, x_bound=b1, next_bound=self.nb_2, x_planes=xd)
            del X1
            X2 = hip.ft_nonlin(B, 512, coef_in=T1, bias=self.l_1.bias, bn=self.bn_2, split=sp, out_bound=b2, planes=xd)
            del T1
            T2, b3 = hip.irrep_gemm(X2, None, 512, 256, B, f16x2=self.l_2.wsplit2, x_bound=b2, next_bound=self.nb_3, add=T0, x_planes=xd)
            del X2, T0
            X3 = hip.ft_nonlin(B, 256, coef_in=T2, bias=self.l_2.bias, bias2=self.l_in.bias, bn=self.bn_3, split=sp, out_bound=b3)
            del T2
            T3 = hip.irrep_gemm(X3, None, 256, 32, B, f16x2=self.l_out.wsplit2, x_bound=b3)
            return hip.ft_nonlin(B, 32, coef_in=T3, bias=self.l_out.bias, resid_spatial=x, spatial_out=True, split=sp)

        if roles is not None:
            hip.row_bound(x, roles=roles)

        def gemm(X, layer, C, O, add=None):
            return hip.irrep_gemm(X, layer.wpack, C, O, B, split=layer.wsplit if self.gemm == 'bf16x3' else None, add=add)

        def ft(C, **kw):
            return hip.ft_nonlin(B, C, split=sp, **kw)
        X0 = ft(32, x_spatial=x)
        T0 = gemm(X0, self.l_in, 32, 256)
        del X0
        X1 = ft(256, coef_in=T0, bias=self.l_in.bias, bn=self.bn_1)
        T1 = gemm(X1, self.l_1, 256, 512)
        del X1
        X2 = ft(512, coef_in=T1, bias=self.l_1.bias, bn=self.bn_2)
        del T1
        T2 = gemm(X2, self.l_2, 512, 256, add=T0)
        del X2, T0
        X3 = ft(256, coef_in=T2, bias=self.l_2.bias, bias2=self.l_in.bias, bn=self.bn_3)
        del T2
        T3 = gemm(X3, self.l_out, 256, 32)
        return ft(32, coef_in=T3, bias=self.l_out.bias, resid_spatial=x, spatial_out=True)


    def scale_headroom(self, x):
        self._plan(); self._plan_bounds()
        hip.ensure_fourier()
        B = x.shape[0]
        out = {}

        def report(name, bound, coefs_f32, C):
            actual = hip.pack_coefs_f16x2(coefs_f32, C, B)[1][:B]
            bits = torch.log2(bound[:B].double() / actual.double().clamp_min(1e-300))
            out[name] = {'min': round(float(bits.min()), 2), 'mean': round(float(bits.mean()), 2), 'max': round(float(bits.max()), 2)}
        b0 = hip.row_bound(x)
        report('gemm_32_256_input', b0, hip.ft_nonlin(B, 32, x_spatial=x, split=True), 32)
        X0 = hip.ft_nonlin(B, 32, x_spatial=x, split='f16x2', out_bound=b0)
        T0, b1 = hip.irrep_gemm(X0, None, 32, 256, B, f16x2=self.l_in.wsplit2, x_bound=b0, next_bound=self.nb_1)
        report('gemm_256_512_input', b1, hip.ft_nonlin(B, 256, coef_in=T0, bias=self.l_in.bias, bn=self.bn_1, split=True), 256)
        X1 = hip.ft_nonlin(B, 256, coef_in=T0, bias=self.l_in.bias, bn=self.bn_1, split='f16x2', out_bound=b1)
        T1, b2 = hip.irrep_gemm(X1, None, 256, 512, B, f16x2=self.l_1.wsplit2, x_bound=b1, next_bound=self.nb_2)
        report('gemm_512_256_input', b2, hip.ft_nonlin(B, 512, coef_in=T1, bias=self.l_1.bias, bn=self.bn_2, split=True), 512)
        X2 = hip.ft_nonlin(B, 512, coef_in=T1, bias=self.l_1.bias, bn=self.bn_2, split='f16x2', out_bound=b2)
        T2, b3 = hip.irrep_gemm(X2, None, 512, 256, B, f16x2=self.l_2.wsplit2, x_bound=b2, next_bound=self.nb_3, add=T0)
        report('gemm_256_32_input', b3, hip.ft_nonlin(B, 256, coef_in=T2, bias=self.l_2.bias, bias2=self.l_in.bias, bn=self.bn_3, split=True), 256)
        return out


class FourierRD:

    def __init__(self, block):
        self.block = block
        self._key = None
        self.gemm = hip.GEMM_MODE

    def _plan(self):
        key = _version_key(self.block)
        if self._key != key:
            b = self.block
            self.l_in = _Layer(b.comb_layer_in[2]); self.bn_in = _fold_bn(b.comb_layer_in[0])
            self.l_out = _Layer(b.comb_layer_out[2]); self.bn_out = _fold_bn(b.comb_layer_out[0])
            self.l_sc = _Layer(b.short_cut_layer[2]); self.bn_sc = _fold_bn(b.short_cut_layer[0])
            self._key = key

    def forward(self, x):
        self._plan()
        hip.ensure_fourier()
        B = x.shape[0]
        sp = {'f32': False, 'bf16x3': True, 'f16x2': 'f16x2'}[self.gemm]
        if self.gemm == 'f16x2':
            if getattr(self, '_nb_key', None) != self._key:
                self.nb_out = hip.next_bound(self.bn_out, self.l_in.bias)
                self._nb_key = self._key
            bs = hip.row_bound(x, bn=self.bn_sc)
            Xs = hip.ft_nonlin(B, 32, x_spatial=x, bn=self.bn_sc, split=sp, out_bound=bs)
            S = hip.irrep_gemm(Xs, None, self.l_sc.C, self.l_sc.O, B, f16x2=self.l_sc.wsplit2, x_bound=bs)
            del Xs
            ba = hip.row_bound(x, bn=self.bn_in)
            Xa = hip.ft_nonlin(B, 32, x_spatial=x, bn=self.bn_in, split=sp, out_bound=ba)
            T1, b1 = hip.irrep_gemm(Xa, None, self.l_in.C, self.l_in.O, B, f16x2=self.l_in.wsplit2, x_bound=ba, next_bound=self.nb_out)
            del Xa
            X1 = hip.ft_nonlin(B, 64, coef_in=T1, bias=self.l_in.bias, bn=self.bn_out, split=sp, out_bound=b1)
            del T1
            T2 = hip.irrep_gemm(X1, None, self.l_out.C, self.l_out.O, B, f16x2=self.l_out.wsplit2, x_bound=b1, add=S)
            del X1, S
            return hip.ft_nonlin(B, 16, coef_in=T2, bias=self.l_out.bias, bias2=self.l_sc.bias, spatial_out=True, split=sp)

        def gemm(X, layer, add=None):
            return hip.irrep_gemm(X, layer.wpack, layer.C, layer.O, B, split=layer.wsplit if self.gemm == 'bf16x3' else None, add=add)

        def ft(C, **kw):
            return hip.ft_nonlin(B, C, split=sp, **kw)
        Xs = ft(32, x_spatial=x, bn=self.bn_sc)
        S = gemm(Xs, self.l_sc)
        del Xs
        Xa = ft(32, x_spatial=x, bn=self.bn_in)
        T1 = gemm(Xa, self.l_in)
        del Xa
        X1 = ft(64, coef_in=T1, bias=self.l_in.bias, bn=self.bn_out)
        del T1
        T2 = gemm(X1, self.l_out, add=S)
        del X1, S
        return ft(16, coef_in=T2, bias=self.l_out.bias, bias2=self.l_sc.bias, spatial_out=True)
```

Measured before the change: 1101.

## Fuse extractor tail into per-keypoint row GEMM plus gf_finish kernel

Adds a row-layout variant of the thin Conv_out GEMM that writes per-keypoint [60,32] rows. A new gf_finish kernel consumes those rows and, per keypoint in one wave, applies the inverse Fourier transform on matrix cores, adds bias and residual, normalises, computes the invariant descriptor and role maxima, and does the forward transform for the feature coefficients. This replaces the four separate kernels ft_nonlin, gf_finalize, inv_descriptor and feat_coefs, cutting launches and global round trips. The fused path is on by default, is taken only for f16x2 mode with float32 features, and adds a fairly complex kernel with a high LDS footprint.

```diff
diff --git a/include/roreg_hip.h b/include/roreg_hip.h
--- a/include/roreg_hip.h
+++ b/include/roreg_hip.h
@@ -251,6 +251,10 @@
                            int x_planes , void *stream);
 int roreg_gemm_persistent(int on);
 int roreg_gemm_thin(int on);
+int roreg_irrep_gemm_f16x2_rows(const float *const *X, float *T3r, const void *const *Wsplit2, const float *x_bound_dev, int w_exp, int C, int B, void *stream);
+int roreg_gf_finish(const float *T3r, const float *x, const float *b_out, const float *role_scale , const float *role_shift ,
+                    float *eqv, float *inv, float *role_out , float *eqv_ft, int B, void *stream);
+int roreg_gf_finish_route(int on);
 int roreg_row_bound(const void *x_spatial, int x_bf16 , const float *bn_scale, const float *bn_shift,
                     float *bound_out, int B, int C, void *stream);
 int roreg_ft_nonlin(const float *Xin , const float *x_spatial, const float *bias,
diff --git a/roreg_amd/_abi.py b/roreg_amd/_abi.py
--- a/roreg_amd/_abi.py
+++ b/roreg_amd/_abi.py
@@ -79,6 +79,9 @@
     'roreg_linear_cat3': (c_int, [_P, _P, _P, _P, c_int, c_int, _P, _P, c_int, _P, _P]),
     'roreg_gemm_persistent': (c_int, [c_int]),
     'roreg_gemm_thin': (c_int, [c_int]),
+    'roreg_gf_finish_route': (c_int, [c_int]),
+    'roreg_irrep_gemm_f16x2_rows': (c_int, [_P, _P, _P, _P, c_int, c_int, c_int, _P]),
+    'roreg_gf_finish': (c_int, [_P, _P, _P, _P, _P, _P, _P, _P, _P, c_int, _P]),
     'roreg_instnorm_stats': (c_int, [_P, c_int, c_int, c_float, _P, _P, _P, c_int, c_int, _P]),
     'roreg_mlp_tail': (c_int, [_P, c_int, c_int, _P, _P, _P, _P, _P, c_int, c_int, _P]),
     'roreg_mlp_tail_mfma': (c_int, [_P, c_int, c_int, _P, _P, _P, _P, _P, c_int, c_int, _P]),
diff --git a/roreg_amd/_hip_fourier.py b/roreg_amd/_hip_fourier.py
--- a/roreg_amd/_hip_fourier.py
+++ b/roreg_amd/_hip_fourier.py
@@ -7,7 +7,7 @@
 from . import hip as _core
 from .hip import HipError, _check, _feat, _ptr, _stream, lib
 
-__all__ = ['DenseSplitLayer', 'IRREP_DIMS', 'IRREP_OFFSETS', '_bf16_split3', '_keypoint_of_columns', '_ptr_array', '_res_ptr', '_tile_cache', 'bf16_split3_frags', 'bf16_split3_pack', 'bound_exp', 'coef_pitch', 'coef_size', 'coef_views', 'dense_split', 'ensure_fourier', 'f16_scale_exp', 'f16_split2_frags', 'f16_split2_pack', 'frag_pack', 'ft_nonlin', 'ft_nonlin_gathered', 'ft_nonlin_packed', 'gemm_persistent', 'gemm_thin', 'group_conv_split_pack', 'irrep_gemm', 'next_bound', 'next_bound_spatial', 'pack_coefs_f16x2', 'row_bound', 'unpack_coefs_f16x2', 'words_to_planes']
+__all__ = ['DenseSplitLayer', 'IRREP_DIMS', 'IRREP_OFFSETS', '_bf16_split3', '_keypoint_of_columns', '_ptr_array', '_res_ptr', '_tile_cache', 'bf16_split3_frags', 'bf16_split3_pack', 'bound_exp', 'coef_pitch', 'coef_size', 'coef_views', 'dense_split', 'ensure_fourier', 'f16_scale_exp', 'f16_split2_frags', 'f16_split2_pack', 'frag_pack', 'ft_nonlin', 'ft_nonlin_gathered', 'ft_nonlin_packed', 'gemm_persistent', 'gemm_thin', 'gf_finish', 'gf_finish_rows', 'gf_finish_usable', 'group_conv_split_pack', 'irrep_gemm', 'irrep_gemm_rows', 'next_bound', 'next_bound_spatial', 'pack_coefs_f16x2', 'row_bound', 'unpack_coefs_f16x2', 'words_to_planes']
 
 
 _fourier_ready = False
@@ -119,6 +119,44 @@
                         """`with hip.gemm_thin(True | False):` -- whether the thin layers (C == 32 or O == 32, fp16 x 2, word layout, no residual) run on their own
     kernels inside the block (roreg_gemm_thin; the default) or on the generic one.  Same bits either way -- tests and A/B measurements.""")
 
+gf_finish = _GemmSwitch('roreg_gf_finish_route', lambda on: int(bool(on)),
+                        """`with hip.gf_finish(True | False):` -- whether the engine ends the extractor with Conv_out in per-keypoint rows + gf_finish_kernel (roreg_gf_finish_route;
+    the default, ROREG_GF_FINISH=0 in the environment turns it off) or with the four kernels ft_nonlin, gf_finalize, inv_descriptor, feat_coefs.  Same bits either
+    way -- tests and A/B measurements.""")
+
+
+def gf_finish_usable(gemm_mode, *dtypes):
+    return (gemm_mode == 'f16x2' and _core.GEMM_MODE == 'f16x2' and all(d == torch.float32 for d in dtypes)
+            and lib().roreg_gemm_thin(-1) == 1 and lib().roreg_gf_finish_route(-1) == 1)
+
+
+def irrep_gemm_rows(X_buf, C, B, f16x2, x_bound):
+    Bp = coef_pitch(B)
+    wl, w_exp = f16x2
+    if X_buf.numel() != 60 * C * Bp or x_bound is None or x_bound.numel() != Bp:
+        raise HipError(f'irrep_gemm_rows: X_buf must hold 60*C*{Bp} words and x_bound {Bp} values')
+    out = torch.empty((Bp, 60, 32), dtype=torch.float32, device=X_buf.device)
+    _check(lib().roreg_irrep_gemm_f16x2_rows(_ptr_array(coef_views(X_buf, C, B)), _ptr(out), _ptr_array(wl), _ptr(x_bound, torch.float32), int(w_exp), C, Bp,
+                                             _stream()), 'roreg_irrep_gemm_f16x2_rows')
+    return out
+
+
+def gf_finish_rows(T3r, x, b_out, roles=None):
+    ensure_fourier()
+    B = int(x.shape[0])
+    if x.shape[1:] != (32, 60) or x.dtype != torch.float32 or not x.is_contiguous() or T3r.shape != (coef_pitch(B), 60, 32) or b_out.numel() != 32:
+        raise HipError('gf_finish_rows: T3r [Bp,60,32], x [B,32,60] contiguous float32, b_out [32]')
+    eqv = torch.empty((B, 32, 60), dtype=torch.float32, device=x.device)
+    eft = torch.empty((B, 32, 60), dtype=torch.float32, device=x.device)
+    inv = torch.empty((B, 32), dtype=torch.float32, device=x.device)
+    scale = shift = role = None
+    if roles is not None:
+        scale, shift, role = _core._role_args(roles, B)
+        scale, shift = scale[64:], shift[64:]
+    _check(lib().roreg_gf_finish(_ptr(T3r, torch.float32), _ptr(x, torch.float32), _ptr(b_out, torch.float32), _ptr(scale), _ptr(shift), _ptr(eqv), _ptr(inv),
+                                 _ptr(role), _ptr(eft), B, _stream()), 'roreg_gf_finish')
+    return eqv, inv, eft
+
 
 def row_bound(x, bn=None, roles=None):
     B, C = int(x.shape[0]), int(x.shape[1])
diff --git a/roreg_amd/csrc/fourier.hip b/roreg_amd/csrc/fourier.hip
--- a/roreg_amd/csrc/fourier.hip
+++ b/roreg_amd/csrc/fourier.hip
@@ -131,6 +131,7 @@
     const float *Add[NIRR];
     const float *xbound;
     int w_exp;
+    int out_rows;
     const float *nb_u, *nb_v;
     float *out_bound;
     int O;
@@ -672,7 +673,7 @@
     }
 }
 
-template <int D, int CB>
+template <int D, int CB, bool ROWS = false>
 __device__ __forceinline__ void thin_m_body(const GemmSplitDescs &p, int irr, int nt, f16x8 *as) {
     constexpr int NI = 2 * D;
     constexpr int NDMA = (NI + 3) / 4;
@@ -776,6 +777,24 @@
 #pragma unroll
         for (int r = 0; r < 16; ++r) { const int o = cd_row32(r, h); ur[r] = p.nb_u[o]; vr[r] = p.nb_v[o]; }
     }
+    if constexpr (ROWS) {
+        constexpr int off = D == 1 ? 0 : D == 4 ? 19 : D == 5 ? 35 : -1;
+#pragma unroll
+        for (int cb = 0; cb < CB; ++cb) {
+            const int nc = n + cb, b = column_keypoint(nc, D), i = (nc >> 5) % D;
+            float *__restrict__ ob = p.Out[0] + ((size_t)b * ROREG_G + (off >= 0 ? off : 1 + 9 * (irr - 1)) + i * D) * ROREG_F + 4 * h;
+#pragma unroll
+            for (int rb = 0; rb < D; ++rb)
+#pragma unroll
+                for (int r4 = 0; r4 < 4; ++r4) {
+                    f32x4 o;
+#pragma unroll
+                    for (int e = 0; e < 4; ++e) o[e] = acc[rb][cb][4 * r4 + e] * oscale[cb];
+                    *reinterpret_cast<f32x4 *>(ob + rb * ROREG_F + 8 * r4) = o;
+                }
+        }
+        return;
+    }
     float *__restrict__ ob = p.Out[irr] + n + (size_t)(4 * h) * N;
 #pragma unroll
     for (int rb = 0; rb < D; ++rb)
@@ -808,6 +827,17 @@
         case 1: case 2: thin_m_body<3, 2>(p, irr, nt, as); break;
         case 3: thin_m_body<4, 1>(p, irr, nt, as); break;
         default: thin_m_body<5, 1>(p, irr, nt, as); break;
+    }
+}
+__global__ __launch_bounds__(256, 2) void irrep_gemm_thin_m_rows_kernel(GemmSplitDescs p) {
+    __shared__ __attribute__((aligned(16))) f16x8 as[3 * 10 * 64];
+    int irr, nt;
+    thin_wg_irrep<true>(p, irr, nt);
+    switch (irr) {
+        case 0: thin_m_body<1, 2, true>(p, irr, nt, as); break;
+        case 1: case 2: thin_m_body<3, 2, true>(p, irr, nt, as); break;
+        case 3: thin_m_body<4, 1, true>(p, irr, nt, as); break;
+        default: thin_m_body<5, 1, true>(p, irr, nt, as); break;
     }
 }
 #undef ROREG_WAIT_LDS2
@@ -2013,6 +2043,204 @@
 #undef OFF_OF
 #undef OFF_Q
 
+struct GfFinishParams {
+    const float *T3r;
+    const float *x;
+    const float *b_out;
+    const float *role_scale, *role_shift;
+    float *eqv, *inv, *role_out, *eqv_ft;
+    const f16x8 *A1h, *A2h;
+    int f_exp, B;
+};
+
+__global__ __launch_bounds__(256, 2) void gf_finish_kernel(GfFinishParams p) {
+    constexpr int NA = 4 * 2 * 2 * 64 * 4;
+    extern __shared__ __attribute__((aligned(16))) float gf_smem[];
+    float *sA1 = gf_smem, *sA2 = gf_smem + NA, *sT = gf_smem + 2 * NA, *sRole = sT + 4 * 32 * 65;
+    const int lane = threadIdx.x & 63, jn = lane & 31, h = lane >> 5;
+    {
+        const float *g1 = reinterpret_cast<const float *>(p.A1h), *g2 = reinterpret_cast<const float *>(p.A2h);
+        for (int i = threadIdx.x; i < NA; i += 256) { sA1[i] = g1[i]; sA2[i] = g2[i]; }
+        if (threadIdx.x < 128) sRole[threadIdx.x] = p.role_scale ? (threadIdx.x < 64 ? p.role_scale[threadIdx.x] : p.role_shift[threadIdx.x - 64]) : 0.f;
+    }
+    __syncthreads();
+    const f16x8 *sA1h = reinterpret_cast<const f16x8 *>(sA1), *sA2h = reinterpret_cast<const f16x8 *>(sA2);
+    const int wave_global = __builtin_amdgcn_readfirstlane((blockIdx.x * 256 + threadIdx.x) >> 6);
+    const int n_waves = gridDim.x * 4;
+    const int B = p.B;
+    const bool act = lane < ROREG_G;
+    const float bo = p.b_out[jn] + 0.f;
+    float *ti = sT + (threadIdx.x >> 6) * (32 * 65);
+
+    auto load = [&](int b, float (&cv)[32], float (&xv)[32]) {
+        const float *t = p.T3r + (size_t)b * (ROREG_G * ROREG_F) + h * (8 * ROREG_F) + jn;
+        static_for<32>([&](auto ic) {
+            constexpr int st = decltype(ic)::value / 8, e = decltype(ic)::value % 8;
+            constexpr int q0 = 16 * st + e, q1 = 16 * st + 8 + e;
+            if constexpr (q1 < ROREG_G) cv[st * 8 + e] = __builtin_nontemporal_load(t + q0 * ROREG_F);
+            else cv[st * 8 + e] = __builtin_nontemporal_load(t + q0 * ROREG_F - h * (8 * ROREG_F));
+        });
+        const float *xs = p.x + (size_t)b * (ROREG_F * ROREG_G) + (act ? lane : 0);
+        static_for<32>([&](auto ic) {
+            constexpr int c = decltype(ic)::value;
+            xv[c] = xs[c * ROREG_G];
+        });
+    };
+    auto table_mma = [&](const f16x8 *a, const f16x8 (&b)[2], f32x16 c) {
+        f16x8 av[2];
+#pragma unroll
+        for (int pl = 0; pl < 2; ++pl) av[pl] = a[64 * pl];
+        return split_mma<2>(av, b, c);
+    };
+    auto column_scale = [&](float mx, float &xscale, float &oscale) {
+        mx = fmaxf(mx, __shfl_xor(mx, 32));
+        int e = 0;
+        if (mx > 0.f && mx < __builtin_inff()) { int ex; (void)frexpf(mx, &ex); e = 14 - ex; }
+        xscale = ldexpf(1.f, e); oscale = ldexpf(1.f, -(e + p.f_exp));
+    };
+    auto transform = [&](const f16x8 *tab, const float (&k)[32], f32x16 (&v)[2]) {
+        float mx = 0.f;
+#pragma unroll
+        for (int s = 0; s < 32; ++s) mx = fmaxf(mx, fabsf(k[s]));
+        float xsc, osc;
+        column_scale(mx, xsc, osc);
+#pragma unroll
+        for (int t = 0; t < 2; ++t)
+#pragma unroll
+            for (int r = 0; r < 16; ++r) v[t][r] = 0.f;
+#pragma unroll
+        for (int st = 0; st < 4; ++st) {
+            float x8[8];
+#pragma unroll
+            for (int e = 0; e < 8; ++e) x8[e] = k[st * 8 + e];
+            f16x8 bh, bl;
+            split2(x8, xsc, bh, bl);
+            const f16x8 b[2] = {bh, bl};
+            v[0] = table_mma(tab + ((st * 2 + 0) * 2) * 64 + lane, b, v[0]);
+            v[1] = table_mma(tab + ((st * 2 + 1) * 2) * 64 + lane, b, v[1]);
+        }
+#pragma unroll
+        for (int t = 0; t < 2; ++t)
+#pragma unroll
+            for (int r = 0; r < 16; ++r) v[t][r] *= osc;
+    };
+#define ROREG_LDS_DONE() asm volatile("s_waitcnt lgkmcnt(0)" ::: "memory")
+    auto process = [&](int b, int next_b, float (&cv)[32], float (&xv)[32], float (&cnext)[32], float (&xnext)[32]) {
+        asm volatile("" ::: "memory");
+        load(next_b, cnext, xnext);
+        __builtin_amdgcn_sched_barrier(0);
+#pragma unroll
+        for (int c = 0; c < 32; ++c) ti[c * 65 + lane] = xv[c];
+        asm volatile("" ::: "memory");
+        float k[32];
+#pragma unroll
+        for (int s = 0; s < 32; ++s) k[s] = (16 * (s >> 3) + 8 + (s & 7) < ROREG_G || h == 0) ? cv[s] : 0.f;
+        f32x16 v[2];
+        transform(sA1h, k, v);
+        ROREG_LDS_DONE();
+#pragma unroll
+        for (int t = 0; t < 2; ++t)
+#pragma unroll
+            for (int r = 0; r < 16; ++r) {
+                const int g = cd_row32(r, h, t * 32);
+                if (g < ROREG_G) ti[jn * 65 + g] = (v[t][r] + bo) + ti[jn * 65 + g];
+            }
+        ROREG_LDS_DONE();
+        float w[ROREG_F];
+        float n2 = 0.f;
+#pragma unroll
+        for (int f = 0; f < ROREG_F; ++f) {
+            w[f] = act ? ti[f * 65 + lane] : 0.f;
+            n2 += w[f] * w[f];
+        }
+        const float nrm = clamp_min_norm(sqrtf(n2));
+        float *dst = p.eqv + (size_t)b * (ROREG_F * ROREG_G) + lane;
+#pragma unroll
+        for (int f = 0; f < ROREG_F; ++f) w[f] = w[f] / nrm;
+        if (act) {
+#pragma unroll
+            for (int f = 0; f < ROREG_F; ++f) { dst[f * ROREG_G] = w[f]; ti[f * 65 + lane] = w[f]; }
+        }
+        if (p.role_scale) {
+            float m1 = 0.f, m0 = 0.f;
+            const f32x4 *rs = reinterpret_cast<const f32x4 *>(sRole);
+#pragma unroll
+            for (int c4 = 0; c4 < ROREG_F / 4; ++c4) {
+                const f32x4 s1 = rs[c4], s0 = rs[8 + c4], h1 = rs[16 + c4], h0 = rs[24 + c4];
+#pragma unroll
+                for (int e = 0; e < 4; ++e) {
+                    m1 = fmaxf(m1, fmaxf(fmaf(w[4 * c4 + e], s1[e], h1[e]), 0.f));
+                    m0 = fmaxf(m0, fmaxf(fmaf(w[4 * c4 + e], s0[e], h0[e]), 0.f));
+                }
+            }
+            if (!act) m1 = m0 = 0.f;
+#pragma unroll
+            for (int o = 32; o > 0; o >>= 1) { m1 = fmaxf(m1, __shfl_xor(m1, o)); m0 = fmaxf(m0, __shfl_xor(m0, o)); }
+            if (lane == 0) { p.role_out[(size_t)b * 4 + 2] = m1; p.role_out[(size_t)b * 4 + 3] = m0; }
+        }
+        ROREG_LDS_DONE();
+        {
+            float m = 0.f;
+            if (lane < ROREG_F) m = (float)((double)np_pairwise_sum(ti + lane * 65, ROREG_G) / 60.0);
+            float sq[ROREG_F];
+#pragma unroll
+            for (int f = 0; f < ROREG_F; ++f) {
+                const float mf = __shfl(m, f);
+                sq[f] = __fmul_rn(mf, mf);
+            }
+            const float inrm = __fadd_rn(sqrtf(np_pairwise_sum(sq, ROREG_F)), 1e-5f);
+            if (lane < ROREG_F) p.inv[(size_t)b * ROREG_F + lane] = __fdiv_rn(m, inrm);
+        }
+#pragma unroll
+        for (int t = 0; t < 2; ++t)
+#pragma unroll
+            for (int r = 0; r < 16; ++r) {
+                const int g = cd_row32(r, h, t * 32);
+                float xg = (g < ROREG_G ? ti[jn * 65 + g] : 0.f) + 0.f;
+                if (g >= ROREG_G) xg = 0.f;
+                k[t * 16 + r] = xg;
+            }
+        ROREG_LDS_DONE();
+        f32x16 o[2];
+        transform(sA2h, k, o);
+        if (h == 0) {
+            static_for<32>([&](auto ic) {
+                constexpr int S = decltype(ic)::value;
+                ti[jn * 65 + kPS.qa[S]] = o[S / 16][S % 16];
+            });
+        } else {
+            static_for<32>([&](auto ic) {
+                constexpr int S = decltype(ic)::value;
+                if constexpr (kPS.qb[S] < ROREG_G) ti[jn * 65 + kPS.qb[S]] = o[S / 16][S % 16];
+            });
+        }
+        ROREG_LDS_DONE();
+        float *fo = p.eqv_ft + (size_t)b * (ROREG_F * ROREG_G) + lane;
+#pragma unroll
+        for (int c8 = 0; c8 < 4; ++c8) {
+            float tv[8];
+#pragma unroll
+            for (int q = 0; q < 8; ++q) tv[q] = ti[(c8 * 8 + q) * 65 + lane];
+#pragma unroll
+            for (int q = 0; q < 8; ++q)
+                if (act) fo[(c8 * 8 + q) * ROREG_G] = tv[q];
+        }
+        ROREG_LDS_DONE();
+    };
+#undef ROREG_LDS_DONE
+    if (wave_global < B) {
+        const int last = wave_global + ((B - 1 - wave_global) / n_waves) * n_waves;
+        float ca[32], xa[32], cb[32], xb[32];
+        load(wave_global, ca, xa);
+        __builtin_amdgcn_s_waitcnt(0x0F70);
+        for (int b = wave_global; b <= last; b += 2 * n_waves) {
+            const int b1 = min(b + n_waves, last), b2 = min(b + 2 * n_waves, last);
+            process(b, b1, ca, xa, cb, xb);
+            process(b1, b2, cb, xb, ca, xa);
+        }
+    }
+}
+
 float *g_A1 = nullptr, *g_A2 = nullptr;
 uint16_t *g_A1s = nullptr, *g_A2s = nullptr, *g_A1h = nullptr, *g_A2h = nullptr;
 int g_f_exp = 0;
@@ -2203,9 +2431,11 @@
     }
 };
 static GemmSwitch g_gemm_persist{"ROREG_GEMM_PERSIST", 0, 2};
+static GemmSwitch g_gf_finish{"ROREG_GF_FINISH", 1, 1};
 static GemmSwitch g_gemm_thin{"ROREG_GEMM_THIN", 1, 1};
 extern "C" int roreg_gemm_persistent(int on) { return g_gemm_persist.set(on); }
 extern "C" int roreg_gemm_thin(int on) { return g_gemm_thin.set(on); }
+extern "C" int roreg_gf_finish_route(int on) { return g_gf_finish.set(on); }
 static int gemm_cu_count() {
     static const int n = [] {
         int dev = 0, cus = 0;
@@ -2225,6 +2455,7 @@
         p.K[r] = dims[r] * C; p.M[r] = dims[r] * O; p.Mpad[r] = round_up(dims[r] * O, 128); p.N[r] = dims[r] * B;
         if (WO == 4 && p.Mpad[r] % 256 != 0) { roreg::set_error("%s: tile_m = 256 needs O %% 256 == 0 (got %d)", what, O); return 2; }
     }
+    p.out_rows = 0;
     p.xbound = xbound; p.w_exp = w_exp; p.nb_u = nb_u; p.nb_v = nb_v; p.out_bound = out_bound; p.O = O;
     if constexpr (NP == 2) {
         if (!x_planes && !Add && (O == 32 || (C == 32 && O % 32 == 0 && O <= 512)) && g_gemm_thin.get()) {
@@ -2481,3 +2712,41 @@
     ROREG_CHECK_LAUNCH("roreg_feat_coefs");
     return 0;
 }
+
+extern "C" int roreg_irrep_gemm_f16x2_rows(const float *const *X, float *T3r, const void *const *Wsplit2, const float *x_bound_dev, int w_exp, int C, int B,
+                                           void *stream) {
+    ROREG_REQUIRE(X && T3r && Wsplit2 && x_bound_dev && C > 0 && B > 0, "roreg_irrep_gemm_f16x2_rows: bad arguments");
+    ROREG_REQUIRE(C % 32 == 0 && B % 32 == 0, "roreg_irrep_gemm_f16x2_rows: C %% 32 and B %% 32 must be 0 (got %d, %d)", C, B);
+    static const int dims[5] = {1, 3, 3, 4, 5};
+    constexpr int O = ROREG_F;
+    GemmSplitDescs p;
+    memset(&p, 0, sizeof(p));
+    int wgs = 0;
+    for (int r = 0; r < 5; ++r) {
+        p.X[r] = X[r]; p.W[r] = Wsplit2[r];
+        p.K[r] = dims[r] * C; p.M[r] = dims[r] * O; p.Mpad[r] = round_up(dims[r] * O, 128); p.N[r] = dims[r] * B;
+        const int tc = thin_tile_cols<true>(r);
+        wgs += (p.N[r] + tc - 1) / tc;
+    }
+    p.Out[0] = T3r; p.out_rows = 1; p.xbound = x_bound_dev; p.w_exp = w_exp; p.O = O;
+    hipLaunchKernelGGL(irrep_gemm_thin_m_rows_kernel, dim3(wgs), dim3(256), 0, roreg::as_stream(stream), p);
+    ROREG_CHECK_LAUNCH("roreg_irrep_gemm_f16x2_rows");
+    return 0;
+}
+
+extern "C" int roreg_gf_finish(const float *T3r, const float *x, const float *b_out, const float *role_scale, const float *role_shift, float *eqv, float *inv,
+                               float *role_out, float *eqv_ft, int B, void *stream) {
+    if (B == 0) return 0;
+    ROREG_REQUIRE(g_A1h && g_A2h, "roreg_gf_finish: roreg_set_fourier_tables has not been called");
+    ROREG_REQUIRE(T3r && x && b_out && eqv && inv && eqv_ft && B > 0, "roreg_gf_finish: bad arguments");
+    ROREG_REQUIRE((role_scale == nullptr) == (role_shift == nullptr) && (role_scale == nullptr) == (role_out == nullptr),
+                  "roreg_gf_finish: role_scale, role_shift and role_out go together");
+    GfFinishParams p;
+    memset(&p, 0, sizeof(p));
+    p.T3r = T3r; p.x = x; p.b_out = b_out; p.role_scale = role_scale; p.role_shift = role_shift;
+    p.eqv = eqv; p.inv = inv; p.role_out = role_out; p.eqv_ft = eqv_ft;
+    p.A1h = reinterpret_cast<const f16x8 *>(g_A1h); p.A2h = reinterpret_cast<const f16x8 *>(g_A2h); p.f_exp = g_f_exp; p.B = B;
+    constexpr size_t lds = (2 * (4 * 2 * 2 * 64 * 4) + 4 * 32 * 65 + 128) * sizeof(float);
+    const long long want = ((long long)B + 3) / 4, cap = 2ll * gemm_cu_count() * 4;
+    return roreg::launch_lds("roreg_gf_finish", gf_finish_kernel, dim3((unsigned)(want > cap ? cap : want)), dim3(256), lds, roreg::as_stream(stream), p);
+}
diff --git a/roreg_amd/csrc/pointwise.hip b/roreg_amd/csrc/pointwise.hip
--- a/roreg_amd/csrc/pointwise.hip
+++ b/roreg_amd/csrc/pointwise.hip
@@ -1,25 +1,10 @@
 #include "common.h"
+#include "primitives.h"
 
 #pragma clang fp contract(off)
 
 namespace {
 
-__device__ __forceinline__ float np_pairwise_sum(const float *a, int n) {
-    float r[8];
-#pragma unroll
-    for (int j = 0; j < 8; ++j) r[j] = a[j];
-    int i = 8;
-    for (; i < n - (n % 8); i += 8) {
-#pragma unroll
-        for (int j = 0; j < 8; ++j) r[j] = __fadd_rn(r[j], a[i + j]);
-    }
-    float res = __fadd_rn(__fadd_rn(__fadd_rn(r[0], r[1]), __fadd_rn(r[2], r[3])),
-                          __fadd_rn(__fadd_rn(r[4], r[5]), __fadd_rn(r[6], r[7])));
-    for (; i < n; ++i) res = __fadd_rn(res, a[i]);
-    return res;
-}
-
-__device__ __forceinline__ float clamp_min_norm(float n) { return n < 1e-4f ? 1e-4f : n; }
 
 template <typename OT>
 __global__ __launch_bounds__(256) void gf_finalize_kernel(const float *__restrict__ raw, void *__restrict__ eqv_v,
diff --git a/roreg_amd/csrc/primitives.h b/roreg_amd/csrc/primitives.h
--- a/roreg_amd/csrc/primitives.h
+++ b/roreg_amd/csrc/primitives.h
@@ -74,6 +74,23 @@
     return v;
 }
 
+__device__ __forceinline__ float np_pairwise_sum(const float *a, int n) {
+    float r[8];
+#pragma unroll
+    for (int j = 0; j < 8; ++j) r[j] = a[j];
+    int i = 8;
+    for (; i < n - (n % 8); i += 8) {
+#pragma unroll
+        for (int j = 0; j < 8; ++j) r[j] = __fadd_rn(r[j], a[i + j]);
+    }
+    float res = __fadd_rn(__fadd_rn(__fadd_rn(r[0], r[1]), __fadd_rn(r[2], r[3])),
+                          __fadd_rn(__fadd_rn(r[4], r[5]), __fadd_rn(r[6], r[7])));
+    for (; i < n; ++i) res = __fadd_rn(res, a[i]);
+    return res;
+}
+
+__device__ __forceinline__ float clamp_min_norm(float n) { return n < 1e-4f ? 1e-4f : n; }
+
 __device__ __forceinline__ int seg_of(const int *__restrict__ off, int n_seg, int r) {
     int lo = 0, hi = n_seg - 1;
     while (lo < hi) {
diff --git a/roreg_amd/engine.py b/roreg_amd/engine.py
--- a/roreg_amd/engine.py
+++ b/roreg_amd/engine.py
@@ -289,11 +289,22 @@
         x = feats if torch.is_tensor(feats) else torch.from_numpy(np.ascontiguousarray(feats, np.float32))
         x = x.to('cuda', torch.float32).to(self.feat_dtype).contiguous()
         roles = self._role_request(x.shape[0])
+        eqv, inv, eft = self._extract_rows(x, roles)
+        k = keys if torch.is_tensor(keys) else torch.from_numpy(np.ascontiguousarray(keys, np.float64))
+        return CloudState(before=x, eqv=eqv, eqv_ft=eft, inv=inv, keys=k.to('cuda', torch.float64).contiguous(),
+                          role=roles[2] if roles else None, role_bn=roles[0] if roles else None)
+
+    def _extract_rows(self, x, roles):
+        net = self.gf.PartI_net
         with torch.no_grad():
-            eqv = self.gf.PartI_net(x, want_inv=False, out_dtype=self.feat_dtype, roles=roles)['eqv']
-        k = keys if torch.is_tensor(keys) else torch.from_numpy(np.ascontiguousarray(keys, np.float64))
-        return CloudState(before=x, eqv=eqv, eqv_ft=hip.feat_coefs(eqv), inv=hip.inv_descriptor(eqv, roles=roles), keys=k.to('cuda', torch.float64).contiguous(),
-                          role=roles[2] if roles else None, role_bn=roles[0] if roles else None)
+            if x.shape[0] and net.mode == 'fourier':
+                if net._fourier is None:
+                    from .network.gf_fourier import FourierGF
+                    object.__setattr__(net, '_fourier', FourierGF(net))
+                if hip.gf_finish_usable(net._fourier.gemm, x.dtype, self.feat_dtype):
+                    return net._fourier.forward_finished(x.contiguous(), roles=roles)
+            eqv = net(x, want_inv=False, out_dtype=self.feat_dtype, roles=roles)['eqv']
+        return eqv, hip.inv_descriptor(eqv, roles=roles), hip.feat_coefs(eqv)
 
     def _role_request(self, n):
         bn = self.et.conv_init_bn() if self.et is not None else None
@@ -331,10 +342,7 @@
             else:
                 xcat = torch.cat(xs, 0)
             roles = self._role_request(rows)
-            with torch.no_grad():
-                eqv = self.gf.PartI_net(xcat, want_inv=False, out_dtype=self.feat_dtype, roles=roles)['eqv']
-            inv = hip.inv_descriptor(eqv, roles=roles)
-            eft = hip.feat_coefs(eqv)
+            eqv, inv, eft = self._extract_rows(xcat, roles)
             on_host = [q for q in range(i, j) if not (torch.is_tensor(keys_list[q]) and keys_list[q].is_cuda)]
             k_dev = {}
             if on_host:
diff --git a/roreg_amd/network/gf_fourier.py b/roreg_amd/network/gf_fourier.py
--- a/roreg_amd/network/gf_fourier.py
+++ b/roreg_amd/network/gf_fourier.py
@@ -59,28 +59,44 @@
             self.nb_3 = hip.next_bound(self.bn_3, self.l_2.bias, self.l_in.bias)
             self._nb_key = self._key
 
+    def _conv_out_operand(self, x, roles=None):
+        self._plan()
+        hip.ensure_fourier()
+        B = x.shape[0]
+        sp = 'f16x2'
+        self._plan_bounds()
+        b0 = hip.row_bound(x, roles=roles)
+        X0 = hip.ft_nonlin(B, 32, x_spatial=x, split=sp, out_bound=b0)
+        T0, b1 = hip.irrep_gemm(X0, None, 32, 256, B, f16x2=self.l_in.wsplit2, x_bound=b0, next_bound=self.nb_1)
+        del X0
+        xd = hip.use_planes(512) and hip.use_planes(256)
+        X1 = hip.ft_nonlin(B, 256, coef_in=T0, bias=self.l_in.bias, bn=self.bn_1, split=sp, out_bound=b1, planes=xd)
+        T1, b2 = hip.irrep_gemm(X1, None, 256, 512, B, f16x2=self.l_1.wsplit2, x_bound=b1, next_bound=self.nb_2, x_planes=xd)
+        del X1
+        X2 = hip.ft_nonlin(B, 512, coef_in=T1, bias=self.l_1.bias, bn=self.bn_2, split=sp, out_bound=b2, planes=xd)
+        del T1
+        T2, b3 = hip.irrep_gemm(X2, None, 512, 256, B, f16x2=self.l_2.wsplit2, x_bound=b2, next_bound=self.nb_3, add=T0, x_planes=xd)
+        del X2, T0
+        return hip.ft_nonlin(B, 256, coef_in=T2, bias=self.l_2.bias, bias2=self.l_in.bias, bn=self.bn_3, split=sp, out_bound=b3), b3
+
+    def forward_finished(self, x, roles=None):
+        if self.gemm != 'f16x2' or x.dtype != torch.float32:
+            raise hip.HipError('FourierGF.forward_finished: the fp16 x 2 mode on float32 features only')
+        B = x.shape[0]
+        X3, b3 = self._conv_out_operand(x, roles)
+        T3r = hip.irrep_gemm_rows(X3, 256, B, self.l_out.wsplit2, b3)
+        del X3
+        return hip.gf_finish_rows(T3r, x, self.l_out.bias, roles=roles)
+
     def forward_raw(self, x, roles=None):
         self._plan()
         hip.ensure_fourier()
         B = x.shape[0]
         sp = {'f32': False, 'bf16x3': True, 'f16x2': 'f16x2'}[self.gemm]
         if self.gemm == 'f16x2':
-            self._plan_bounds()
-            b0 = hip.row_bound(x, roles=roles)
-            X0 = hip.ft_nonlin(B, 32, x_spatial=x, split=sp, out_bound=b0)
-            T0, b1 = hip.irrep_gemm(X0, None, 32, 256, B, f16x2=self.l_in.wsplit2, x_bound=b0, next_bound=self.nb_1)
-            del X0
-            xd = hip.use_planes(512) and hip.use_planes(256)
-            X1 = hip.ft_nonlin(B, 256, coef_in=T0, bias=self.l_in.bias, bn=self.bn_1, split=sp, out_bound=b1, planes=xd)
-            T1, b2 = hip.irrep_gemm(X1, None, 256, 512, B, f16x2=self.l_1.wsplit2, x_bound=b1, next_bound=self.nb_2, x_planes=xd)
-            del X1
-            X2 = hip.ft_nonlin(B, 512, coef_in=T1, bias=self.l_1.bias, bn=self.bn_2, split=sp, out_bound=b2, planes=xd)
-            del T1
-            T2, b3 = hip.irrep_gemm(X2, None, 512, 256, B, f16x2=self.l_2.wsplit2, x_bound=b2, next_bound=self.nb_3, add=T0, x_planes=xd)
-            del X2, T0
-            X3 = hip.ft_nonlin(B, 256, coef_in=T2, bias=self.l_2.bias, bias2=self.l_in.bias, bn=self.bn_3, split=sp, out_bound=b3)
-            del T2
+            X3, b3 = self._conv_out_operand(x, roles)
             T3 = hip.irrep_gemm(X3, None, 256, 32, B, f16x2=self.l_out.wsplit2, x_bound=b3)
+            del X3
             return hip.ft_nonlin(B, 32, coef_in=T3, bias=self.l_out.bias, resid_spatial=x, spatial_out=True, split=sp)
 
         if roles is not None:
```

Measured after the change: 1114, median of 6. 1.01x the previous value.
